# AiRyunn/BoT

Measured on AMD Instinct MI355X. Metric: edges/sec full-batch GAT fwd+bwd on ogbn-arxiv; achieved HBM GB/s vs peak, higher is better.
Workload: dtype f32

## Files before the change

### bot_amd/_C.py

```python
from __future__ import annotations

import ctypes
import os
from ctypes import c_char_p, c_double, c_float, c_int32, c_int64, c_uint64, c_void_p

import torch

_HERE = os.path.dirname(os.path.abspath(__file__))
LIB_PATH = os.environ.get("BOT_AMD_LIB") or os.path.join(_HERE, "lib", "libbot_gnn.so")
ABI_VERSION = 19

if not os.path.exists(LIB_PATH):
    raise ImportError(
        f"{LIB_PATH} is missing: build the gfx950 kernels first "
        "(`make -C bot_amd/csrc` or `python -c 'import __graft_entry__ as g; g.build()'`). "
        "bot_amd has no CPU / PyTorch fallback."
    )
_lib = ctypes.CDLL(LIB_PATH)

_P = c_void_p
_SIGS = {
    "bot_abi_version": (ctypes.c_int, []),
    "bot_last_error": (c_char_p, []),
    "bot_last_kernel": (c_char_p, []),
    "bot_debug_abort_trace": (ctypes.c_int, [c_char_p]),
    "bot_row_plan_default_chunk": (c_int32, [c_int64]),
    "bot_row_plan_size_host": (ctypes.c_int, [_P, c_int64, c_int32, _P, _P, _P]),
    "bot_row_plan_fill_host": (ctypes.c_int, [_P, c_int64, c_int32, _P, _P, _P]),
    "bot_degrees_i64": (ctypes.c_int, [_P, c_int64, _P, _P]),
    "bot_spmm_workspace_floats": (c_int64, [c_int64, c_int32, c_int32]),
    "bot_spmm_set_layout": (ctypes.c_int, [c_int32]),
    "bot_spmm_f32": (ctypes.c_int, [_P, _P, c_int64, c_int64, _P, c_int64, _P, _P, c_int64, _P, c_int64, c_int64, _P, _P,
                                    c_int32, c_int32, _P, c_int64, c_int64, _P, c_int64, c_int64, _P, _P]),
    "bot_spmm_blocked_f32": (ctypes.c_int, [_P, _P, _P, _P, _P, c_int32, c_int32, c_int32, c_int32, c_int32, c_int32, _P, c_int64, _P,
                                            c_int32, c_int32, _P, c_int64, _P, c_int64, _P]),
    "bot_spmm_dot_f32": (ctypes.c_int, [_P, _P, c_int64, c_int64, _P, c_int64, _P, _P, c_int64, _P, c_int64, c_int64, _P, _P,
                                        _P, c_int64, c_int64, c_int32, c_int32, _P, c_int64, c_int64, _P, _P, _P, _P]),
    "bot_spmm_bcast_f32": (ctypes.c_int, [_P, _P, c_int64, c_int64, _P, c_int64, _P, _P, c_int64, _P, c_int64, _P, _P, c_int32,
                                          c_int32, _P, c_int64, c_int64, _P, _P]),
    "bot_spmm_bcast_halves_f16": (ctypes.c_int, [_P, _P, c_int64, c_int64, _P, c_int64, _P, _P, c_int64, _P, c_int64, _P, _P, c_int32, c_int32, _P, _P,
                                                 c_int64, c_int64, c_int32, c_int32, _P, _P]),
    "bot_spmm_dot_bcast_f32": (ctypes.c_int, [_P, _P, c_int64, c_int64, _P, c_int64, _P, _P, c_int64, _P, c_int64, c_int64, _P,
                                              _P, _P, c_int64, c_int32, c_int32, _P, c_int64, _P, _P, _P]),
    "bot_sddmm_dot_f32": (ctypes.c_int, [_P, _P, c_int64, c_int64, _P, c_int64, _P, c_int64, c_int64, _P, c_int64, c_int64,
                                         c_int32, c_int32, _P, _P, c_int32, _P]),
    "bot_sddmm_dot_bcast_f32": (ctypes.c_int, [_P, _P, c_int64, c_int64, _P, c_int64, _P, c_int64, _P, c_int64, c_int64, c_int32,
                                               c_int32, _P, _P, _P]),
    "bot_sddmm_u_add_v_f32": (ctypes.c_int, [_P, _P, c_int64, _P, _P, c_int32, _P, _P]),
    "bot_gat_attn_fwd_f32": (ctypes.c_int, [_P, _P, c_int64, c_int64, _P, c_int64, c_int32, _P, _P, _P, _P, _P, c_float,
                                            c_int32, _P, _P, _P, c_float, c_uint64, _P, _P, _P]),
    "bot_gat_attn_bwd_f32": (ctypes.c_int, [_P, _P, c_int64, c_int64, _P, c_int64, c_int32, _P, _P, _P, _P, c_float, c_int32,
                                            _P, _P, _P, _P, _P, _P, _P, c_float, c_uint64, _P, _P]),
    "bot_gat_infer_workspace_floats": (c_int64, [c_int64, c_int32, c_int32]),
    "bot_gat_infer_f32": (ctypes.c_int, [_P, _P, c_int64, c_int64, _P, c_int64, _P, _P, c_int64, c_int64, _P, c_int64, c_int64,
                                         _P, c_int64, _P, c_int64, _P, _P, c_float, c_int32, c_int32, _P, c_int64, c_int64, _P, _P,
                                         c_int32, _P, c_int64, c_int64, _P, _P, _P]),
    "bot_segment_sum_f32": (ctypes.c_int, [_P, c_int64, c_int64, _P, c_int64, c_int32, _P, _P, c_int32, _P, _P]),
    "bot_gather_rows_f32": (ctypes.c_int, [_P, c_int64, _P, c_int64, c_int32, _P, c_int64, _P]),
    "bot_scatter_add_rows_f32": (ctypes.c_int, [_P, c_int64, _P, c_int64, c_int32, _P, c_int64, _P]),
    "bot_merge_weight_fwd_f32": (ctypes.c_int, [_P, _P, _P, _P, c_int32, c_int32, c_int32, c_int32, c_int32, c_int32, _P, _P]),
    "bot_merge_weight_bwd_f32": (ctypes.c_int, [_P, _P, _P, c_int32, c_int32, c_int32, c_int32, c_int32, c_int32, _P, _P, _P, _P, _P, _P]),
    "bot_edge_mlp_workspace_floats": (c_int64, []),
    "bot_edge_mlp_fwd_f32": (ctypes.c_int, [_P, c_int32, _P, _P, c_int32, _P, c_int32, c_int64, _P, _P]),
    "bot_edge_mlp_bwd_f32": (ctypes.c_int, [_P, c_int32, _P, _P, c_int32, _P, c_int32, _P, c_int64, _P, _P, _P, _P, _P]),
    "bot_random_keep_workspace_bytes": (c_int64, []),
    "bot_random_keep_u8": (ctypes.c_int, [c_int64, c_int64, c_uint64, _P, _P, _P]),
    "bot_halves_workspace_floats": (c_int64, []),
    "bot_halves_scale_f32": (ctypes.c_int, [_P, c_int64, c_int64, c_int32, _P, _P, _P]),
    "bot_halves_split_f16": (ctypes.c_int, [_P, c_int64, c_int64, c_int32, _P, c_int32, _P, c_int64, c_int32, _P]),
    "bot_halves_split_cols_f16": (ctypes.c_int, [_P, c_int64, c_int64, c_int32, _P, c_int32, _P, c_int64, c_int32, c_int32, _P]),
    "bot_halves_split_heads_f16": (ctypes.c_int, [_P, c_int64, c_int64, c_int32, c_int32, _P, _P, c_int64, c_int32, c_int32, _P]),
    "bot_gemm_halves_f32": (ctypes.c_int, [c_int32, c_int32, c_int64, c_int64, c_int64, _P, _P, c_int64, _P, c_int64, _P, c_int64,
                                           c_int32, c_int64, c_int64, c_int64, c_float, _P, c_int64, c_int32, c_int32, _P]),
    "bot_gemm_halves3_nt_f32": (ctypes.c_int, [c_int64, c_int64, c_int64, _P, _P, _P, c_int64, c_int64, _P, c_int64, c_int64, _P, c_int64,
                                               c_int32, _P]),
    "bot_gemm_halves3_tn_workspace_floats": (c_int64, [c_int64, c_int64, c_int64]),
    "bot_gemm_halves3_tn_f32": (ctypes.c_int, [c_int64, c_int64, c_int64, c_int64, c_int64, _P, _P, _P, c_int64, c_int64, _P, c_int64, c_int64, _P,
                                               c_int64, _P, c_int32, _P]),
    "bot_gemm_halves3_nt_grouped_f32": (ctypes.c_int, [c_int64, c_int64, _P, _P, _P, c_int64, c_int64, _P, c_int64, c_int64, _P, c_int64, c_int32, _P,
                                                       c_int32, _P, _P, c_int32, _P, c_int32, _P]),
    "bot_gemm_halves3_tn_grouped_workspace_floats": (c_int64, [c_int64, c_int32]),
    "bot_gemm_halves3_tn_grouped_f32": (ctypes.c_int, [c_int64, _P, _P, _P, c_int64, c_int64, _P, c_int64, c_int64, _P, c_int32, _P, _P, c_int32, _P]),
    "bot_tn_narrow_workspace_floats": (c_int64, [c_int64, c_int32, c_int32]),
    "bot_tn_narrow_f32": (ctypes.c_int, [_P, c_int64, _P, c_int64, c_int64, c_int32, c_int32, _P, c_int64, c_int32, _P, _P]),
    "bot_bn_act_bwd_reduce_max_f32": (ctypes.c_int, [_P, c_int64, _P, c_int64, c_int64, c_int32, _P, _P, _P, _P, c_int32, c_float, c_uint64, _P, _P, _P, _P, _P]),
    "bot_bn_bwd_bound_f32": (ctypes.c_int, [c_int32, c_int64, _P, _P, _P, c_double, _P, _P, _P, _P]),
    "bot_bn_act_bwd_apply_halves_f32": (ctypes.c_int, [_P, c_int64, _P, c_int64, c_int64, c_int32, _P, _P, _P, _P, c_int32, c_float, c_uint64, _P, _P, _P, c_double,
                                                       _P, c_int64, _P, _P, c_int64, c_int32, c_int32, c_int32, _P]),
    "bot_label_split_f32": (ctypes.c_int, [_P, c_int64, _P, c_int64, _P, c_float, c_uint64, _P, c_int32, _P, _P, _P, _P, _P]),
    "bot_build_input_f32": (ctypes.c_int, [_P, c_int64, c_int64, c_int32, c_int32, _P, c_float, c_uint64, _P, _P, c_int64, _P]),
    "bot_build_input_reuse_f32": (ctypes.c_int, [_P, c_int64, c_int64, c_int32, c_int32, _P, _P, _P, c_int64, c_float, c_uint64, _P, _P, c_int64, _P]),
    "bot_node_loss_f32": (ctypes.c_int, [_P, c_int64, c_int64, c_int32, _P, c_int64, _P, _P, c_int32, c_float, _P, c_int64, _P, c_int64, _P]),
    "bot_rmsprop_step_f32": (ctypes.c_int, [c_int32, _P, _P, _P, _P, c_float, _P, c_float, c_float, c_float, _P]),
    "bot_gemm_halves_last_algo": (ctypes.c_int, [_P, _P]),
    "bot_gemm_halves_library_version": (ctypes.c_int, [_P, _P]),
    "bot_tn_gemm_workspace_floats": (c_int64, [c_int64, c_int32, c_int32, c_int32]),
    "bot_tn_gemm_f32": (ctypes.c_int, [_P, c_int64, _P, c_int64, c_int64, c_int32, c_int32, _P, c_int64, c_int32, c_int32, c_int64, c_int64,
                                       c_int64, _P, _P]),
    "bot_skinny_gemm_f32": (ctypes.c_int, [_P, c_int64, _P, c_int64, c_int32, _P, c_int64, c_int64, c_int32, c_int32, c_int32, c_int32,
                                           c_int64, c_int64, c_int64, _P]),
    "bot_bn_workspace_floats": (c_int64, [c_int32]),
    "bot_colstats_f32": (ctypes.c_int, [_P, c_int64, c_int64, c_int32, _P, _P, _P, _P]),
    "bot_colsum_f32": (ctypes.c_int, [_P, c_int64, c_int64, c_int32, _P, _P, _P]),
    "bot_bn_stats_f32": (ctypes.c_int, [_P, c_int64, c_int64, c_int32, c_float, c_float, _P, _P, _P, _P, _P, _P, _P]),
    "bot_bn_stats_halves_f32": (ctypes.c_int, [_P, c_int64, c_int64, c_int32, c_float, c_float, _P, _P, _P, _P, _P, _P, _P, c_float, _P, _P, _P]),
    "bot_bn_act_fwd_halves_f32": (ctypes.c_int, [_P, c_int64, c_int64, c_int32, _P, _P, _P, _P, c_int32, c_float, c_uint64, _P, _P, c_int64,
                                                 _P, _P, c_int64, c_int32, c_int32, _P]),
    "bot_bn_act_fwd_f32": (ctypes.c_int, [_P, c_int64, c_int64, c_int32, _P, _P, _P, _P, c_int32, c_float, c_uint64, _P, _P, c_int64, _P]),
    "bot_bn_act_bwd_reduce_f32": (ctypes.c_int, [_P, c_int64, _P, c_int64, c_int64, c_int32, _P, _P, _P, _P, c_int32, c_float,
                                                 c_uint64, _P, _P, _P, _P, _P]),
    "bot_bn_act_bwd_apply_f32": (ctypes.c_int, [_P, c_int64, _P, c_int64, c_int64, c_int32, _P, _P, _P, _P, c_int32, c_float,
                                                c_uint64, _P, _P, _P, c_double, _P, c_int64, _P, _P]),
    "bot_halves_tn_combine_f32": (ctypes.c_int, [_P, _P, c_int32, c_int32, c_int32, c_int32, _P, _P, _P, c_int64, _P]),
    "bot_halves_scale_from_slots2_f32": (ctypes.c_int, [_P, c_float, _P, c_float, _P, _P]),
    "bot_halves_tail_f16": (ctypes.c_int, [c_int64, c_int32, _P, _P, _P, _P, _P, c_int64, c_int32, _P]),
    "bot_spmm_dot_halves_fits": (ctypes.c_int, [_P, c_int64, c_int64, _P, c_int64, c_int64, c_int32, c_int32, _P, c_int64, c_int64, c_int32]),
    "bot_spmm_dot_halves_f16": (ctypes.c_int, [_P, _P, c_int64, c_int64, _P, c_int64, _P, _P, c_int64, _P, c_int64, c_int64, _P, _P, _P, c_int64, c_int64,
                                               c_int32, c_int32, _P, _P, c_int64, c_int64, c_int32, _P, _P, _P]),
    "bot_gemm_halves3_nt_bn_rows": (c_int32, [c_int64]),
    "bot_gemm_halves3_nt3_f32": (ctypes.c_int, [c_int64, c_int64, c_int64, _P, _P, c_int64, _P, _P, c_int64, c_int64, _P, c_int64, c_int64, c_int32, _P, c_int64,
                                                _P, c_int32, _P]),
    "bot_bn_act_bwd_reduce_partials_f32": (ctypes.c_int, [_P, c_int32, c_int32, _P, _P, _P]),
    "bot_bn_bwd_bound_partials_f32": (ctypes.c_int, [c_int32, _P, c_int32, _P, _P, c_double, _P, _P, _P, _P]),
    "bot_bn_bwd_partials_finish_f32": (ctypes.c_int, [_P, _P, c_int32, c_int32, _P, _P, c_int32, c_double, _P, _P, _P, _P]),
    "bot_gemm_halves3_nt2_f32": (ctypes.c_int, [c_int64, c_int64, c_int64, _P, _P, c_int64, _P, _P, c_int64, c_int64, _P, c_int64, c_int64, c_int32, _P, c_int64,
                                                c_int32, _P]),
    "bot_halves_split_frag_f16": (ctypes.c_int, [_P, c_int64, c_int64, c_int32, _P, _P, c_int32, _P]),
    "bot_gemm_halves3_tn2_f32": (ctypes.c_int, [c_int64, c_int64, c_int64, c_int64, c_int64, _P, _P, _P, c_int64, _P, c_int64, c_int64, _P, c_int64, c_int64, _P,
                                                c_int64, _P, c_int32, _P]),
    "bot_stream_create": (ctypes.c_int, [c_int32, _P]),
    "bot_gemm_halves3_nt_grouped2_f32": (ctypes.c_int, [c_int64, c_int64, _P, _P, _P, c_int64, c_int64, _P, c_int64, c_int64, _P, c_int64, c_int32, _P,
                                                        c_int32, _P, _P, c_int32, _P, _P, _P, _P, c_int32, c_int32, _P]),
    "bot_bn_stats_halves_partials_f32": (ctypes.c_int, [_P, _P, c_int32, _P, c_int64, c_int32, c_float, c_float, _P, _P, _P, _P, _P, _P, _P, c_float, _P, _P, _P]),
    "bot_absmax_slots": (c_int32, []),
    "bot_absmax_slots_f32": (ctypes.c_int, [_P, c_int64, c_int64, c_int32, _P, _P]),
    "bot_halves_scale_from_slots_f32": (ctypes.c_int, [_P, _P, _P]),
    "bot_sample_neighbors_count_i32": (ctypes.c_int, [_P, c_int64, _P, c_int64, c_int32, _P, _P]),
    "bot_sample_neighbors_i32": (ctypes.c_int, [_P, c_int64, _P, c_int64, c_int32, c_uint64, _P, _P, _P]),
    "bot_block_tiles": (c_int64, [c_int64]),
    "bot_block_mark_i32": (ctypes.c_int, [_P, c_int64, _P, _P, c_int64, _P, c_int64, _P, _P, _P]),
    "bot_block_relabel_i32": (ctypes.c_int, [_P, c_int64, _P, _P, _P, c_int64, _P, c_int64, _P, c_int64, _P, _P, _P, _P]),
    "bot_subgraph_mark_i32": (ctypes.c_int, [_P, c_int64, _P, c_int64, _P, _P]),
    "bot_subgraph_count_i32": (ctypes.c_int, [_P, _P, c_int64, _P, c_int64, _P, _P, _P]),
    "bot_subgraph_fill_i32": (ctypes.c_int, [_P, _P, _P, c_int64, _P, c_int64, _P, _P, _P, _P, _P]),
    "bot_subgraph_unmark_i32": (ctypes.c_int, [_P, c_int64, _P, c_int64, _P]),
    "bot_sample_weights_prepare_f32": (ctypes.c_int, [_P, _P, c_int64, c_int64, _P, _P, _P, _P, _P]),
    "bot_sample_neighbors_weighted_count_i32": (ctypes.c_int, [_P, c_int64, _P, c_int64, c_int32, _P, _P]),
    "bot_sample_neighbors_weighted_i32": (ctypes.c_int, [_P, _P, _P, c_int64, _P, c_int64, c_int32, c_uint64, _P, _P, _P]),
}
for _name, (_res, _args) in _SIGS.items():
    _fn = getattr(_lib, _name)
    _fn.restype, _fn.argtypes = _res, _args
EXPORTED = tuple(_SIGS)

if _lib.bot_abi_version() != ABI_VERSION:
    raise ImportError(f"libbot_gnn.so ABI {_lib.bot_abi_version()} != binding ABI {ABI_VERSION}; rebuild")


class BotKernelError(RuntimeError):
    pass


PROFILE = None


PROFILE_SKIP = ()


def _timed(name, key, launch):
    if PROFILE is None or name in PROFILE_SKIP:
        return launch()
    e0, e1 = torch.cuda.Event(enable_timing=True), torch.cuda.Event(enable_timing=True)
    e0.record()
    rc = launch()
    e1.record()
    PROFILE.append((name, key, e0, e1, _lib.bot_last_kernel().decode()))
    return rc


def _check(rc: int, what: str):
    if rc != 0:
        raise BotKernelError(f"{what} failed (rc={rc}): {_lib.bot_last_error().decode()}")


def _ptr(t):
    return None if t is None else t.data_ptr()


def _ld(t):
    return max(int(t.stride(-2)), int(t.shape[-1])) if t.shape[-2] == 1 else int(t.stride(-2))


def _stream():
    return torch.cuda.current_stream().cuda_stream


def _dev(*ts):
    dev = None
    for t in ts:
        if t is None:
            continue
        if not t.is_cuda:
            raise BotKernelError(
                "bot_amd kernels run on MI355X only: got a CPU tensor and there is no CPU fallback "
                "(move the graph and features to the GPU)")
        if dev is None:
            dev = t.device
        elif t.device != dev:
            raise BotKernelError(f"operands live on different devices ({dev} and {t.device}): graph structures and features "
                                 "must be on the same GPU")


def _f32(t, name):
    if t is not None and t.dtype != torch.float32:
# ... 699 lines not shown
    return (ctypes.c_int64 * len(flat))(*flat)


def gemm_halves3_nt_grouped(a, b, scale_a, scale_b, a2_off, b2_off, out, groups, k_seg, mode=0, col_scale=None, col_shift=None, relu=False, absmax=None,
                            stats=None):
    _dev(a, b, out, scale_a, scale_b, col_scale, col_shift, absmax)
    assert a.dtype == torch.float16 and b.dtype == torch.float16 and a.dim() == 2 and b.dim() == 2 and a.stride(1) == 1 and b.stride(1) == 1
    assert out.dtype == torch.float32 and out.stride(-1) == 1
    tab = _table(groups, 6)
    sp = sm = sv = None
    sF = 0
    if stats is not None:
        sp, sm, sv = stats
        _dev(sp, sm, sv)
        sF = sv.shape[1]
        tiles = (a.shape[0] + 255) // 256
        assert sp.shape == (tiles, 2, sF) and sm.shape == (tiles, 2, sF) and sv.shape == (tiles, sF)
        assert sp.is_contiguous() and sm.is_contiguous() and sv.is_contiguous()
        assert sp.dtype == sm.dtype == sv.dtype == torch.float32
    _check(_timed("gemm_halves", (a.shape[0], sum(int(g[1]) * 96 * int(g[4]) for g in groups), 1, 1), lambda: _lib.bot_gemm_halves3_nt_grouped2_f32(
        a.shape[0], b.shape[0], scale_a.data_ptr(), scale_b.data_ptr(), a.data_ptr(), _ld(a), a2_off, b.data_ptr(), _ld(b), b2_off, out.data_ptr(),
        int(out.stride(-2)), len(groups), tab, int(k_seg), _ptr(col_scale), _ptr(col_shift), int(bool(relu)), _ptr(absmax), _ptr(sp), _ptr(sm), _ptr(sv),
        int(sF), int(mode), _stream())), "gemm_halves3_nt_grouped")
    return out


def gemm_halves3_tn_grouped(x, d, scale_x, scale_d, x2_off, d2_off, out, tiles, mode=0):
    _dev(x, d, out, scale_x, scale_d)
    assert x.dtype == torch.float16 and d.dtype == torch.float16 and x.stride(1) == 1 and d.stride(1) == 1 and x.shape[0] == d.shape[0]
    assert out.dtype == torch.float32 and out.is_contiguous()
    n = x.shape[0]
    ws = torch.empty(int(_lib.bot_gemm_halves3_tn_grouped_workspace_floats(n, len(tiles))), dtype=torch.float32, device=x.device)
    tab = _table(tiles, 7)
    _check(_timed("gemm_halves", (n, sum(3 * int(t[1]) * int(t[3]) for t in tiles), 1, 1), lambda: _lib.bot_gemm_halves3_tn_grouped_f32(
        n, scale_x.data_ptr(), scale_d.data_ptr(), x.data_ptr(), _ld(x), x2_off, d.data_ptr(), _ld(d), d2_off, out.data_ptr(), len(tiles), tab,
        ws.data_ptr(), int(mode), _stream())), "gemm_halves3_tn_grouped")
    return out


def gemm_halves3_tn(x, d, scale_x, scale_d, piece_x, piece_d, k, p, mode=0, x2_off=None, d2_off=None, scale_d2=None, p_split=0):
    _dev(x, d, scale_x, scale_d, scale_d2)
    n = x.shape[0]
    out = torch.empty((k, p), dtype=torch.float32, device=x.device)
    ws = torch.empty(int(_lib.bot_gemm_halves3_tn_workspace_floats(n, piece_x, piece_d)), dtype=torch.float32, device=x.device)
    _check(_timed("gemm_halves", (k, p, 3 * n, 1), lambda: _lib.bot_gemm_halves3_tn2_f32(
        n, k, p, piece_x, piece_d, scale_x.data_ptr(), scale_d.data_ptr(), _ptr(scale_d2), int(p_split), x.data_ptr(), _ld(x),
        2 * piece_x if x2_off is None else x2_off, d.data_ptr(), _ld(d), 2 * piece_d if d2_off is None else d2_off,
        out.data_ptr(), _ld(out), ws.data_ptr(), int(mode), _stream())), "gemm_halves3_tn")
    return out


def _idx64(t, name):
    if t.dtype != torch.int64 or not t.is_contiguous() or t.dim() != 1:
        raise BotKernelError(f"{name} must be a contiguous 1-D int64 tensor (got {t.dtype}, stride {tuple(t.stride())})")


def _labels64(labels):
    if labels.dtype != torch.int64:
        raise BotKernelError(f"labels must be int64 (got {labels.dtype})")
    lab = labels.reshape(labels.shape[0], -1)
    if lab.shape[1] > 1 and lab.stride(1) != 1:
        lab = lab.contiguous()
    return lab


def label_split(train_idx, labels, mask, mask_rate, seed, use_labels, code, wn):
    _dev(train_idx, labels, wn)
    _idx64(train_idx, "train_idx")
    count = torch.empty(1, dtype=torch.float32, device=wn.device)
    ws = torch.empty(128, dtype=torch.int32, device=wn.device)
    lab = _labels64(labels)
    if wn.dtype != torch.float32 or not wn.is_contiguous() or (code is not None and (code.dtype != torch.int32 or not code.is_contiguous())):
        raise BotKernelError("label_split: wn must be contiguous float32, code contiguous int32")
    m = None
    if mask is not None:
        _dev(mask)
        m = mask.to(torch.bool).contiguous().view(torch.uint8)
        if m.numel() != train_idx.numel():
            raise BotKernelError("label_split: mask must have one entry per training node")
    _check(_lib.bot_label_split_f32(train_idx.data_ptr(), train_idx.numel(), lab.data_ptr(), lab.stride(0), _ptr(m), float(mask_rate), int(seed),
                                    _seed_off(1.0), int(bool(use_labels)), _ptr(code), wn.data_ptr(), count.data_ptr(), ws.data_ptr(), _stream()), "label_split")
    return count


def build_input(feat, code, n_classes, p, seed):
    _dev(feat)
    _f32(feat, "feat")
    n, F = feat.shape
    out = torch.empty((n, F + n_classes), dtype=torch.float32, device=feat.device)
    _check(_lib.bot_build_input_f32(feat.data_ptr(), _ld(feat), n, F, n_classes, _ptr(code), float(p), int(seed), _seed_off(p), out.data_ptr(), _ld(out),
                                    _stream()), "build_input")
    return out


REUSE_CALLS = 0


def build_input_reuse(feat, code, reuse, pred, n_classes, p, seed, out=None):
    global REUSE_CALLS
    _dev(feat, code, reuse, pred, out)
    _f32(feat, "feat"), _f32(pred, "pred"), _f32(out, "out")
    n, F = feat.shape
    if feat.stride(1) != 1 and F > 1:
        feat = feat.contiguous()
    if pred.dim() != 2 or pred.shape[0] != n or pred.shape[1] < n_classes or (pred.stride(1) != 1 and pred.shape[1] > 1):
        raise BotKernelError(f"build_input_reuse: pred must be [{n}, >= {n_classes}] with unit column stride, got {tuple(pred.shape)}")
    if code is None or code.dtype != torch.int32 or not code.is_contiguous() or code.numel() != n:
        raise BotKernelError(f"build_input_reuse: code must be contiguous int32 [{n}]")
    if reuse is not None and (reuse.dtype != torch.uint8 or not reuse.is_contiguous() or reuse.numel() != n):
        raise BotKernelError(f"build_input_reuse: reuse must be contiguous uint8 [{n}]")
    if out is None:
        out = torch.empty((n, F + n_classes), dtype=torch.float32, device=feat.device)
    elif out.shape != (n, F + n_classes) or out.stride(1) != 1:
        raise BotKernelError(f"build_input_reuse: out must be [{n}, {F + n_classes}] with unit column stride")
    _check(_lib.bot_build_input_reuse_f32(feat.data_ptr(), _ld(feat), n, F, n_classes, code.data_ptr(), _ptr(reuse), pred.data_ptr(), _ld(pred), float(p),
                                          int(seed), _seed_off(p), out.data_ptr(), _ld(out), _stream()), "build_input_reuse")
    REUSE_CALLS += 1
    torch.autograd.graph.increment_version(out)
    return out


LOSS_KINDS = {"logit": 0, "loge": 1, "savage": 2}


def node_loss(x, labels, wn, count, kind, eps, want_grad=True):
    _dev(x, labels, wn, count)
    _f32(x, "x")
    n, C = x.shape
    n_pad = (n + 63) // 64 * 64
    y = torch.empty(n_pad, dtype=torch.float32, device=x.device)
    dx = torch.empty((n, C), dtype=torch.float32, device=x.device) if want_grad else None
    lab = _labels64(labels)
    if wn.dtype != torch.float32 or not wn.is_contiguous() or count.dtype != torch.float32:
        raise BotKernelError("node_loss: wn / count must be contiguous float32")
    _check(_lib.bot_node_loss_f32(x.data_ptr(), _ld(x), n, C, lab.data_ptr(), lab.stride(0), wn.data_ptr(), count.data_ptr(), LOSS_KINDS[kind], float(eps),
                                  y.data_ptr(), n_pad, _ptr(dx), C, _stream()), "node_loss")
    return y, dx


def rmsprop_step(params, grads, square_avgs, lr, alpha, eps, weight_decay, lr_dev=None):
    for i in range(0, len(params), 48):
        ps, gs, sq = params[i:i + 48], grads[i:i + 48], square_avgs[i:i + 48]
        k = len(ps)
        for t in (*ps, *gs, *sq):
            if t.dtype != torch.float32 or not t.is_contiguous():
                raise BotKernelError("rmsprop_step: contiguous float32 tensors only")
        P = (c_void_p * k)(*[t.data_ptr() for t in ps])
        G = (c_void_p * k)(*[t.data_ptr() for t in gs])
        S = (c_void_p * k)(*[t.data_ptr() for t in sq])
        Nn = (c_int64 * k)(*[t.numel() for t in ps])
        if lr_dev is not None and (lr_dev.dtype != torch.float32 or lr_dev.device != ps[0].device):
            raise BotKernelError("rmsprop_step: a tensor learning rate must be float32 on the parameters' device")
        _check(_lib.bot_rmsprop_step_f32(k, P, G, S, Nn, float(lr), _ptr(lr_dev), float(alpha), float(eps), float(weight_decay), _stream()), "rmsprop_step")


def skinny_gemm(a, b, *, b_is_kn, out, accumulate=False, batch=1, strides=(0, 0, 0), m=None, n=None, k=None, ldc=None):
    _dev(a, b, out)
    for t, name in ((a, "a"), (b, "b"), (out, "out")):
        _f32(t, name)
        if t.stride(-1) != 1 and t.shape[-1] != 1:
            raise BotKernelError(f"skinny_gemm: {name} must have unit column stride")
    if m is None:
        m, k = a.shape[-2], a.shape[-1]
    if n is None:
        n = b.shape[-1] if b_is_kn else b.shape[-2]
    sa, sb, sc = strides
    _check(_timed("skinny_gemm", (m, n, k, batch), lambda: _lib.bot_skinny_gemm_f32(
        a.data_ptr(), _ld(a), b.data_ptr(), _ld(b), int(b_is_kn), out.data_ptr(), _ld(out) if ldc is None else ldc, m, n, k,
        int(accumulate), batch, sa, sb, sc, _stream())), "skinny_gemm")
    return out


def tn_gemm(x, y, *, out=None, batch=1, strides=(0, 0, 0), n=None, kx=None, ky=None, transpose_out=False):
    _dev(x, y)
    _f32(x, "x"), _f32(y, "y")
    if (x.stride(-1) != 1 and x.shape[-1] != 1) or (y.stride(-1) != 1 and y.shape[-1] != 1):
        raise BotKernelError("tn_gemm: operands must have unit column stride")
    if n is None:
        n, kx, ky = x.shape[-2], x.shape[-1], y.shape[-1]
    if out is None:
        shp = (ky, kx) if transpose_out else (kx, ky)
        out = torch.empty(shp if batch == 1 else (batch,) + shp, dtype=torch.float32, device=x.device)
    sx, sy, so = strides
    if batch > 1 and so == 0:
        so = out.stride(0)
    ws = torch.empty(int(_lib.bot_tn_gemm_workspace_floats(n, kx, ky, batch)), dtype=torch.float32, device=x.device)
    _check(_timed("tn_gemm", (n, kx, ky, batch), lambda: _lib.bot_tn_gemm_f32(
        x.data_ptr(), _ld(x), y.data_ptr(), _ld(y), n, kx, ky, out.data_ptr(), _ld(out), int(transpose_out), batch, sx, sy, so,
        ws.data_ptr(),
        _stream())), "tn_gemm")
    return out


def tn_narrow(x, y, out, transpose_out=False):
    _dev(x, y, out)
    _f32(x, "x"), _f32(y, "y"), _f32(out, "out")
    n, kx, ky = x.shape[0], x.shape[1], y.shape[1]
    assert y.shape[0] == n and out.shape == ((ky, kx) if transpose_out else (kx, ky))
    if x.stride(1) != 1 or y.stride(1) != 1 or (out.stride(1) != 1 and out.shape[1] != 1):
        raise BotKernelError("tn_narrow: operands must have unit column stride")
    ws = torch.empty(int(_lib.bot_tn_narrow_workspace_floats(n, kx, ky)), dtype=torch.float32, device=x.device)
    _check(_timed("tn_narrow", (n, kx, ky), lambda: _lib.bot_tn_narrow_f32(
        x.data_ptr(), _ld(x), y.data_ptr(), _ld(y), n, kx, ky, out.data_ptr(), _ld(out), int(transpose_out), ws.data_ptr(), _stream())), "tn_narrow")
    return out


def colsum(x):
    _dev(x)
    x = _mat(x, "x")
    n, F = x.shape
    out = torch.empty(F, dtype=torch.float32, device=x.device)
    _check(_lib.bot_colsum_f32(x.data_ptr(), x.stride(0), n, F, out.data_ptr(), _bn_ws(F, x.device).data_ptr(), _stream()), "colsum")
    return out


def _written(*ts):
    ts = [t for t in ts if t is not None]
    if ts:
        torch._C._increment_version(ts)


def bn_stats(x, eps, momentum, running_mean=None, running_var=None, num_batches_tracked=None):
    _dev(x, running_mean, running_var)
    x = _mat(x, "x")
    n, F = x.shape
    mean = torch.empty(F, dtype=torch.float32, device=x.device)
    invstd = torch.empty(F, dtype=torch.float32, device=x.device)
    _check(_lib.bot_bn_stats_f32(x.data_ptr(), x.stride(0), n, F, float(eps), float(momentum), mean.data_ptr(), invstd.data_ptr(),
                                 _ptr(running_mean), _ptr(running_var), _ptr(num_batches_tracked), _bn_ws(F, x.device).data_ptr(),
                                 _stream()), "bn_stats")
    _written(running_mean, running_var, num_batches_tracked)
    return mean, invstd


def bn_stats_halves(x, eps, momentum, running_mean, running_var, num_batches_tracked, weight, bias, p):
    _dev(x, running_mean, running_var, weight, bias)
    x = _mat(x, "x")
    n, F = x.shape
    mean = torch.empty(F, dtype=torch.float32, device=x.device)
    invstd = torch.empty(F, dtype=torch.float32, device=x.device)
    hscale = torch.empty(2, dtype=torch.float32, device=x.device)
    _check(_lib.bot_bn_stats_halves_f32(x.data_ptr(), x.stride(0), n, F, float(eps), float(momentum), mean.data_ptr(), invstd.data_ptr(),
                                        _ptr(running_mean), _ptr(running_var), _ptr(num_batches_tracked), _ptr(weight), _ptr(bias),
                                        float(p), hscale.data_ptr(), _bn_ws(F, x.device).data_ptr(), _stream()), "bn_stats_halves")
    _written(running_mean, running_var, num_batches_tracked)
    return mean, invstd, hscale


def bn_stats_halves_partials(part, minmax, pivot, n, eps, momentum, running_mean, running_var, num_batches_tracked, weight, bias, p):
    _dev(part, minmax, pivot, running_mean, running_var, weight, bias)
    nblk, _, F = part.shape
    assert pivot.shape == (nblk, F) and minmax.shape == part.shape and part.is_contiguous() and minmax.is_contiguous() and pivot.is_contiguous()
    mean = torch.empty(F, dtype=torch.float32, device=part.device)
    invstd = torch.empty(F, dtype=torch.float32, device=part.device)
    hscale = torch.empty(2, dtype=torch.float32, device=part.device)
    ws = torch.empty(F, dtype=torch.float32, device=part.device)
    _check(_lib.bot_bn_stats_halves_partials_f32(part.data_ptr(), minmax.data_ptr(), int(nblk), pivot.data_ptr(), int(n), int(F), float(eps), float(momentum),
                                                 mean.data_ptr(), invstd.data_ptr(), _ptr(running_mean), _ptr(running_var), _ptr(num_batches_tracked),
                                                 _ptr(weight), _ptr(bias), float(p), hscale.data_ptr(), ws.data_ptr(), _stream()), "bn_stats_halves_partials")
    _written(running_mean, running_var, num_batches_tracked)
    return mean, invstd, hscale


def bn_act_fwd(x, mean, invstd, weight, bias, relu, p, seed, halves=None, want_y=True):
    _dev(x, mean, invstd)
    x = _mat(x, "x")
    n, F = x.shape
    if halves is not None:
        hscale, piece = halves[:2]
        pieces = halves[2] if len(halves) > 2 else 3
        y = torch.empty((n, F), dtype=torch.float32, device=x.device) if want_y else None
        buf = torch.empty((n, pieces * piece), dtype=torch.float16, device=x.device)
        _check(_timed("bn_act_fwd", (F,), lambda: _lib.bot_bn_act_fwd_halves_f32(
            x.data_ptr(), x.stride(0), n, F, mean.data_ptr(), invstd.data_ptr(), _ptr(weight), _ptr(bias), int(relu), float(p),
            int(seed), _seed_off(p), _ptr(y), F, hscale.data_ptr(), buf.data_ptr(), buf.stride(0), piece, pieces, _stream())),
            "bn_act_fwd_halves")
        return y, buf
    y = torch.empty((n, F), dtype=torch.float32, device=x.device)
    _check(_timed("bn_act_fwd", (F,), lambda: _lib.bot_bn_act_fwd_f32(
        x.data_ptr(), x.stride(0), n, F, mean.data_ptr(), invstd.data_ptr(), _ptr(weight), _ptr(bias), int(relu), float(p),
        int(seed), _seed_off(p), y.data_ptr(), y.stride(0), _stream())), "bn_act_fwd")
    return y


def bn_act_bwd_reduce(dy, x, mean, invstd, weight, bias, relu, p, seed, want_max=False):
    _dev(dy, x)
    dy, x = _mat(dy, "dy"), _mat(x, "x")
    n, F = x.shape
    sg = torch.empty(F, dtype=torch.float32, device=x.device)
    sgx = torch.empty(F, dtype=torch.float32, device=x.device)
    ws = _bn_ws(F, x.device)
    fn = _lib.bot_bn_act_bwd_reduce_max_f32 if want_max else _lib.bot_bn_act_bwd_reduce_f32
    _check(fn(dy.data_ptr(), dy.stride(0), x.data_ptr(), x.stride(0), n, F, mean.data_ptr(), invstd.data_ptr(), _ptr(weight), _ptr(bias), int(relu),
              float(p), int(seed), _seed_off(p), sg.data_ptr(), sgx.data_ptr(), ws.data_ptr(), _stream()), "bn_act_bwd_reduce")
    return (sg, sgx, ws) if want_max else (sg, sgx)


def bn_bwd_bound(ws, n, sum_g, sum_gx, total_count, weight, invstd, slots):
    _dev(ws, invstd, slots)
    F = invstd.shape[0]
    _check(_lib.bot_bn_bwd_bound_f32(F, n, ws.data_ptr(), _ptr(sum_g), _ptr(sum_gx), float(total_count), _ptr(weight), invstd.data_ptr(), slots.data_ptr(),
                                     _stream()), "bn_bwd_bound")
    return slots


def bn_act_bwd_apply_halves(dy, x, mean, invstd, weight, bias, relu, p, seed, sum_g, sum_gx, total_count, hscale, hout, hD, hDP, out=None, h2_off=None):
# ... 62 lines not shown


class PreparedWeights:

    def __init__(self, prefix, n_pos):
        self.prefix, self.n_pos = prefix, n_pos


def sample_weights_prepare(csc, w):
    _dev(csc.indptr, w)
    _f32(w, "edge weights")
    E = int(csc.indices.numel())
    if not (w.dim() == 1 or (w.dim() == 2 and w.shape[1] == 1)) or w.shape[0] != E:
        raise ValueError(f"edge weights must be [E] or [E, 1] with E = {E}, got {tuple(w.shape)}")
    w = w.reshape(-1).contiguous()
    dev = w.device
    prefix = torch.empty(E, dtype=torch.int64, device=dev)
    n_pos = torch.empty(csc.n_rows, dtype=torch.int32, device=dev)
    flag = torch.empty(1, dtype=torch.int32, device=dev)
    rc = _lib.bot_sample_weights_prepare_f32(csc.indptr.data_ptr(), csc.eid.data_ptr(), csc.n_rows, E, w.data_ptr(), prefix.data_ptr(),
                                             n_pos.data_ptr(), flag.data_ptr(), _stream())
    if rc == -2:
        raise ValueError(f"edge weights: {_lib.bot_last_error().decode()}")
    _check(rc, "sample_weights_prepare")
    return PreparedWeights(prefix, n_pos)


def sample_neighbors_weighted(csc, prepared, seeds, k, seed):
    _dev(csc.indptr, prepared.prefix, seeds)
    assert seeds.dtype == torch.int32 and seeds.is_contiguous()
    n = int(seeds.numel())
    dev = seeds.device
    counts = torch.empty(n, dtype=torch.int32, device=dev)
    _check(_lib.bot_sample_neighbors_weighted_count_i32(prepared.n_pos.data_ptr(), csc.n_rows, _ptr(seeds), n, int(k), _ptr(counts),
                                                        _stream()), "sample_neighbors_weighted_count")
    offsets = torch.zeros(n + 1, dtype=torch.int64, device=dev)
    torch.cumsum(counts, 0, out=offsets[1:])
    total = int(offsets[-1])
    pos = torch.empty(total, dtype=torch.int32, device=dev)
    _check(_timed("sample_weighted", (int(k),), lambda: _lib.bot_sample_neighbors_weighted_i32(
        csc.indptr.data_ptr(), prepared.prefix.data_ptr(), prepared.n_pos.data_ptr(), csc.n_rows, _ptr(seeds), n, int(k),
        seed & 0xFFFFFFFFFFFFFFFF, offsets.data_ptr(), _ptr(pos), _stream())), "sample_neighbors_weighted")
    return offsets, pos


def block_relabel(csc, seeds, pos, node_map):
    _dev(csc.indptr, seeds, pos, node_map)
    n_seeds, n_pos, n_nodes = int(seeds.numel()), int(pos.numel()), int(node_map.numel())
    dev = seeds.device
    tiles = torch.empty(max(1, int(_lib.bot_block_tiles(n_nodes))), dtype=torch.int64, device=dev)
    n_new = torch.zeros(1, dtype=torch.int64, device=dev)
    _check(_lib.bot_block_mark_i32(_ptr(seeds), n_seeds, csc.indices.data_ptr(), _ptr(pos), n_pos, node_map.data_ptr(), n_nodes,
                                   tiles.data_ptr(), n_new.data_ptr(), _stream()), "block_mark")
    n_src = n_seeds + int(n_new)
    src_nid = torch.empty(n_src, dtype=torch.int32, device=dev)
    local = torch.empty(n_pos, dtype=torch.int32, device=dev)
    parent_eid = torch.empty(n_pos, dtype=torch.int32, device=dev)
    _check(_lib.bot_block_relabel_i32(_ptr(seeds), n_seeds, csc.indices.data_ptr(), csc.eid.data_ptr(), _ptr(pos), n_pos, node_map.data_ptr(),
                                      n_nodes, tiles.data_ptr(), n_src, _ptr(src_nid), _ptr(local), _ptr(parent_eid), _stream()), "block_relabel")
    return src_nid, local, parent_eid


def node_subgraph(csc, nodes, node_map):
    _dev(csc.indptr, nodes, node_map)
    _i32(nodes, "nodes"), _i32(node_map, "node_map")
    n, n_nodes = int(nodes.numel()), int(node_map.numel())
    dev = nodes.device
    if csc.n_rows != n_nodes:
        raise ValueError(f"node_subgraph takes a square parent: {csc.n_rows} CSC rows, a node map of {n_nodes}")
    if n > n_nodes:
        raise ValueError(f"{n} nodes asked of a graph of {n_nodes}: the set holds a duplicate")
    tail = torch.zeros(n + 2, dtype=torch.int64, device=dev)
    offsets, n_dup = tail[:n + 1], tail[n + 1:]
    empty = torch.empty(0, dtype=torch.int32, device=dev)
    if n == 0:
        return offsets, empty, empty.clone()
    counts = torch.empty(n, dtype=torch.int32, device=dev)
    st = _stream()

    def extract():
        rc = _lib.bot_subgraph_mark_i32(nodes.data_ptr(), n, node_map.data_ptr(), n_nodes, n_dup.data_ptr(), st)
        return rc or _lib.bot_subgraph_count_i32(csc.indptr.data_ptr(), csc.indices.data_ptr(), csc.n_rows, nodes.data_ptr(), n,
                                                 node_map.data_ptr(), counts.data_ptr(), st)
    _check(_timed("subgraph", ("count",), extract), "subgraph_mark / subgraph_count")
    torch.cumsum(counts, 0, out=offsets[1:])
    total, bad = (int(x) for x in tail[n:].tolist())
    if bad:
        _check(_lib.bot_subgraph_unmark_i32(nodes.data_ptr(), n, node_map.data_ptr(), n_nodes, st), "subgraph_unmark")
        out_of_range, dup = bad >> 32, bad & 0xFFFFFFFF
        raise ValueError(f"node_subgraph: {dup} duplicate and {out_of_range} out-of-range ids among the {n} nodes "
                         f"(ids are unique and in [0, {n_nodes}))")
    local_src = torch.empty(total, dtype=torch.int32, device=dev)
    parent_eid = torch.empty(total, dtype=torch.int32, device=dev)

    def fill():
        rc = 0
        if total:
            rc = _lib.bot_subgraph_fill_i32(csc.indptr.data_ptr(), csc.indices.data_ptr(), csc.eid.data_ptr(), csc.n_rows, nodes.data_ptr(), n,
                                            node_map.data_ptr(), offsets.data_ptr(), local_src.data_ptr(), parent_eid.data_ptr(), st)
        return rc or _lib.bot_subgraph_unmark_i32(nodes.data_ptr(), n, node_map.data_ptr(), n_nodes, st)
    _check(_timed("subgraph", ("fill",), fill), "subgraph_fill / subgraph_unmark")
    return offsets, local_src, parent_eid


def edge_mlp_fwd(ef, W1, b1, W2):
    _dev(ef, W1, b1, W2)
    ef, W1, b1, W2 = (_f32(t, "edge_mlp operand").contiguous() for t in (ef, W1, b1, W2))
    E, H = ef.shape[0], W2.shape[0]
    out = torch.empty((E, H), dtype=torch.float32, device=ef.device)
    _check(_lib.bot_edge_mlp_fwd_f32(ef.data_ptr(), ef.shape[1], W1.data_ptr(), b1.data_ptr(), W1.shape[0], W2.data_ptr(), H, E,
                                     out.data_ptr(), _stream()), "edge_mlp_fwd")
    return out


def edge_mlp_bwd(ef, W1, b1, W2, dz):
    _dev(ef, W1, b1, W2, dz)
    ef, W1, b1, W2, dz = (_f32(t, "edge_mlp operand").contiguous() for t in (ef, W1, b1, W2, dz))
    E, H = ef.shape[0], W2.shape[0]
    dW1, db1, dW2 = torch.empty_like(W1), torch.empty_like(b1), torch.empty_like(W2)
    ws = torch.empty(int(_lib.bot_edge_mlp_workspace_floats()), dtype=torch.float32, device=ef.device)
    _check(_lib.bot_edge_mlp_bwd_f32(ef.data_ptr(), ef.shape[1], W1.data_ptr(), b1.data_ptr(), W1.shape[0], W2.data_ptr(), H,
                                     dz.data_ptr(), E, dW1.data_ptr(), db1.data_ptr(), dW2.data_ptr(), ws.data_ptr(), _stream()),
           "edge_mlp_bwd")
    return dW1, db1, dW2


def merge_weight_fwd(W, Wres, attn_l, attn_r, H, D, P, with_fc, block=None):
    block = H * D if block is None else int(block)
    _dev(W, Wres, attn_l, attn_r)
    W = _f32(W, "W").contiguous()
    Wres = None if Wres is None else _f32(Wres, "Wres").contiguous()
    al = _f32(attn_l, "attn_l").contiguous()
    ar = None if attn_r is None else _f32(attn_r, "attn_r").contiguous()
    K = W.shape[1]
    out = torch.empty((K, P), dtype=torch.float32, device=W.device)
    _check(_lib.bot_merge_weight_fwd_f32(W.data_ptr(), _ptr(Wres), al.data_ptr(), _ptr(ar), H, D, K, P, int(with_fc), block, out.data_ptr(),
                                         _stream()), "merge_weight_fwd")
    return out


def merge_weight_bwd(W, attn_l, attn_r, H, D, P, with_fc, has_res, dm, block=None):
    _dev(W, attn_l, attn_r, dm)
    block = H * D if block is None else int(block)
    W, al, dm = W.contiguous(), attn_l.contiguous(), _f32(dm, "d_merged").contiguous()
    ar = None if attn_r is None else attn_r.contiguous()
    K = W.shape[1]
    dW = torch.empty_like(W)
    dWres = torch.empty_like(W) if has_res else None
    dal = torch.empty_like(al)
    dar = None if ar is None else torch.empty_like(ar)
    _check(_lib.bot_merge_weight_bwd_f32(W.data_ptr(), al.data_ptr(), _ptr(ar), H, D, K, P, int(with_fc), block, dm.data_ptr(), dW.data_ptr(),
                                         _ptr(dWres), dal.data_ptr(), _ptr(dar), _stream()), "merge_weight_bwd")
    return dW, dWres, dal, dar
```

### bot_amd/csrc/common.h

```cpp
#pragma once
#include <hip/hip_runtime.h>
#include <stdint.h>
#include <stdio.h>

#include "../../include/bot_gnn.h"

namespace bot {

void set_error(const char* fmt, ...);
void set_kernel(const char* fmt, ...);
void launch_halves_scale(const float* part, int n, float* scale, hipStream_t st);

inline int hip_status(const char* what) {
    hipError_t e = hipGetLastError();
    if (e != hipSuccess) {
        set_error("%s: %s", what, hipGetErrorString(e));
        return (int)e;
    }
    return 0;
}

#define BOT_REQUIRE(cond, code, ...)    \
    do {                                \
        if (!(cond)) {                  \
            bot::set_error(__VA_ARGS__); \
            return (code);              \
        }                               \
    } while (0)

inline bool aligned(const void* p, size_t a) { return (reinterpret_cast<uintptr_t>(p) % a) == 0; }

constexpr int kBlock = 256;
constexpr int kWave = 64;

template <int VEC> struct Vec;
template <> struct Vec<1> { using type = float; };
template <> struct Vec<2> { using type = float2; };
template <> struct Vec<4> { using type = float4; };

template <int VEC>
__device__ __forceinline__ void vload(float (&r)[VEC], const float* p) {
    using T = typename Vec<VEC>::type;
    T v = *reinterpret_cast<const T*>(p);
    if constexpr (VEC == 1) { r[0] = v; }
    if constexpr (VEC == 2) { r[0] = v.x; r[1] = v.y; }
    if constexpr (VEC == 4) { r[0] = v.x; r[1] = v.y; r[2] = v.z; r[3] = v.w; }
}

template <int VEC>
__device__ __forceinline__ void vstore_nt(float* p, const float (&r)[VEC]) {
    typedef float nv __attribute__((ext_vector_type(VEC)));
    nv v;
#pragma unroll
    for (int t = 0; t < VEC; ++t) v[t] = r[t];
    __builtin_nontemporal_store(v, reinterpret_cast<nv*>(p));
}

template <int VEC>
__device__ __forceinline__ void vstore(float* p, const float (&r)[VEC]) {
    using T = typename Vec<VEC>::type;
    T v;
    if constexpr (VEC == 1) { v = r[0]; }
    if constexpr (VEC == 2) { v.x = r[0]; v.y = r[1]; }
    if constexpr (VEC == 4) { v.x = r[0]; v.y = r[1]; v.z = r[2]; v.w = r[3]; }
    *reinterpret_cast<T*>(p) = v;
}

template <int LANES>
__device__ __forceinline__ int group_bcast(int v, int j) {
    if constexpr (LANES == 64) return __builtin_amdgcn_readlane(v, j);
    else return __shfl(v, j, LANES);
}
template <int LANES>
__device__ __forceinline__ float group_bcast(float v, int j) {
    return __int_as_float(group_bcast<LANES>(__float_as_int(v), j));
}

template <int LANES>
__device__ __forceinline__ float group_sum(float v) {
#pragma unroll
    for (int m = LANES / 2; m >= 1; m >>= 1) v += __shfl_xor(v, m, LANES);
    return v;
}
template <int LANES>
__device__ __forceinline__ float group_max(float v) {
#pragma unroll
    for (int m = LANES / 2; m >= 1; m >>= 1) v = fmaxf(v, __shfl_xor(v, m, LANES));
    return v;
}

template <int LANES>
__device__ __forceinline__ float transpose_reduce4(float (&p)[4], int lane) {
    const bool h2 = lane & 2;
    float r[2];
#pragma unroll
    for (int i = 0; i < 2; ++i) {
        const float keep = h2 ? p[i + 2] : p[i];
        const float send = h2 ? p[i] : p[i + 2];
        r[i] = keep + __shfl_xor(send, 2, LANES);
    }
    const bool h1 = lane & 1;
    float s = (h1 ? r[1] : r[0]) + __shfl_xor(h1 ? r[0] : r[1], 1, LANES);
#pragma unroll
    for (int m = 4; m < LANES; m <<= 1) s += __shfl_xor(s, m, LANES);
    return s;
}

template <int LANES>
__device__ __forceinline__ float transpose_reduce16(float (&p)[16], int lane) {
    float q[8], r[4], s2[2];
    const bool b8 = lane & 8, b4 = lane & 4, b2 = lane & 2, b1 = lane & 1;
#pragma unroll
    for (int i = 0; i < 8; ++i) q[i] = (b8 ? p[i + 8] : p[i]) + __shfl_xor(b8 ? p[i] : p[i + 8], 8, LANES);
#pragma unroll
    for (int i = 0; i < 4; ++i) r[i] = (b4 ? q[i + 4] : q[i]) + __shfl_xor(b4 ? q[i] : q[i + 4], 4, LANES);
#pragma unroll
    for (int i = 0; i < 2; ++i) s2[i] = (b2 ? r[i + 2] : r[i]) + __shfl_xor(b2 ? r[i] : r[i + 2], 2, LANES);
    float s = (b1 ? s2[1] : s2[0]) + __shfl_xor(b1 ? s2[0] : s2[1], 1, LANES);
#pragma unroll
    for (int m = 16; m < LANES; m <<= 1) s += __shfl_xor(s, m, LANES);
    return s;
}

struct Philox {
    static __device__ __forceinline__ void round(uint32_t (&c)[4], uint32_t k0, uint32_t k1) {
        const uint64_t p0 = (uint64_t)0xD2511F53u * c[0], p1 = (uint64_t)0xCD9E8D57u * c[2];
        const uint32_t n0 = (uint32_t)(p1 >> 32) ^ c[1] ^ k0, n1 = (uint32_t)p1;
        const uint32_t n2 = (uint32_t)(p0 >> 32) ^ c[3] ^ k1, n3 = (uint32_t)p0;
        c[0] = n0, c[1] = n1, c[2] = n2, c[3] = n3;
    }
    static __device__ __forceinline__ void gen(uint64_t seed, uint64_t ctr, uint32_t (&out)[4]) {
        uint32_t c[4] = {(uint32_t)ctr, (uint32_t)(ctr >> 32), 0u, 0u};
        uint32_t k0 = (uint32_t)seed, k1 = (uint32_t)(seed >> 32);
#pragma unroll
        for (int i = 0; i < 10; ++i) {
            round(c, k0, k1);
            k0 += 0x9E3779B9u, k1 += 0xBB67AE85u;
        }
#pragma unroll
        for (int i = 0; i < 4; ++i) out[i] = c[i];
    }
};

constexpr int kAbsmaxSlots = 64;
#ifdef __HIPCC__
__device__ __forceinline__ float wave_absmax(float m) {
#pragma unroll
    for (int o = 32; o > 0; o >>= 1) m = fmaxf(m, __shfl_xor(m, o));
    return m;
}
__device__ __forceinline__ void absmax_publish(float wave_max, uint32_t* slots) {
    if ((threadIdx.x & 63) == 0) {
        const uint32_t bits = __float_as_uint(wave_max);
        uint32_t* p = slots + ((blockIdx.x + 7 * blockIdx.y) & (kAbsmaxSlots - 1));
        if (bits > __hip_atomic_load(p, __ATOMIC_RELAXED, __HIP_MEMORY_SCOPE_AGENT)) atomicMax(p, bits);
    }
}
#endif
void launch_absmax_slots(const float* x, int64_t ldx, int64_t n, int32_t F, uint32_t* slots, hipStream_t st);

constexpr float kHalvesShift = 2048.f;

inline int pick_vec(int32_t D, std::initializer_list<int64_t> strides, std::initializer_list<const void*> ptrs) {
    for (int v : {4, 2}) {
        bool ok = (D % v) == 0;
        for (int64_t s : strides) ok = ok && (s % v) == 0;
        for (const void* p : ptrs) ok = ok && (p == nullptr || aligned(p, 4 * v));
        if (ok) return v;
    }
    return 1;
}


}
```

### bot_amd/csrc/halves.hip

```cpp
#include <hip/hip_fp16.h>

#include "common.h"

namespace bot {

constexpr int kMaxBlocks = 1024;

__global__ __launch_bounds__(kBlock) void absmax_partial_kernel(const float* x, int64_t ldx, int64_t n, int32_t F, float* part) {
    __shared__ float lds[kBlock / kWave];
    float m = 0.f;
    const int64_t total = n * (int64_t)F;
    if (ldx == F && (reinterpret_cast<uintptr_t>(x) & 15) == 0) {
        const int64_t nq = total >> 2;
        const float4* x4 = reinterpret_cast<const float4*>(x);
        const int64_t stride = (int64_t)gridDim.x * kBlock;
        int64_t i = (int64_t)blockIdx.x * kBlock + threadIdx.x;
        for (; i + 3 * stride < nq; i += 4 * stride) {
            const float4 a = x4[i], b = x4[i + stride], c = x4[i + 2 * stride], d = x4[i + 3 * stride];
            m = fmaxf(m, fmaxf(fmaxf(fmaxf(fabsf(a.x), fabsf(a.y)), fmaxf(fabsf(a.z), fabsf(a.w))),
                               fmaxf(fmaxf(fabsf(b.x), fabsf(b.y)), fmaxf(fabsf(b.z), fabsf(b.w)))));
            m = fmaxf(m, fmaxf(fmaxf(fmaxf(fabsf(c.x), fabsf(c.y)), fmaxf(fabsf(c.z), fabsf(c.w))),
                               fmaxf(fmaxf(fabsf(d.x), fabsf(d.y)), fmaxf(fabsf(d.z), fabsf(d.w)))));
        }
        for (; i < nq; i += stride) {
            const float4 a = x4[i];
            m = fmaxf(m, fmaxf(fmaxf(fabsf(a.x), fabsf(a.y)), fmaxf(fabsf(a.z), fabsf(a.w))));
        }
        for (int64_t j = (nq << 2) + (int64_t)blockIdx.x * kBlock + threadIdx.x; j < total; j += stride) m = fmaxf(m, fabsf(x[j]));
    } else if (ldx == F) {
        for (int64_t i = (int64_t)blockIdx.x * kBlock + threadIdx.x; i < total; i += (int64_t)gridDim.x * kBlock) m = fmaxf(m, fabsf(x[i]));
    } else {
        for (int64_t i = (int64_t)blockIdx.x * kBlock + threadIdx.x; i < total; i += (int64_t)gridDim.x * kBlock) {
            const int64_t r = i / F;
            m = fmaxf(m, fabsf(x[r * ldx + (i - r * F)]));
        }
    }
#pragma unroll
    for (int o = 32; o > 0; o >>= 1) m = fmaxf(m, __shfl_xor(m, o));
    if ((threadIdx.x & 63) == 0) lds[threadIdx.x >> 6] = m;
    __syncthreads();
    if (threadIdx.x == 0) {
        for (int w = 1; w < kBlock / kWave; ++w) m = fmaxf(m, lds[w]);
        part[blockIdx.x] = m;
    }
}

__global__ __launch_bounds__(kWave) void halves_scale_kernel(const float* part, int nblk, float* scale) {
    float m = 0.f;
    for (int i = threadIdx.x; i < nblk; i += kWave) m = fmaxf(m, part[i]);
#pragma unroll
    for (int o = 32; o > 0; o >>= 1) m = fmaxf(m, __shfl_xor(m, o));
    if (threadIdx.x == 0) {
        float s = 1.f;
        if (m > 0.f && m < INFINITY) {
            int e;
            const float f = frexpf(m, &e);
            if (f == 0.5f) e -= 1;
            s = ldexpf(1.f, min(60, 14 - e));
        }
        scale[0] = s;
        scale[1] = 1.f / s;
    }
}

template <int ORDER>
__global__ __launch_bounds__(128) void halves_split_kernel(const float* x, int64_t ldx, int32_t F, const float* scale, __half* out,
                                                           int64_t ldo, int32_t piece, bool wide, int32_t width) {
    const int64_t r = blockIdx.x;
    const int c = (blockIdx.y * 128 + threadIdx.x) * 2;
    if (c >= width) return;
    const float s = scale ? scale[0] : 1.f;
    float v0 = 0.f, v1 = 0.f;
    const float* xr = x + r * ldx;
    if (c + 1 < F) {
        if (wide) {
            const float2 v = *reinterpret_cast<const float2*>(xr + c);
            v0 = v.x * s, v1 = v.y * s;
        } else {
            v0 = xr[c] * s, v1 = xr[c + 1] * s;
        }
    } else if (c < F) {
        v0 = xr[c] * s;
    }
    const __half a0 = __float2half_rn(v0), a1 = __float2half_rn(v1);
    const float r0 = v0 - __half2float(a0), r1 = v1 - __half2float(a1);
    __half* o = out + r * ldo + c;
    const __half2 hi = __halves2half2(a0, a1);
    *reinterpret_cast<__half2*>(o) = hi;
    if (ORDER == 0) {
        *reinterpret_cast<__half2*>(o + piece) = hi;
        *reinterpret_cast<__half2*>(o + 2 * (int64_t)piece) = __halves2half2(__float2half_rn(r0 * kHalvesShift), __float2half_rn(r1 * kHalvesShift));
    } else if (ORDER == 2) {
        *reinterpret_cast<__half2*>(o + piece) = __halves2half2(__float2half_rn(r0 * kHalvesShift), __float2half_rn(r1 * kHalvesShift));
    } else {
        *reinterpret_cast<__half2*>(o + piece) = __halves2half2(__float2half_rn(r0), __float2half_rn(r1));
        *reinterpret_cast<__half2*>(o + 2 * (int64_t)piece) =
            __halves2half2(__float2half_rn(__half2float(a0) * (1.f / kHalvesShift)), __float2half_rn(__half2float(a1) * (1.f / kHalvesShift)));
    }
}

__global__ __launch_bounds__(128) void halves_split_frag_kernel(const float* x, int64_t ldx, int64_t n, int32_t F, const float* scale, __half* out,
                                                                int32_t piece, int64_t region) {
    const int64_t r = blockIdx.x;
    const int c = (blockIdx.y * 128 + threadIdx.x) * 2;
    if (c >= piece) return;
    const float s = scale ? scale[0] : 1.f;
    float v0 = 0.f, v1 = 0.f;
    if (r < n) {
        const float* xr = x + r * ldx;
        if (c < F) v0 = xr[c] * s;
        if (c + 1 < F) v1 = xr[c + 1] * s;
    }
    const __half a0 = __float2half_rn(v0), a1 = __float2half_rn(v1);
    const float r0 = v0 - __half2float(a0), r1 = v1 - __half2float(a1);
    const int T = piece >> 5;
    const int64_t o = ((((r >> 4) * T + (c >> 5)) * 64) + ((r & 15) + 16 * ((c & 31) >> 3))) * 8 + (c & 7);
    *reinterpret_cast<__half2*>(out + o) = __halves2half2(a0, a1);
    *reinterpret_cast<__half2*>(out + region + o) = __halves2half2(__float2half_rn(r0), __float2half_rn(r1));
}

__global__ __launch_bounds__(128) void halves_split_heads_kernel(const float* x, int64_t ldx, int32_t H, int32_t D, const float* scale, __half* out,
                                                                 int64_t ldo, int32_t h2_off, int32_t DP, bool wide) {
    const int64_t r = blockIdx.x;
    const int c = (blockIdx.y * 128 + threadIdx.x) * 2;
    if (c >= H * DP) return;
    const int h = c / DP, j = c - h * DP;
    const float s = scale ? scale[0] : 1.f;
    float v0 = 0.f, v1 = 0.f;
    const float* xr = x + r * ldx + (int64_t)h * D + j;
    if (j + 1 < D) {
        if (wide) {
            const float2 v = *reinterpret_cast<const float2*>(xr);
            v0 = v.x * s, v1 = v.y * s;
        } else {
            v0 = xr[0] * s, v1 = xr[1] * s;
        }
    } else if (j < D) {
        v0 = xr[0] * s;
    }
    const __half a0 = __float2half_rn(v0), a1 = __float2half_rn(v1);
    const float r0 = v0 - __half2float(a0), r1 = v1 - __half2float(a1);
    __half* o = out + r * ldo + c;
    *reinterpret_cast<__half2*>(o) = __halves2half2(a0, a1);
    *reinterpret_cast<__half2*>(o + h2_off) = __halves2half2(__float2half_rn(r0 * kHalvesShift), __float2half_rn(r1 * kHalvesShift));
}

__global__ __launch_bounds__(kWave) void halves_scale2_kernel(const float* part, int nblk, float mult, const float* cap, float cap_ratio, float* scale) {
    float m = 0.f;
    for (int i = threadIdx.x; i < nblk; i += kWave) m = fmaxf(m, part[i]);
#pragma unroll
    for (int o = 32; o > 0; o >>= 1) m = fmaxf(m, __shfl_xor(m, o));
    if (threadIdx.x == 0) {
        m *= mult;
        float s = 1.f;
        if (m > 0.f && m < INFINITY) {
            int e;
            const float f = frexpf(m, &e);
            if (f == 0.5f) e -= 1;
            s = ldexpf(1.f, min(60, 14 - e));
        }
        if (cap) s = fminf(s, cap[0] * cap_ratio);
        scale[0] = s;
        scale[1] = 1.f / s;
    }
}

constexpr int kTailSegs = 8;
struct TailArgs {
    int col[kTailSegs], width[kTailSegs];
    const float* src[kTailSegs];
    int64_t ld[kTailSegs];
    int n_seg, total;
};
__global__ __launch_bounds__(kBlock) void halves_tail_kernel(TailArgs t, int64_t n, const float* scale, __half* out, int64_t ldo, int32_t h2_off) {
    const int64_t gid = (int64_t)blockIdx.x * kBlock + threadIdx.x;
    if (gid >= n * t.total) return;
    const int64_t r = gid / t.total;
    int j = (int)(gid - r * t.total), g = 0;
    while (j >= t.width[g]) j -= t.width[g], ++g;
    const float v = t.src[g] ? t.src[g][r * t.ld[g] + j] * scale[0] : 0.f;
    const __half a = __float2half_rn(v);
    __half* o = out + r * ldo + t.col[g] + j;
    o[0] = a;
    o[h2_off] = __float2half_rn((v - __half2float(a)) * kHalvesShift);
}

void launch_halves_scale(const float* part, int n, float* scale, hipStream_t st) {
    hipLaunchKernelGGL(halves_scale_kernel, dim3(1), dim3(kWave), 0, st, part, n, scale);
}

__global__ __launch_bounds__(kBlock) void absmax_slots_kernel(const float* x, int64_t ldx, int64_t n, int32_t F, uint32_t* slots) {
    float m = 0.f;
    const int64_t total = n * (int64_t)F;
    const int64_t stride = (int64_t)gridDim.x * kBlock;
    if (ldx == F && (reinterpret_cast<uintptr_t>(x) & 15) == 0) {
        const int64_t nq = total >> 2;
        const float4* x4 = reinterpret_cast<const float4*>(x);
        int64_t i = (int64_t)blockIdx.x * kBlock + threadIdx.x;
        for (; i + 3 * stride < nq; i += 4 * stride) {
            const float4 a = x4[i], b = x4[i + stride], c = x4[i + 2 * stride], d = x4[i + 3 * stride];
            m = fmaxf(m, fmaxf(fmaxf(fmaxf(fabsf(a.x), fabsf(a.y)), fmaxf(fabsf(a.z), fabsf(a.w))),
                               fmaxf(fmaxf(fabsf(b.x), fabsf(b.y)), fmaxf(fabsf(b.z), fabsf(b.w)))));
            m = fmaxf(m, fmaxf(fmaxf(fmaxf(fabsf(c.x), fabsf(c.y)), fmaxf(fabsf(c.z), fabsf(c.w))),
                               fmaxf(fmaxf(fabsf(d.x), fabsf(d.y)), fmaxf(fabsf(d.z), fabsf(d.w)))));
        }
        for (; i < nq; i += stride) {
            const float4 a = x4[i];
            m = fmaxf(m, fmaxf(fmaxf(fabsf(a.x), fabsf(a.y)), fmaxf(fabsf(a.z), fabsf(a.w))));
        }
        for (int64_t j = (nq << 2) + (int64_t)blockIdx.x * kBlock + threadIdx.x; j < total; j += stride) m = fmaxf(m, fabsf(x[j]));
    } else {
        for (int64_t i = (int64_t)blockIdx.x * kBlock + threadIdx.x; i < total; i += stride) {
// ... 175 lines not shown
```

### bot_amd/csrc/merge.hip

```cpp
#include "common.h"

namespace bot {

struct MergeArgs {
    const float* W;
    const float* Wres;
    const float* al;
    const float* ar;
    int32_t H, D, K, P, with_fc;
    int32_t blk;
    float* out;
    const float* dm;
    float* dW;
    float* dWres;
    float* dal;
    float* dar;
};

__global__ __launch_bounds__(kBlock) void merge_fwd_kernel(MergeArgs a, int n_tiles, int tiles_k) {
    __shared__ float tile[32][33];
    const int HD = a.H * a.D;
    const int c0 = a.with_fc ? a.blk : 0, c1 = c0 + (a.Wres ? a.blk : 0), c2 = c1 + a.H, c3 = c2 + (a.ar ? a.H : 0);
    if ((int)blockIdx.x < n_tiles) {
        const int tk = blockIdx.x % tiles_k, tp = blockIdx.x / tiles_k;
        const int tx = threadIdx.x & 31, ty = threadIdx.x >> 5;
#pragma unroll
        for (int j = 0; j < 32; j += 8) {
            const int p = tp * 32 + ty + j, k = tk * 32 + tx;
            float v = 0.f;
            if (p < c1 && k < a.K) {
                const bool first = p < c0 || !a.with_fc;
                const int q = p < c0 ? p : p - c0;
                if (q < HD) v = (a.with_fc && first) ? a.W[(int64_t)q * a.K + k] : a.Wres[(int64_t)q * a.K + k];
            }
            tile[ty + j][tx] = v;
        }
        __syncthreads();
#pragma unroll
        for (int j = 0; j < 32; j += 8) {
            const int k = tk * 32 + ty + j, p = tp * 32 + tx;
            if (p < c1 && k < a.K) a.out[(int64_t)k * a.P + p] = tile[tx][ty + j];
        }
        return;
    }
    const int64_t gid = (int64_t)(blockIdx.x - n_tiles) * kBlock + threadIdx.x;
    const int nq = a.P - c1;
    if (gid >= (int64_t)nq * a.K) return;
    const int q = (int)(gid / a.K), k = (int)(gid - (int64_t)q * a.K), p = c1 + q;
    float v = 0.f;
    if (p < c3) {
        const bool left = p < c2;
        const int h = left ? p - c1 : p - c2;
        const float* at = left ? a.al : a.ar;
        const float* wc = a.W + (int64_t)h * a.D * a.K + k;
        const float* ah = at + h * a.D;
        float s0 = 0.f, s1 = 0.f, s2 = 0.f, s3 = 0.f;
        int d = 0;
        for (; d + 8 <= a.D; d += 8) {
            float w[8];
#pragma unroll
            for (int t = 0; t < 8; ++t) w[t] = wc[(int64_t)(d + t) * a.K];
            s0 = fmaf(w[0], ah[d], s0), s1 = fmaf(w[1], ah[d + 1], s1), s2 = fmaf(w[2], ah[d + 2], s2), s3 = fmaf(w[3], ah[d + 3], s3);
            s0 = fmaf(w[4], ah[d + 4], s0), s1 = fmaf(w[5], ah[d + 5], s1), s2 = fmaf(w[6], ah[d + 6], s2), s3 = fmaf(w[7], ah[d + 7], s3);
        }
        for (; d < a.D; ++d) s0 = fmaf(wc[(int64_t)d * a.K], ah[d], s0);
        v = (s0 + s1) + (s2 + s3);
    }
    a.out[(int64_t)k * a.P + p] = v;
}

__global__ __launch_bounds__(kBlock) void merge_bwd_w_kernel(MergeArgs a) {
    const int64_t gid = (int64_t)blockIdx.x * kBlock + threadIdx.x;
    const int HD = a.H * a.D;
    if (gid >= (int64_t)HD * a.K) return;
    const int p = (int)(gid / a.K), k = (int)(gid - (int64_t)p * a.K);
    const int h = p / a.D;
    const int c0 = a.with_fc ? a.blk : 0, c1 = c0 + (a.Wres ? a.blk : 0), c2 = c1 + a.H;
    const float* row = a.dm + (int64_t)k * a.P;
    float g = a.with_fc ? row[p] : 0.f;
    g = fmaf(a.al[p], row[c1 + h], g);
    if (a.ar) g = fmaf(a.ar[p], row[c2 + h], g);
    a.dW[gid] = g;
    if (a.dWres) a.dWres[gid] = row[c0 + p];
}

__global__ __launch_bounds__(kBlock) void merge_bwd_a_kernel(MergeArgs a) {
    const int lane = threadIdx.x & 63;
    const int p = (int)(((int64_t)blockIdx.x * kBlock + threadIdx.x) >> 6);
    const int HD = a.H * a.D;
    if (p >= HD) return;
    const int h = p / a.D;
    const int c0 = a.with_fc ? a.blk : 0, c1 = c0 + (a.Wres ? a.blk : 0), c2 = c1 + a.H;
    float sl = 0.f, sr = 0.f;
    for (int k = lane; k < a.K; k += 64) {
        const float w = a.W[(int64_t)p * a.K + k];
        sl = fmaf(w, a.dm[(int64_t)k * a.P + c1 + h], sl);
        if (a.ar) sr = fmaf(w, a.dm[(int64_t)k * a.P + c2 + h], sr);
    }
    sl = group_sum<64>(sl);
    sr = group_sum<64>(sr);
    if (lane == 0) {
        a.dal[p] = sl;
        if (a.dar) a.dar[p] = sr;
    }
}

static int merge_check(const char* who, const float* W, const float* al, int32_t H, int32_t D, int32_t K, int32_t P, const float* Wres,
                       const float* ar, int32_t with_fc, int32_t blk) {
    BOT_REQUIRE(H >= 1 && D >= 1 && K >= 1, BOT_E_RANGE, "%s: H=%d D=%d K=%d", who, H, D, K);
    BOT_REQUIRE(blk >= H * D, BOT_E_RANGE, "%s: block width %d smaller than H*D = %d", who, blk, H * D);
    BOT_REQUIRE(W && al, BOT_E_NULL, "%s: W / attn_l is NULL", who);
    const int64_t used = (int64_t)(with_fc ? blk : 0) + (Wres ? blk : 0) + H + (ar ? H : 0);
    BOT_REQUIRE(P >= used, BOT_E_RANGE, "%s: P=%d smaller than the %lld merged columns", who, P, (long long)used);
    return 0;
}

}

extern "C" {

int bot_merge_weight_fwd_f32(const float* W, const float* Wres, const float* attn_l, const float* attn_r, int32_t H, int32_t D,
                             int32_t K, int32_t P, int32_t with_fc, int32_t block, float* out, bot_stream_t stream) {
    using namespace bot;
    if (int rc = merge_check("merge_weight_fwd", W, attn_l, H, D, K, P, Wres, attn_r, with_fc, block)) return rc;
    BOT_REQUIRE(out != nullptr, BOT_E_NULL, "merge_weight_fwd: out is NULL");
    MergeArgs a{W, Wres, attn_l, attn_r, H, D, K, P, with_fc, block, out, nullptr, nullptr, nullptr, nullptr, nullptr};
    const int c1 = (with_fc ? block : 0) + (Wres ? block : 0);
    const int tiles_k = (K + 31) / 32, n_tiles = tiles_k * ((c1 + 31) / 32);
    const int64_t rest = (int64_t)(P - c1) * K;
    hipLaunchKernelGGL(merge_fwd_kernel, dim3((unsigned)(n_tiles + (rest + kBlock - 1) / kBlock)), dim3(kBlock), 0, (hipStream_t)stream, a,
                       n_tiles, tiles_k);
    return hip_status("merge_weight_fwd launch");
}

int bot_merge_weight_bwd_f32(const float* W, const float* attn_l, const float* attn_r, int32_t H, int32_t D, int32_t K, int32_t P,
                             int32_t with_fc, int32_t block, const float* d_merged, float* dW, float* dWres, float* d_attn_l, float* d_attn_r,
                             bot_stream_t stream) {
    using namespace bot;
    if (int rc = merge_check("merge_weight_bwd", W, attn_l, H, D, K, P, dWres, attn_r, with_fc, block)) return rc;
    BOT_REQUIRE(d_merged && dW && d_attn_l && ((attn_r == nullptr) == (d_attn_r == nullptr)), BOT_E_NULL, "merge_weight_bwd: NULL pointer");
    MergeArgs a{W, dWres, attn_l, attn_r, H, D, K, P, with_fc, block, nullptr, d_merged, dW, dWres, d_attn_l, d_attn_r};
    hipStream_t st = (hipStream_t)stream;
    const int64_t n = (int64_t)H * D * K;
    hipLaunchKernelGGL(merge_bwd_w_kernel, dim3((unsigned)((n + kBlock - 1) / kBlock)), dim3(kBlock), 0, st, a);
    hipLaunchKernelGGL(merge_bwd_a_kernel, dim3((unsigned)(((int64_t)H * D * 64 + kBlock - 1) / kBlock)), dim3(kBlock), 0, st, a);
    return hip_status("merge_weight_bwd launch");
}

}
```

### bot_amd/nn/__init__.py

```python
from __future__ import annotations

import torch
import torch.nn as nn
import torch.nn.functional as F

from .. import gemm, halo, ops
from ..errors import DGLError

__all__ = ["ElementWiseLinear", "GraphConv", "GATConv", "GCN", "GAT"]


def _pair(x):
    return x if isinstance(x, tuple) else (x, x)


def _sampled(graph) -> bool:
    return graph.is_block and graph.halo is None


def _src_rows(graph, x):
    if not _sampled(graph):
        return graph.extend(x)
    if x.shape[0] != graph.number_of_src_nodes():
        raise ValueError(f"a block takes features of its {graph.number_of_src_nodes()} source nodes, got {x.shape[0]} rows")
# ... 167 lines not shown

    def reset_parameters(self):
        gain = nn.init.calculate_gain("relu")
        for lin in (getattr(self, n, None) for n in ("fc", "fc_src", "fc_dst", "res_fc")):
            if isinstance(lin, nn.Linear):
                nn.init.xavier_normal_(lin.weight, gain=gain)
        nn.init.xavier_normal_(self.attn_l, gain=gain)
        if isinstance(self.attn_r, nn.Parameter):
            nn.init.xavier_normal_(self.attn_r, gain=gain)

    def set_allow_zero_in_degree(self, set_value):
        self._allow_zero_in_degree = set_value

    def _kept_edges(self, graph):
        return ops.random_edge_keep(graph, self.edge_drop)

    def forward(self, graph, feat, keep=None):
        if not self._allow_zero_in_degree:
            assert not has_zero_in_degree(graph), "0-in-degree nodes (models.py:477-479)"
        H, D = self._num_heads, self._out_feats
        if isinstance(feat, tuple):
            h, h_dst = self.feat_drop(feat[0]), self.feat_drop(feat[1])
            W, W_dst = (self.fc_src.weight, self.fc_dst.weight) if hasattr(self, "fc_src") else (self.fc.weight, self.fc.weight)
        else:
            if not hasattr(self, "fc"):
                raise DGLError("a GATConv built with a pair of input sizes takes a (feat_src, feat_dst) pair")
            h = self.feat_drop(feat)
            h_dst = h[:graph.number_of_dst_nodes()] if _sampled(graph) else h
            W = W_dst = self.fc.weight
        ft = F.linear(h, W).view(-1, H, D)
        Wh = W.view(H, D, -1)
        el = F.linear(h, (Wh * self.attn_l.view(H, D, 1)).sum(1))
        er = None
        if self.attn_r is not None:
            Wd = Wh if W_dst is W else W_dst.view(H, D, -1)
            er = F.linear(h_dst, (Wd * self.attn_r.view(H, D, 1)).sum(1)).unsqueeze(-1)
        if self._use_symmetric_norm:
            norm = degree_norm(graph, "out", -0.5)
            ft = ft * _bcast(norm, ft)
            el = el * norm.unsqueeze(-1)
        transfer = halo.start(graph, ft) if halo.enabled(graph) else None
        if transfer is None:
            ft = _src_rows(graph, ft)
        el = _src_rows(graph, el).unsqueeze(-1)
        keep_order = "eid"
        if keep is None and self.training and self.edge_drop > 0:
            keep, keep_order = self._kept_edges(graph), "csc"
        a = ops.gat_attention(graph, el, er, keep=keep, negative_slope=self.leaky_relu.negative_slope, order="csc",
                              keep_order=keep_order)
        a = self.attn_drop(a)
        rst = ops.u_mul_e_sum(graph, ft, a, order="csc") if transfer is None else halo.u_mul_e_sum(graph, ft, a, transfer=transfer)
        if self._use_symmetric_norm:
            rst = rst * _bcast(degree_norm(graph, "in", 0.5), rst)
        if self.res_fc is not None:
            rst = torch.addmm(rst.reshape(rst.shape[0], H * D), h_dst, self.res_fc.weight.t()).view(-1, H, D)
        if self._activation is not None:
            rst = self._activation(rst)
        return rst


def _block_list(graph, feat, n_layers):
    if not isinstance(graph, (list, tuple)):
        if feat is None:
            raise TypeError("a stack called on a Graph needs its node features")
        return None
    if len(graph) != n_layers:
        raise ValueError(f"{n_layers} layers need {n_layers} blocks, got {len(graph)}")
    return list(graph)


class GCN(nn.Module):

    def __init__(self, in_feats, n_classes, n_hidden, n_layers, activation, norm="none", norm_adj="symm",
                 dropout=0.0, input_drop=0, residual=False, use_linear=False):
        super().__init__()
        self.n_layers, self.n_hidden, self.n_classes = n_layers, n_hidden, n_classes
        self.use_linear, self.residual = use_linear, residual
        self.convs = nn.ModuleList()
        if use_linear:
            self.linear = nn.ModuleList()
        self.norms = nn.ModuleList()
        for i in range(n_layers):
            fin = n_hidden if i > 0 else in_feats
            fout = n_hidden if i < n_layers - 1 else n_classes
            last = i == n_layers - 1
            self.convs.append(GraphConv(fin, fout, "both" if norm_adj == "symm" else "right", bias=norm == "none" or last))
            if use_linear:
                self.linear.append(nn.Linear(fin, fout, bias=False))
            if not last and norm == "batch":
                self.norms.append(nn.BatchNorm1d(fout))
        self.input_drop, self.dropout = nn.Dropout(input_drop), nn.Dropout(dropout)
        self.activation = activation

    def forward(self, graph, feat=None):
        from . import fused
        blocks = _block_list(graph, feat, self.n_layers)
        h = graph.to_internal(feat) if blocks is None else (blocks[0].srcdata["feat"] if feat is None else feat)
        if not fused.take_input_dropped():
            h = self.input_drop(h)
        h_last = None
        for i in range(self.n_layers):
            g = graph if blocks is None else blocks[i]
            conv = self.convs[i](g, h)
            if self.use_linear:
                h = conv + self.linear[i](h if blocks is None else h[:conv.shape[0]])
            else:
                h = conv
            if i < self.n_layers - 1:
                if self.residual and h_last is not None:
                    h = h + (h_last if blocks is None else h_last[:h.shape[0]])
                h_last = h
                if len(self.norms):
                    h = _epilogue(h, self.norms[i], self.activation, self.dropout, self.training)
                else:
                    h = self.dropout(self.activation(h))
        return h if blocks is not None else graph.to_original(h)


class GAT(nn.Module):

    def __init__(self, dim_node, dim_edge, dim_output, n_hidden, n_layers, n_heads, activation, norm="none",
                 dropout=0.0, input_drop=0.0, attn_drop=0.0, edge_drop=0.0, non_interactive_attn=False,
                 use_symmetric_norm=False, linear=False, residual=False):
        super().__init__()
        self.n_node_feats, self.n_hidden, self.n_classes = dim_node, n_hidden, dim_output
        self.n_layers, self.num_heads = n_layers, n_heads
        self.convs, self.norms, self.biases = nn.ModuleList(), nn.ModuleList(), nn.ModuleList()
        for i in range(n_layers):
            last = i == n_layers - 1
            fin = n_heads * n_hidden if i > 0 else dim_node
            fout = dim_output if last else n_hidden
            heads = 1 if last else n_heads
            self.convs.append(GATConv(fin, fout, num_heads=heads, attn_drop=attn_drop, edge_drop=edge_drop,
                                      non_interactive_attn=non_interactive_attn,
                                      use_symmetric_norm=use_symmetric_norm, linear=linear))
            if last:
                self.biases.append(ElementWiseLinear(fout, weight=False, bias=True))
            elif norm == "batch":
                self.norms.append(nn.BatchNorm1d(heads * fout))
            elif norm == "none":
                self.biases.append(ElementWiseLinear(heads * fout, weight=False, bias=True))
        self.input_drop, self.dropout = nn.Dropout(input_drop), nn.Dropout(dropout)
        self.activation, self.residual = activation, residual
        self.fuse_layers = True

    def forward(self, graph, feat=None):
        from . import fused
        blocks = _block_list(graph, feat, self.n_layers)
        h = graph.to_internal(feat) if blocks is None else (blocks[0].srcdata["feat"] if feat is None else feat)
        if not fused.take_input_dropped():
            h = self.input_drop(h)
        h_last = None
        infer = self.fuse_layers and not self.training and not torch.is_grad_enabled() and (h.is_cuda or fused.FORCE)
        for i in range(self.n_layers):
            last = i == self.n_layers - 1
            g = graph if blocks is None else blocks[i]
            if infer:
                epi = self.biases[-1] if last else (self.norms[i] if len(self.norms) else self.biases[i])
                if fused.can_infer(self.convs[i], epi, self.activation, g, self.residual, last):
                    h = fused.gat_infer_layer(self.convs[i], epi, g, h, relu=not last, first=i == 0)
                    if last:
                        return h if blocks is not None else graph.to_original(h)
                    continue
            norm = None if last else (self.norms[i] if len(self.norms) else False)
            if (self.fuse_layers and norm is not False and (h.is_cuda or fused.FORCE)
                    and fused.can_fuse(self.convs[i], norm, self.activation, g, self.training, self.residual)):
                y_needed = True
                if not last and norm is not None:
                    nxt_last = i + 1 == self.n_layers - 1
                    nxt_norm = None if nxt_last else (self.norms[i + 1] if len(self.norms) else False)
                    nxt_g, rows = (graph, h.shape[0]) if blocks is None else (blocks[i + 1], g.number_of_dst_nodes())
                    y_needed = nxt_norm is False or not fused.halves_only_consumer(
                        self.convs[i + 1], nxt_norm, self.activation, nxt_g, self.training, self.residual, rows, h.is_cuda)
                h = fused.gat_hidden_layer(self.convs[i], norm, g, h, self.dropout.p, self.training, y_needed=y_needed)
                if last:
                    h = h.view(h.shape[0], self.convs[i]._num_heads, -1)
                else:
                    continue
            else:
                h = self.convs[i](g, h)
            if i < self.n_layers - 1:
                if self.residual and h_last is not None:
                    h = h + (h_last if blocks is None else h_last[:h.shape[0]])
                h_last = h
                h = h.flatten(1)
                if len(self.norms):
                    h = _epilogue(h, self.norms[i], self.activation, self.dropout, self.training)
                else:
                    h = self.dropout(self.activation(self.biases[i](h)))
        out = self.biases[-1](h.view(h.shape[0], -1) if h.shape[1] == 1 else h.mean(1))
        return out if blocks is not None else graph.to_original(out)
```

### bot_amd/nn/fused.py

```python
from __future__ import annotations

import os
from types import SimpleNamespace

import torch
import torch.nn as nn
import torch.nn.functional as F

from .. import _C, gemm, halo, side
from ..graph import take_rows
from ..ops import bn_epilogue_forward, bn_epilogue_sums, new_dropout_seed, stats_partials_for


ABSMAX_BYPRODUCT = os.environ.get("BOT_ABSMAX_BYPRODUCT", "1") != "0"
SKIP_Y = os.environ.get("BOT_SKIP_Y", "1") != "0"
HANDLES = 0
SKINNY = os.environ.get("BOT_SKINNY", "1") != "0"
FORCE = False
CALLS = 0
AGG_CALLS = 0
L0_CALLS = 0


def can_fuse(conv, norm, activation, graph, training, stack_residual) -> bool:
    epilogue_ok = norm is None or (isinstance(norm, nn.BatchNorm1d) and activation in (F.relu, torch.relu) and not stack_residual)
    return (epilogue_ok and hasattr(conv, "fc") and not (conv._use_symmetric_norm and graph.halo is not None)
            and conv._activation is None
            and not (training and (conv.edge_drop > 0 or conv.feat_drop.p > 0)) and conv._out_feats <= 256)


def sym_scales(graph):
    from . import _graph_cache, degree_norm
    c = _graph_cache(graph)
    if "sym_scales" not in c:
        csc = graph.csc
        s_out, s_in = degree_norm(graph, "out", -0.5), degree_norm(graph, "in", 0.5)
        deg = (csc.indptr[1:] - csc.indptr[:-1]).long()
        dst = torch.repeat_interleave(torch.arange(csc.n_rows, device=deg.device), deg)
        c["sym_scales"] = (s_out, (take_rows(s_out, csc.indices) * s_in[dst]).unsqueeze(1).contiguous())
    return c["sym_scales"]


def block_width(HD: int) -> int:
    return (HD + 3) // 4 * 4


def cat_weight(conv):
    H, D = conv._num_heads, conv._out_feats
    W = conv.fc.weight
    Wh = W.view(H, D, -1)
    gap = block_width(H * D) - H * D
    rows = [W] + ([W.new_zeros(gap, W.shape[1])] if gap else [])
    if conv.res_fc is not None:
        rows += [conv.res_fc.weight] + ([W.new_zeros(gap, W.shape[1])] if gap else [])
    rows.append((Wh * conv.attn_l.view(H, D, 1)).sum(1))
    if conv.attn_r is not None:
        rows.append((Wh * conv.attn_r.view(H, D, 1)).sum(1))
    used = sum(r.shape[0] for r in rows)
    pad = (-used) % 128
    if pad:
        rows.append(W.new_zeros(pad, W.shape[1]))
    return torch.cat(rows)


class _MergeWeight(torch.autograd.Function):

    @staticmethod
    def forward(ctx, W, Wres, attn_l, attn_r, H, D, with_fc):
        blk = block_width(H * D) if with_fc else H * D
        used = (blk if with_fc else 0) + (blk if Wres is not None else 0) + H + (H if attn_r is not None else 0)
        P = used + (-used) % 128
        ctx.save_for_backward(W, attn_l, attn_r)
        ctx.wres_ref = Wres
        ctx.cfg = (H, D, P, with_fc, Wres is not None, blk)
        return _C.merge_weight_fwd(W, Wres, attn_l.reshape(-1), None if attn_r is None else attn_r.reshape(-1), H, D, P, with_fc, block=blk)

    @staticmethod
    def backward(ctx, dm):
        W, attn_l, attn_r = ctx.saved_tensors
        H, D, P, with_fc, has_res, blk = ctx.cfg

        def body():
            return _C.merge_weight_bwd(W, attn_l.reshape(-1), None if attn_r is None else attn_r.reshape(-1), H, D, P, with_fc, has_res, dm, block=blk)
        if side.produced(dm):
            if with_fc and side.MERGE_ON_SIDE and side.usable(dm) and all(p is None or (p.grad is None and side.unhooked(p))
                                                                          for p in (W, ctx.wres_ref, attn_l, attn_r)):
                dW, dWres, dal, dar = side.run(body, dm, W, attn_l, attn_r)
            else:
                side.join()
                dW, dWres, dal, dar = body()
        else:
            dW, dWres, dal, dar = body()
        return dW, dWres, dal.view_as(attn_l), (None if dar is None else dar.view_as(attn_r)), None, None, None


def merged_weight(conv, with_fc=True):
    W = conv.fc.weight
    if W.is_cuda and WEIGHT_KP:
        return _MergeWeight.apply(W, conv.res_fc.weight if conv.res_fc is not None else None, conv.attn_l,
                                  conv.attn_r if isinstance(conv.attn_r, torch.Tensor) else None, conv._num_heads, conv._out_feats,
                                  with_fc)
    return _kp(cat_weight(conv) if with_fc else cat_weight_aggfirst(conv))


def _ext_width(HD, H):
    return HD + (H + 3) // 4 * 4


def _extend_forward(graph, out, HD, H, c):
    import torch.distributed as dist
    plan = graph.halo
    n_own = out.shape[0]
    W = _ext_width(HD, H)
    ext = torch.empty((n_own + plan.n_halo, W), dtype=out.dtype, device=out.device)
    ext[:n_own, :HD] = out[:, :HD]
    ext[:n_own, HD:HD + H] = out[:, c:c + H]
    if W > HD + H:
        ext[:n_own, HD + H:].zero_()
    send = _C.gather_rows(ext[:n_own], plan.send_rows) if plan.n_send else ext.new_empty((0, W))
    halo.a2a(ext[n_own:], send, plan.recv_splits, plan.send_splits, plan.group)
    return ext


def _extend_backward(graph, dext, n_own):
    import torch.distributed as dist
    plan = graph.halo
    back = torch.empty((plan.n_send, dext.shape[1]), dtype=dext.dtype, device=dext.device)
    halo.a2a(back, dext[n_own:], plan.send_splits, plan.recv_splits, plan.group)
    own = dext[:n_own]
    off = 0
    for cnt in plan.send_splits:
        if cnt:
            _C.scatter_add_rows(own, plan.send_rows[off:off + cnt], back[off:off + cnt])
        off += cnt
    return own


OVERLAP_CALLS = 0
_ship_rows, _return_rows, _fold_back = halo.ship_rows, halo.return_rows, halo.fold_back


def _epilogue_forward(x, bn, bn_w, bn_b, bn_training, drop_p, y_needed=True, partials=None):
    global HANDLES
    y, mean, invstd, epi = bn_epilogue_forward(x, bn, bn_w, bn_b, True, drop_p, bn_training, True, True, y_needed, partials)
    if gemm.is_handle(y):
        HANDLES += 1
    return y, mean, invstd, epi


def _finish_forward(ctx, x, bn, bn_w, bn_b, bn_training, drop_p, y_needed, partials=None, **keep):
    y, ctx.epi = x, None
    if bn is not None:
        y, mean, invstd, ctx.epi = _epilogue_forward(x, bn, bn_w, bn_b, bn_training, drop_p, y_needed, partials)
        keep.update(x=x, mean=mean, invstd=invstd, bn_w=bn_w, bn_b=bn_b)
    ctx.saved_names = tuple(keep)
    ctx.save_for_backward(*keep.values())
    return y


def _saved(ctx):
    return SimpleNamespace(**dict(zip(ctx.saved_names, ctx.saved_tensors)))


def _attn_backward(ctx, da, el, er, a):
    g = ctx.graph
    H, _, _, has_er, slope = ctx.cfg
    if ctx.sym:
        s_out, w_e = sym_scales(g)
        da = da * w_e
    dz, der = _C.gat_attn_bwd(g.csc, el, er, None, None, slope, H, a, da, None, None, has_er, ctx.zs, drop=ctx.adrop)
    d_el = _C.segment_sum(g.csr, dz, g.csr2csc)
    if ctx.sym:
        d_el = d_el * s_out.unsqueeze(1)
    return d_el, der


def _score_columns(dout, c, d_el, der=None):
    H = d_el.shape[1]
    dout[:, c:c + H] = d_el
    used = c + H
    if der is not None:
        nd = der.shape[0]
        dout[:nd, used:used + H] = der
        if nd < dout.shape[0]:
            dout[nd:, used:used + H].zero_()
        used += H
    if used < dout.shape[1]:
        dout[:, used:].zero_()
    return used


DOUT_DIRECT = os.environ.get("BOT_DOUT_DIRECT", "1") != "0"
DOUT_DIRECT_CALLS = 0
TAIL_CAP = 2.0 ** 20


def rowsum_bound(graph, attn_p: float) -> float:
    from . import _graph_cache
    c = _graph_cache(graph)
    if "max_out_deg" not in c:
        ip = graph.csr.indptr
        c["max_out_deg"] = int((ip[1:] - ip[:-1]).max()) if ip.numel() > 1 else 0
    return max(1.0, c["max_out_deg"] / (1.0 - attn_p))


def _dout_direct_ok(ctx, g, h, H, D, P, B, has_res, epi) -> bool:
    HD = H * D
    c = 2 * B
    return (DOUT_DIRECT and ctx.halves is not None and has_res and epi is not None and not ctx.overlap and g.halo is None and not ctx.sym
            and g.number_of_dst_nodes() == h.shape[0]
            and HD % 2 == 0 and H >= 2 and c % 32 == 0 and P % 64 == 0 and gemm.left_order(P) == 2
            and gemm.NT_KERNEL == "halves3" and gemm.TN_KERNEL == "halves3" and (ctx.halves[2] * P >= gemm.TN_MIN_OUT or gemm.FORCE or FORCE) and not epi.sync)


class _GATHidden(torch.autograd.Function):
    @staticmethod
    def forward(ctx, h, Wcat, bn_w, bn_b, graph, bn, H, D, has_res, has_er, slope, attn_p, drop_p, bn_training, kp, sym, y_needed=True):
        N, HD = graph.number_of_dst_nodes(), H * D
        csc = graph.csc
        ctx.cfg, ctx.graph = (H, D, has_res, has_er, slope), graph
        ctx.sym = sym
        ctx.kp = kp
        xh = None
        if gemm.enabled(h):
            xh = gemm.take(h, 0)
            ws = gemm.split_right(Wcat.t().contiguous() if kp else Wcat)
            ctx.wscale = ws.scale
            ctx.xscale = xh.scale
            out = gemm.mm_nt(xh, ws)
        else:
            out = torch.mm(h, Wcat) if kp else torch.mm(h, Wcat.t())
        ctx.halves = None if xh is None else (xh.n, xh.F, xh.piece, xh.order)
        ctx.bn_link = None if xh is None else xh.bn_link
        hk = h if xh is None else xh.buf
        B = block_width(HD)
        c = 2 * B if has_res else B
        ext = None
        ctx.overlap = halo.enabled(graph) and not sym
        if ctx.overlap:
            global OVERLAP_CALLS
            OVERLAP_CALLS += 1
            plan, sp = graph.halo, graph.halo_split
            el_own = out[:, c:c + H].contiguous()
            el_halo, _, _ = _ship_rows(plan, el_own)
            ft_halo, work, send_keep = _ship_rows(plan, out[:, :HD], async_op=True)
            el = torch.cat([el_own, el_halo])
            er = out[:, c + H:c + 2 * H].contiguous() if has_er else None
            ctx.zs = _C.zsign_buffer(csc, H, slope)
            ctx.adrop = (attn_p, new_dropout_seed(attn_p)) if attn_p > 0 else None
            a, a_d = _C.gat_attn_fwd(csc, el, er, None, None, None, slope, H, None, ctx.zs, drop=ctx.adrop or (0.0, 0))
            res = out[:, B:B + HD].unflatten(1, (H, D)) if has_res else None
            x3 = _C.spmm(sp["csc_own"], out[:, :HD].unflatten(1, (H, D)), a_d, sp["csc_own_pos"], addend=res)
            work.wait()
            del send_keep
            if sp["csc_halo"].nnz:
                _C.spmm(sp["csc_halo"], ft_halo.unflatten(1, (H, D)), a_d, sp["csc_halo_pos"], out=x3, addend=x3)
            return _finish_forward(ctx, x3.view(N, HD), bn, bn_w, bn_b, bn_training, drop_p, y_needed,
                                   h=hk, Wcat=Wcat, table=out, el=el, er=er, a=a, a_d=a_d, ft_halo=ft_halo)
        if graph.halo is not None:
            ext = _extend_forward(graph, out, HD, H, c)
            ft = ext[:, :HD].unflatten(1, (H, D))
            el = ext[:, HD:HD + H].contiguous()
        else:
            ft = out[:, :HD].unflatten(1, (H, D))
            el = out[:, c:c + H].contiguous()
        er = out[:N, c + H:c + 2 * H].contiguous() if has_er else None
        if sym:
            s_out, w_e = sym_scales(graph)
            el = el * s_out.unsqueeze(1)
        ctx.zs = _C.zsign_buffer(csc, H, slope)
        ctx.adrop = (attn_p, new_dropout_seed(attn_p)) if attn_p > 0 else None
        a, a_d = _C.gat_attn_fwd(csc, el, er, None, None, None, slope, H, None, ctx.zs, drop=ctx.adrop or (0.0, 0))
        if sym:
            a_d = a_d * w_e
        res = out[:N, B:B + HD].unflatten(1, (H, D)) if has_res else None
        if HD % 4 and bn is not None and sweep_is_row_kernel(graph, H, D):
            xbuf = torch.empty((N, (HD + 3) // 4 * 4), dtype=out.dtype, device=out.device)
            x = xbuf[:, :HD]
            _C.spmm(csc, ft, a_d, None, out=x.unflatten(1, (H, D)), addend=res)
        else:
            x = _C.spmm(csc, ft, a_d, None, addend=res).view(N, HD)
        return _finish_forward(ctx, x, bn, bn_w, bn_b, bn_training, drop_p, y_needed,
                               h=hk, Wcat=Wcat, table=ext if ext is not None else out, el=el, er=er, a=a, a_d=a_d)

    @staticmethod
    def backward(ctx, dy):
        H, D, has_res, has_er, slope = ctx.cfg
        g, epi, s = ctx.graph, ctx.epi, _saved(ctx)
        h, Wcat, table, el, er, a, a_d = s.h, s.Wcat, s.table, s.el, s.er, s.a, s.a_d
        dy = dy.contiguous()
        d_bn_w = d_bn_b = None
        kp = ctx.kp
        N, HD, P = h.shape[0], H * D, Wcat.shape[1 if kp else 0]
        Nd = g.number_of_dst_nodes()
        B = block_width(HD)
        if _dout_direct_ok(ctx, g, h, H, D, P, B, has_res, epi):
            out = _backward_direct(ctx, dy, s, P, B)
            if out is not None:
                return out
        dout = torch.empty((N, P), dtype=dy.dtype, device=h.device)
        dx = dout[:Nd, B:B + HD] if has_res else torch.empty((Nd, HD), dtype=dy.dtype, device=h.device)
        slots = None
        if B != HD:
            dout[:, HD:B].zero_()
            if has_res:
                dout[:, B + HD:2 * B].zero_()
        if has_res and Nd < N:
            dout[Nd:, B:B + HD].zero_()
        if epi is None:
            dx.copy_(dy)
        else:
            (sg, sgx), (d_bn_b, d_bn_w) = bn_epilogue_sums(epi, dy, s.x, s.mean, s.invstd, s.bn_w, s.bn_b, True, epi.bn_training and epi.sync)
            if ctx.halves is not None and has_res and not ctx.overlap and g.halo is None and ABSMAX_BYPRODUCT:
                slots = _C.absmax_slots(dy.device)
            _C.bn_act_bwd_apply(dy, s.x, s.mean, s.invstd, s.bn_w, s.bn_b, True, epi.drop_p, epi.seed, sg, sgx, epi.total, out=dx, absmax=slots)
        c = 2 * B if has_res else B
        ft, dx3 = table[:, :HD].unflatten(1, (H, D)), dx.unflatten(1, (H, D))
        if ctx.overlap:
            plan, sp = g.halo, g.halo_split
            da = torch.empty((g.csr.nnz, H), dtype=dy.dtype, device=h.device)
            dft_halo = torch.empty((plan.n_halo, HD), dtype=dy.dtype, device=h.device)
            if sp["csr_halo"].nnz:
                _C.spmm_dot(sp["csr_halo"], dx3, a_d, sp["csr_halo_c2c"], s.ft_halo.unflatten(1, (H, D)), out=dft_halo.unflatten(1, (H, D)), dot=da)
            elif plan.n_halo:
                dft_halo.zero_()
            back_ft, work = _return_rows(plan, dft_halo, async_op=True)
            _C.spmm_dot(sp["csr_own"], dx3, a_d, sp["csr_own_c2c"], ft, out=dout[:, :HD].unflatten(1, (H, D)), dot=da)
            d_el, der = _attn_backward(ctx, da, el, er, a)
            back_el, _ = _return_rows(plan, d_el[N:].contiguous())
            work.wait()
            _fold_back(plan, dout[:, :HD], back_ft)
            d_el = _fold_back(plan, d_el[:N].contiguous(), back_el)
        elif g.halo is not None:
            dext = torch.empty_like(table)
            _, da = _C.spmm_dot(g.csr, dx3, a_d, g.csr2csc, ft, out=dext[:, :HD].unflatten(1, (H, D)))
            d_el, der = _attn_backward(ctx, da, el, er, a)
            _score_columns(dext, HD, d_el)
            own = _extend_backward(g, dext, N)
            dout[:, :HD] = own[:, :HD]
            d_el = own[:, HD:HD + H]
        else:
            _, da = _C.spmm_dot(g.csr, dx3, a_d, g.csr2csc, ft, out=dout[:, :HD].unflatten(1, (H, D)), absmax=slots)
            d_el, der = _attn_backward(ctx, da, el, er, a)
        used = _score_columns(dout, c, d_el, der)
        dW = dh = None
        if ctx.halves is not None:
            xh = gemm.Halves(h, ctx.xscale, *ctx.halves)
            if slots is not None:
                _C.absmax_into(dout[:, c:used], slots)
                dh_ = gemm.split(dout, 0, scale=_C.halves_scale_from_slots(slots))
            else:
                dh_ = gemm.split(dout, 0)
            if ctx.needs_input_grad[0]:
                dh = gemm.mm_nt(dh_, gemm.split_right(Wcat if kp else Wcat.t().contiguous(), scale=ctx.wscale), link=ctx.bn_link)
            if ctx.needs_input_grad[1]:
                def wgrad():
                    dW = gemm.tn(xh, dh_)
                    return dW if kp else dW.t().contiguous()
                dW = side.run(wgrad, xh, dh_) if (side.usable(dout) and xh.piece * dh_.piece >= side.MIN_OUT) else wgrad()
        else:
            if ctx.needs_input_grad[1]:
                dW = torch.mm(h.t(), dout) if kp else torch.mm(dout.t(), h)
            if ctx.needs_input_grad[0]:
                dh = torch.mm(dout, Wcat.t()) if kp else torch.mm(dout, Wcat)
        return (dh, dW, d_bn_w if ctx.needs_input_grad[2] else None, d_bn_b if ctx.needs_input_grad[3] else None,
                None, None, None, None, None, None, None, None, None, None, None, None, None)


def _backward_direct(ctx, dy, s, P, B):
    global DOUT_DIRECT_CALLS
    H, D, _, has_er, _ = ctx.cfg
    g, epi, kp, h, Wcat = ctx.graph, ctx.epi, ctx.kp, s.h, s.Wcat
    N, HD = h.shape[0], H * D
    c = 2 * B
    used = c + (2 * H if has_er else H)
    piece = P
    buf = torch.empty((N, 2 * piece), dtype=torch.float16, device=h.device)
    dxb = torch.empty((N, B), dtype=dy.dtype, device=h.device)
    dx = dxb[:, :HD]
    ft = s.table[:, :HD].unflatten(1, (H, D))
    if not _C.spmm_dot_halves_fits(dx.unflatten(1, (H, D)), ft, buf, D, piece):
        return None
    DOUT_DIRECT_CALLS += 1
    slots = _C.absmax_slots(dy.device)
    (sg, sgx), (d_bn_b, d_bn_w) = bn_epilogue_sums(epi, dy, s.x, s.mean, s.invstd, s.bn_w, s.bn_b, True, epi.bn_training and epi.sync, slots)
    s1 = _C.halves_scale_from_slots(slots, mult=rowsum_bound(g, ctx.adrop[0] if ctx.adrop else 0.0))
    _C.bn_act_bwd_apply_halves(dy, s.x, s.mean, s.invstd, s.bn_w, s.bn_b, True, epi.drop_p, epi.seed, sg, sgx, epi.total,
                               s1, buf[:, B:], HD, HD, out=dx, h2_off=piece)
    da = _C.spmm_dot_halves(g.csr, dx.unflatten(1, (H, D)), s.a_d, g.csr2csc, ft, s1, buf, D, piece)
    d_el, der = _attn_backward(ctx, da, s.el, s.er, s.a)
    slots2 = _C.absmax_slots(dy.device)
    _C.absmax_into(d_el, slots2)
    if has_er:
        _C.absmax_into(der, slots2)
    s2 = _C.halves_scale_from_slots(slots2, cap=s1, cap_ratio=TAIL_CAP)
    segs = [(c, H, d_el)] + ([(c + H, H, der)] if has_er else [])
    if B != HD:
        segs += [(HD, B - HD, None), (B + HD, B - HD, None)]
    if used < P:
        segs.append((used, P - used, None))
    _C.halves_tail(segs, s2, buf, piece)
    dW = dh = None
    xh = gemm.Halves(h, ctx.xscale, *ctx.halves)
    if ctx.needs_input_grad[0]:
        Ws = gemm.split_right(Wcat if kp else Wcat.t().contiguous(), scale=ctx.wscale)
        link = ctx.bn_link
        st = link.stats_for(N, Ws.n, piece) if link is not None else None
        dh = _C.gemm_halves3_nt(buf, Ws.buf, s1, Ws.scale, piece, Ws.piece, piece, a2_off=piece, scale_a2=s2, k_split=c, b_frag=Ws.order == 3, n=Ws.n, bn=st)
        if st is not None:
            link.deliver(st, dh)
    if ctx.needs_input_grad[1]:
        def wgrad():
            dWk = _C.gemm_halves3_tn(xh.buf, buf, xh.scale, s1, xh.piece, piece, xh.F, P, x2_off=xh.h2_off, d2_off=piece, scale_d2=s2, p_split=c)
            return dWk if kp else dWk.t().contiguous()
        dW = side.run(wgrad, xh, buf, s1, s2) if (side.usable(buf) and xh.piece * piece >= side.MIN_OUT) else wgrad()
    return (dh, dW, d_bn_w if ctx.needs_input_grad[2] else None, d_bn_b if ctx.needs_input_grad[3] else None,
            None, None, None, None, None, None, None, None, None, None, None, None, None)


def cat_weight_aggfirst(conv):
    H, D = conv._num_heads, conv._out_feats
    W = conv.fc.weight
    Wh = W.view(H, D, -1)
    rows = [conv.res_fc.weight] if conv.res_fc is not None else []
    rows.append((Wh * conv.attn_l.view(H, D, 1)).sum(1))
    if conv.attn_r is not None:
        rows.append((Wh * conv.attn_r.view(H, D, 1)).sum(1))
    used = sum(r.shape[0] for r in rows)
    pad = (-used) % 128
    if pad:
        rows.append(W.new_zeros(pad, W.shape[1]))
    return torch.cat(rows)


WEIGHT_KP = True


def _kp(w):
    return w.t().contiguous() if WEIGHT_KP else w


AGG_FIRST = True


L0_HALVES = os.environ.get("BOT_L0_HALVES", "1") != "0"
L0_DIRECT = os.environ.get("BOT_L0_DIRECT", "1") != "0"
_L0_TABLES = {}
_L0_DH = {}


def _l0_dh(device, N, H, D, DP):
    key = (str(device), N, H, D, DP)
    buf = _L0_DH.get(key)
    if buf is None:
        buf = torch.zeros((N, 2 * H * DP), dtype=torch.float16, device=device)
        if not (buf.is_cuda and torch.cuda.is_current_stream_capturing()):
            _L0_DH[key] = buf
    return buf


def _l0_tables(H, D, Fin, P2, kp, N):
    key = (H, D, Fin, P2, kp, N)
    if key not in _L0_TABLES:
        FP = (Fin + 63) // 64 * 64
        DP = (D + 63) // 64 * 64
        HD = H * D
        fwd = [(h * D, D, 0, h * FP, 2 * FP // 32, h * D) for h in range(H)]
        dz = [(h * Fin, Fin, 0, h * DP, DP // 32, h * N * Fin) for h in range(H)]
        tn = []
        for h in range(H):
            for j in range((D + 127) // 128):
                pv = min(128, D - 128 * j)
                col = h * D + 128 * j
                tn.append((FP * (1 + h), Fin, h * DP + 128 * j, pv, col * Fin, Fin, 1))
                if kp:
                    tn.append((0, Fin, h * DP + 128 * j, pv, HD * Fin + col, P2, 0))
                else:
                    tn.append((0, Fin, h * DP + 128 * j, pv, HD * Fin + col * Fin, Fin, 1))
        _L0_TABLES[key] = (FP, DP, fwd, dz, tn)
    return _L0_TABLES[key]


def _l0_halves_ok(h, H, D, Fin, has_res, sym, attn_p, graph) -> bool:
    return (L0_HALVES and (h.is_cuda or FORCE) and has_res and not sym and attn_p <= 0.7 and D <= 256 and Fin <= 192 and H * 2 * ((D + 127) // 128) <= 16
            and gemm.MODE == "halves" and gemm.NT_KERNEL == "halves3" and gemm.TN_KERNEL == "halves3" and (h.shape[0] >= gemm.MIN_ROWS or gemm.FORCE or FORCE))


def _small_mm(a, b, b_is_kn, out):
    if a.is_cuda and SKINNY:
        return _C.skinny_gemm(a, b, b_is_kn=b_is_kn, out=out)
    out.copy_(a @ (b if b_is_kn else b.t()))
    return out


def use_agg_first(conv) -> bool:
    return AGG_FIRST and conv._in_src_feats <= conv._out_feats and conv._num_heads <= 4 and conv._in_src_feats <= 256


class _GATHiddenAggFirst(torch.autograd.Function):

    @staticmethod
    def forward(ctx, h, W, Wr, bn_w, bn_b, graph, bn, H, D, has_res, has_er, slope, attn_p, drop_p, bn_training, kp, sym, y_needed=True):
        N, Fin, HD = h.shape[0], h.shape[1], H * D
        Nd = graph.number_of_dst_nodes()
        csc = graph.csc
        ctx.cfg, ctx.graph = (H, D, has_res, has_er, slope), graph
        ctx.sym = sym
        ctx.kp = kp
        skinny = SKINNY and h.is_cuda and Fin <= 256 and N >= 4096
        l0h = _l0_halves_ok(h, H, D, Fin, has_res, sym, attn_p, graph) and not ctx.needs_input_grad[0]
        ctx.l0h = l0h
        if l0h:
            P2 = Wr.shape[1 if kp else 0]
            out2 = torch.empty((N, P2), dtype=h.dtype, device=h.device)
            _small_mm(h, Wr[:, HD:] if kp else Wr[HD:], kp, out2[:, HD:])
        elif skinny:
            out2 = _C.skinny_gemm(h, Wr, b_is_kn=kp, out=torch.empty((N, Wr.shape[1 if kp else 0]), dtype=h.dtype, device=h.device))
        else:
            out2 = torch.mm(h, Wr) if kp else torch.mm(h, Wr.t())
        ctx.skinny = skinny
        c = HD if has_res else 0
        ext = None
        if graph.halo is not None:
            import torch.distributed as dist
            plan = graph.halo
            Wd = _ext_width(Fin, H)
            ext = torch.empty((N + plan.n_halo, Wd), dtype=h.dtype, device=h.device)
            ext[:N, :Fin] = h
            ext[:N, Fin:Fin + H] = out2[:, c:c + H]
            if Wd > Fin + H:
                ext[:N, Fin + H:].zero_()
            send = _C.gather_rows(ext[:N], plan.send_rows) if plan.n_send else ext.new_empty((0, Wd))
            halo.a2a(ext[N:], send, plan.recv_splits, plan.send_splits, plan.group)
            xsrc = ext[:, :Fin]
            el = ext[:, Fin:Fin + H].contiguous()
        else:
            xsrc = h
            el = out2[:, c:c + H].contiguous()
        er = out2[:Nd, c + H:c + 2 * H].contiguous() if has_er else None
        if sym:
            s_out, w_e = sym_scales(graph)
            el = el * s_out.unsqueeze(1)
        ctx.zs = _C.zsign_buffer(csc, H, slope)
        ctx.adrop = (attn_p, new_dropout_seed(attn_p)) if attn_p > 0 else None
        a, a_d = _C.gat_attn_fwd(csc, el, er, None, None, None, slope, H, None, ctx.zs, drop=ctx.adrop or (0.0, 0))
        if sym:
            a_d = a_d * w_e
        if l0h:
            global L0_CALLS
            L0_CALLS += 1
            FP, DP, g_fwd, _, _ = _l0_tables(H, D, Fin, out2.shape[1], kp, Nd)
            KA = (1 + H) * FP
            xscale = _C.halves_scale(h) if ext is None else _C.halves_scale_from_slots(_C.absmax_into(xsrc, _C.absmax_slots(h.device)))
            A = torch.empty((Nd, 2 * KA), dtype=torch.float16, device=h.device)
            _C.halves_split_cols(h if Nd == N else h[:Nd], xscale, 2, A, KA, 0, FP)
            _C.spmm_bcast_halves(csc, xsrc, a_d, None, xscale, A, FP, FP, KA, FP)
            Wres = (Wr.t()[:HD] if kp else Wr[:HD]).contiguous()
            slots = _C.absmax_slots(h.device)
            _C.absmax_into(Wres, slots)
            _C.absmax_into(W, slots)
            wscale = _C.halves_scale_from_slots(slots)
            B = torch.empty((HD, 6 * FP), dtype=torch.float16, device=h.device)
            _C.halves_split_cols(Wres, wscale, 1, B, 2 * FP, 0, FP)
            _C.halves_split_cols(W, wscale, 1, B, 2 * FP, FP, FP)
            x = out2[:Nd, :HD]
            partials = None
            if bn is not None and h.is_cuda | FORCE:
                carries = int(_C._lib.bot_gemm_halves3_nt_bn_rows(2 * FP)) == 256
                partials = stats_partials_for(bn, bn_training, Nd, HD, h.device, carries and gemm.epilogue_piece(HD, x) is not None)
            _C.gemm_halves3_nt_grouped(A, B, xscale, wscale, KA, 2 * FP, out2, g_fwd, FP // 32, stats=partials)
            return _finish_forward(ctx, x, bn, bn_w, bn_b, bn_training, drop_p, y_needed, partials, h=h, W=W, Wr=Wr, z=A,
                                   table=ext if ext is not None else h, el=el, er=er, a=a, a_d=a_d, xscale=xscale)
        z = _C.spmm_bcast(csc, xsrc, a_d, None, head_outer=True)
        Wh = W.view(H, D, Fin)
        if has_res and skinny:
            _C.skinny_gemm(z, Wh, b_is_kn=False, out=out2, accumulate=True, batch=H, strides=(Nd * Fin, D * Fin, D), m=Nd, n=D, k=Fin)
            x = out2[:Nd, :HD]
        elif has_res:
            for i in range(H):
                out2[:Nd, i * D:(i + 1) * D].addmm_(z[i], Wh[i].t())
            x = out2[:Nd, :HD]
        elif skinny:
            agg = _C.skinny_gemm(z, Wh, b_is_kn=False, out=torch.empty((H, Nd, D), dtype=h.dtype, device=h.device), batch=H,
                                 strides=(Nd * Fin, D * Fin, Nd * D), m=Nd, n=D, k=Fin)
            x = agg.permute(1, 0, 2).reshape(Nd, HD)
        else:
            agg = torch.empty((H, Nd, D), dtype=h.dtype, device=h.device)
            for i in range(H):
                torch.mm(z[i], Wh[i].t(), out=agg[i])
            x = agg.permute(1, 0, 2).reshape(Nd, HD)
        return _finish_forward(ctx, x, bn, bn_w, bn_b, bn_training, drop_p, y_needed, h=h, W=W, Wr=Wr, z=z,
                               table=ext if ext is not None else h, el=el, er=er, a=a, a_d=a_d)

    @staticmethod
    def backward(ctx, dy):
        H, D, has_res, has_er, slope = ctx.cfg
        g, epi, s = ctx.graph, ctx.epi, _saved(ctx)
        h, W, Wr, z, table, el, er, a, a_d = s.h, s.W, s.Wr, s.z, s.table, s.el, s.er, s.a, s.a_d
        dy = dy.contiguous()
        d_bn_w = d_bn_b = None
        l0h, kp = ctx.l0h, ctx.kp
        N, Fin, HD, P2 = h.shape[0], h.shape[1], H * D, Wr.shape[1 if kp else 0]
        Nd = g.number_of_dst_nodes()
        dout2 = torch.empty((N, P2), dtype=h.dtype, device=h.device)
        dx = dout2[:Nd, :HD] if has_res else torch.empty((Nd, HD), dtype=h.dtype, device=h.device)
        if has_res and Nd < N:
            dout2[Nd:, :HD].zero_()
        direct = l0h and L0_DIRECT and epi is not None and D % 2 == 0
        slots = _C.absmax_slots(dy.device) if l0h and (ABSMAX_BYPRODUCT or direct) and epi is not None else None
        Dh = dscale = None
        if epi is None:
            dx.copy_(dy)
        else:
            (sg, sgx), (d_bn_b, d_bn_w) = bn_epilogue_sums(epi, dy, s.x, s.mean, s.invstd, s.bn_w, s.bn_b, True, epi.bn_training and epi.sync,
                                                           slots if direct else None)
            if direct:
                DP = (D + 63) // 64 * 64
                dscale = _C.halves_scale_from_slots(slots)
                Dh = _C.bn_act_bwd_apply_halves(dy, s.x, s.mean, s.invstd, s.bn_w, s.bn_b, True, epi.drop_p, epi.seed, sg, sgx, epi.total,
                                                dscale, _l0_dh(dy.device, Nd, H, D, DP), D, DP)
            else:
                _C.bn_act_bwd_apply(dy, s.x, s.mean, s.invstd, s.bn_w, s.bn_b, True, epi.drop_p, epi.seed, sg, sgx, epi.total, out=dx, absmax=slots)
        Wh = W.view(H, D, Fin)
        dz = torch.empty((H, Nd, Fin), dtype=h.dtype, device=h.device)
        dW3 = torch.empty((H, D, Fin), dtype=h.dtype, device=h.device) if ctx.needs_input_grad[1] and not l0h else None
        if l0h:
            FP, DP, _, g_dz, t_tn = _l0_tables(H, D, Fin, P2, kp, Nd)
            if Dh is None:
                dscale = _C.halves_scale_from_slots(slots) if slots is not None else _C.halves_scale(dx)
                Dh = _C.halves_split_heads(dx, dscale, H, D, DP)
            Wt = gemm.split(Wh.transpose(1, 2).reshape(H * Fin, D), 1)
            _C.gemm_halves3_nt_grouped(Dh, Wt.buf, dscale, Wt.scale, H * DP, Wt.piece, dz[0], g_dz, 0)
            flat = torch.empty(HD * Fin + P2 * Fin, dtype=h.dtype, device=h.device)

            def wgrad():
                _C.gemm_halves3_tn_grouped(z, Dh, s.xscale, dscale, (1 + H) * FP, H * DP, flat, t_tn)
                return flat
            if side.usable(flat):
                side.run(wgrad, z, Dh, s.xscale, dscale, flat)
            else:
                wgrad()
        elif ctx.skinny and D <= 256:
            _C.skinny_gemm(dx, Wh, b_is_kn=True, out=dz, batch=H, strides=(D, D * Fin, Nd * Fin), m=Nd, n=Fin, k=D)
        if ctx.skinny and dW3 is not None:
            _C.tn_gemm(dx, z, out=dW3, batch=H, strides=(D, Nd * Fin, 0), n=Nd, kx=D, ky=Fin)
        for i in range(H if not l0h else 0):
            dxi = dx[:, i * D:(i + 1) * D]
            if not (ctx.skinny and D <= 256):
                torch.mm(dxi, Wh[i], out=dz[i])
            if dW3 is not None and not ctx.skinny:
                torch.mm(dxi.t(), z[i], out=dW3[i])
        dW = dW3.view(HD, Fin) if dW3 is not None else None
        halo = g.halo is not None
        c = HD if has_res else 0
        need_dh = ctx.needs_input_grad[0]
        if not need_dh:
            xsrc = table[:, :Fin] if halo else h
            da = _C.sddmm_dot_bcast(g.csc, xsrc, dz)
            dh_g = None
        elif halo:
            dext = torch.empty_like(table)
            _, da = _C.spmm_dot_bcast(g.csr, dz, a_d, g.csr2csc, table[:, :Fin], out=dext[:, :Fin])
        else:
            dh_g, da = _C.spmm_dot_bcast(g.csr, dz, a_d, g.csr2csc, h)
        d_el, der = _attn_backward(ctx, da, el, er, a)
        if halo and not need_dh:
            dsm = d_el.new_zeros((d_el.shape[0], (H + 3) // 4 * 4))
            dsm[:, :H] = d_el
            d_el = _extend_backward(g, dsm, N)[:, :H]
        elif halo:
            _score_columns(dext, Fin, d_el)
            own = _extend_backward(g, dext, N)
            dh_g, d_el = own[:, :Fin], own[:, Fin:Fin + H]
        _score_columns(dout2, c, d_el, der)
        dWr = None
        if l0h:
            dW = flat[:HD * Fin].view(HD, Fin)
            dWr = flat[HD * Fin:].view((Fin, P2) if kp else (P2, Fin))
            tail = dout2[:, HD:]
            if h.is_cuda and tail.shape[1] <= 32:
                _C.tn_narrow(tail, h, dWr[:, HD:] if kp else dWr[HD:], transpose_out=kp)
            elif h.is_cuda:
                _C.tn_gemm(tail, h, out=dWr[:, HD:] if kp else dWr[HD:], transpose_out=kp)
            elif kp:
                dWr[:, HD:] = h.t() @ tail
            else:
                dWr[HD:] = tail.t() @ h
            side.join()
            if not ctx.needs_input_grad[1]:
                dW = None
            if not ctx.needs_input_grad[2]:
                dWr = None
        elif ctx.needs_input_grad[2]:
            dWr = torch.mm(h.t(), dout2) if kp else torch.mm(dout2.t(), h)
        dh = None
        if need_dh:
            dh = torch.addmm(dh_g, dout2, Wr.t() if kp else Wr)
        return (dh, dW, dWr, d_bn_w if ctx.needs_input_grad[3] else None, d_bn_b if ctx.needs_input_grad[4] else None,
                None, None, None, None, None, None, None, None, None, None, None, None, None)


def halves_only_consumer(conv, norm, activation, graph, training, stack_residual, n_rows, on_device) -> bool:
    return (SKIP_Y and (on_device or FORCE) and can_fuse(conv, norm, activation, graph, training, stack_residual) and not use_agg_first(conv)
            and gemm.MODE == "halves" and (gemm.FORCE or (on_device and n_rows >= gemm.MIN_ROWS)))


_INPUT_DROPPED = [False]


class input_already_dropped:

    def __init__(self, on=True):
        self.on = bool(on)

    def __enter__(self):
        _INPUT_DROPPED[0] = self.on
        return self

    def __exit__(self, *exc):
        _INPUT_DROPPED[0] = False
        return False


def take_input_dropped() -> bool:
    v = _INPUT_DROPPED[0]
    _INPUT_DROPPED[0] = False
    return v


def gat_hidden_layer(conv, bn, graph, h, dropout_p, training, y_needed=True):
    from . import has_zero_in_degree
    if not conv._allow_zero_in_degree:
        assert not has_zero_in_degree(graph), "0-in-degree nodes (models.py:477-479)"
    global CALLS
    CALLS += 1
    H, D = conv._num_heads, conv._out_feats
    attn_p = conv.attn_drop.p if training else 0.0
    bn_w = bn.weight if bn is not None and bn.affine else None
    bn_b = bn.bias if bn is not None and bn.affine else None
    bn_training = bn is not None and (bn.training or not bn.track_running_stats)
    if use_agg_first(conv):
        global AGG_CALLS
        AGG_CALLS += 1
        return _GATHiddenAggFirst.apply(h, conv.fc.weight, merged_weight(conv, with_fc=False), bn_w, bn_b, graph, bn, H, D,
                                        conv.res_fc is not None, conv.attn_r is not None, conv.leaky_relu.negative_slope,
                                        attn_p, dropout_p if training and bn is not None else 0.0, bn_training, WEIGHT_KP,
                                        conv._use_symmetric_norm, y_needed)
    if bn is None:
        return _GATHidden.apply(h, merged_weight(conv), None, None, graph, None, H, D, conv.res_fc is not None,
                                conv.attn_r is not None, conv.leaky_relu.negative_slope, attn_p, 0.0, False, WEIGHT_KP,
                                conv._use_symmetric_norm)
    return _GATHidden.apply(h, merged_weight(conv), bn.weight if bn.affine else None, bn.bias if bn.affine else None, graph, bn,
                            H, D, conv.res_fc is not None, conv.attn_r is not None, conv.leaky_relu.negative_slope,
                            conv.attn_drop.p if training else 0.0, dropout_p if training else 0.0, bn_training, WEIGHT_KP,
                            conv._use_symmetric_norm, y_needed)



_GENERATION = [0]


def bump_generation():
    _GENERATION[0] += 1


def _versions(*ts):
    return (_GENERATION[0],) + tuple((t.data_ptr(), t._version) for t in ts if t is not None)


def _cached(owner, slot, key, make):
    c = owner.__dict__.setdefault("_bot_infer_cache", {})
    hit = c.get(slot)
    if hit is None or hit[0] != key:
        hit = c[slot] = (key, make())
    return hit[1]


def _infer_key(conv):
    return _versions(conv.fc.weight, conv.res_fc.weight if conv.res_fc is not None else None, conv.attn_l, conv.attn_r) + (WEIGHT_KP,)


def infer_weight(conv):
    return _cached(conv, "wcat", _infer_key(conv), lambda: merged_weight(conv).detach())


def eval_affine(mod):
    if isinstance(mod, nn.BatchNorm1d):
        key = _versions(mod.weight, mod.bias, mod.running_mean, mod.running_var)

        def make():
            scale = torch.rsqrt(mod.running_var + mod.eps)
            if mod.affine:
                scale = scale * mod.weight
            shift = -mod.running_mean * scale
            if mod.affine:
                shift = shift + mod.bias
            return scale.contiguous(), shift.contiguous()
        return _cached(mod, "affine", key, make)
    return (mod.weight.detach() if mod.weight is not None else None), (mod.bias.detach() if mod.bias is not None else None)


def sweep_is_row_kernel(graph, H, D) -> bool:
    from .. import blocked
    csc = graph.csc
    return not csc.indptr.is_cuda or blocked.plan_for(csc, graph.number_of_nodes(), H, D) is None


def can_infer(conv, epi, activation, graph, stack_residual, last) -> bool:
    if torch.is_grad_enabled() or not hasattr(conv, "fc") or conv._activation is not None or conv.training:
        return False
    if isinstance(epi, nn.BatchNorm1d):
        if epi.training or not epi.track_running_stats or epi.running_mean is None:
            return False
    elif not (type(epi).__name__ == "ElementWiseLinear" and not epi.inplace):
        return False
    if not last and (activation not in (F.relu, torch.relu) or stack_residual):
        return False
    if last and conv._num_heads != 1:
        return False
    return (not (conv._use_symmetric_norm and graph.halo is not None)
            and conv._out_feats <= 256 and sweep_is_row_kernel(graph, conv._num_heads, conv._out_feats))


class _LabelReuse:
    active = None


class label_reuse:
    def __init__(self, static_cols):
        self.static_cols, self.store = int(static_cols), {}

    def __enter__(self):
        self.prev, _LabelReuse.active = _LabelReuse.active, self
        return self

    def __exit__(self, *exc):
        _LabelReuse.active = self.prev
        self.store.clear()
        return False


INFER_CALLS = 0


def count_infer():
    global INFER_CALLS
    INFER_CALLS += 1


L0_INFER = os.environ.get("BOT_L0_INFER", "1") != "0"
L0_INFER_CALLS = 0


L0_INFER_OVER_LABEL_REUSE = os.environ.get("BOT_L0_INFER_LABEL_REUSE", "1") != "0"


def _infer_l0_ok(conv, graph, h, label_reuse_cols) -> bool:
    return (L0_INFER and L0_HALVES and use_agg_first(conv) and (not label_reuse_cols or L0_INFER_OVER_LABEL_REUSE) and graph.halo is None
            and conv.res_fc is not None
            and not conv._use_symmetric_norm and conv._out_feats <= 256 and h.shape[1] <= 192 and (h.is_cuda or FORCE)
            and gemm.MODE == "halves" and gemm.NT_KERNEL == "halves3" and (h.shape[0] >= gemm.MIN_ROWS or gemm.FORCE or FORCE))


def _infer_l0(conv, epi, graph, h, relu):
    global L0_INFER_CALLS
    L0_INFER_CALLS += 1
    H, D = conv._num_heads, conv._out_feats
    HD, N, Fin = H * D, graph.number_of_dst_nodes(), h.shape[1]
    has_er = conv.attn_r is not None
    csc = graph.csc
    Wr = _cached(conv, "wcat_agg", _infer_key(conv), lambda: merged_weight(conv, with_fc=False).detach())
    kp = WEIGHT_KP
    P2 = Wr.shape[1 if kp else 0]
    FP, _, g_fwd, _, _ = _l0_tables(H, D, Fin, P2, kp, N)
    KA = (1 + H) * FP

    def right_operand():
        Wres = (Wr.t()[:HD] if kp else Wr[:HD]).contiguous()
        W = conv.fc.weight.detach()
        slots = _C.absmax_slots(h.device)
        _C.absmax_into(Wres, slots)
        _C.absmax_into(W, slots)
        wscale = _C.halves_scale_from_slots(slots)
        B = torch.empty((HD, 6 * FP), dtype=torch.float16, device=h.device)
        _C.halves_split_cols(Wres, wscale, 1, B, 2 * FP, 0, FP)
        _C.halves_split_cols(W, wscale, 1, B, 2 * FP, FP, FP)
        return B, wscale
    B, wscale = _cached(conv, "infer_l0_halves", _infer_key(conv) + (str(h.device),), right_operand)
    tail = torch.empty((h.shape[0], P2 - HD), dtype=h.dtype, device=h.device)
    _small_mm(h, Wr[:, HD:] if kp else Wr[HD:], kp, tail)
    el = tail[:, :H]
    er = tail[:N, H:2 * H] if has_er else None
    a = _C.gat_attn_fwd(csc, el, er, None, None, None, conv.leaky_relu.negative_slope, H, None)
    xscale = _C.halves_scale(h)
    A = torch.empty((N, 2 * KA), dtype=torch.float16, device=h.device)
    _C.halves_split_cols(h if N == h.shape[0] else h[:N], xscale, 2, A, KA, 0, FP)
    _C.spmm_bcast_halves(csc, h, a, None, xscale, A, FP, FP, KA, FP)
    scale, shift = eval_affine(epi)
    y = torch.empty((N, HD), dtype=h.dtype, device=h.device)
    slots = _C.absmax_slots(h.device) if (relu and ABSMAX_BYPRODUCT and gemm.enabled(h)) else None
    _C.gemm_halves3_nt_grouped(A, B, xscale, wscale, KA, 2 * FP, y, g_fwd, FP // 32, col_scale=scale, col_shift=shift, relu=relu, absmax=slots)
    if slots is not None:
        gemm.stash_scale(y, _C.halves_scale_from_slots(slots))
    return y


@torch.no_grad()
def gat_infer_layer(conv, epi, graph, h, relu, first=False):
# ... 47 lines not shown
```

### include/bot_gnn.h

```cpp
#ifndef BOT_GNN_H
#define BOT_GNN_H

#include <stdint.h>

#ifdef __cplusplus
extern "C" {
#endif

#define BOT_ABI_VERSION 19

#define BOT_E_NULL (-1)
#define BOT_E_RANGE (-2)
#define BOT_E_ALIGN (-3)
#define BOT_E_PLAN (-4)

typedef void* bot_stream_t;

int bot_abi_version(void);
const char* bot_last_error(void);
int bot_stream_create(int32_t high_priority, bot_stream_t* out);
const char* bot_last_kernel(void);
int bot_debug_abort_trace(const char* path_host);

int bot_row_plan_size_host(const int32_t* indptr_host, int64_t n_rows, int32_t chunk,
                           int64_t* n_items, int64_t* n_long, int64_t* n_slots);
int bot_row_plan_fill_host(const int32_t* indptr_host, int64_t n_rows, int32_t chunk,
                           int32_t* items_host , int32_t* long_rows_host ,
                           int32_t* long_ptr_host );
int32_t bot_row_plan_default_chunk(int64_t nnz);

int bot_degrees_i64(const int32_t* indptr, int64_t n_rows, int64_t* deg, bot_stream_t stream);

int64_t bot_spmm_workspace_floats(int64_t n_slots, int32_t H, int32_t D);
int bot_spmm_set_layout(int32_t layout);
int bot_spmm_f32(const int32_t* indptr, const int32_t* indices, int64_t n_rows, int64_t nnz,
                 const int32_t* items, int64_t n_items,
                 const int32_t* long_rows, const int32_t* long_ptr, int64_t n_long,
                 const float* x, int64_t ldx, int64_t hsx,
                 const float* w, const int32_t* wperm,
                 int32_t H, int32_t D,
                 float* out, int64_t ldo, int64_t hso,
                 const float* addend, int64_t lda, int64_t hsa,
                 float* partial, bot_stream_t stream);

int bot_spmm_blocked_f32(const int32_t* tile_rows, const int32_t* ptr, const int32_t* b_src, const uint8_t* b_lrow,
                         const int32_t* b_pos, int32_t n_tiles, int32_t nblk, int32_t block_rows, int32_t T, int32_t epi,
                         int32_t round_tiles, const float* x, int64_t ldx, const float* w, int32_t H, int32_t D, float* out,
                         int64_t ldo, const float* addend, int64_t lda, bot_stream_t stream);


int bot_spmm_dot_f32(const int32_t* indptr, const int32_t* indices, int64_t n_rows, int64_t nnz,
                     const int32_t* items, int64_t n_items,
                     const int32_t* long_rows, const int32_t* long_ptr, int64_t n_long,
                     const float* x, int64_t ldx, int64_t hsx,
                     const float* w, const int32_t* wperm,
                     const float* y, int64_t ldy, int64_t hsy,
                     int32_t H, int32_t D,
                     float* out, int64_t ldo, int64_t hso,
                     float* dot_out, float* partial, uint32_t* absmax_slots, bot_stream_t stream);

int bot_spmm_bcast_f32(const int32_t* indptr, const int32_t* indices, int64_t n_rows, int64_t nnz,
                       const int32_t* items, int64_t n_items,
                       const int32_t* long_rows, const int32_t* long_ptr, int64_t n_long,
                       const float* x, int64_t ldx, const float* w, const int32_t* wperm,
                       int32_t H, int32_t D, float* out, int64_t ldo, int64_t hso,
                       float* partial, bot_stream_t stream);
int bot_spmm_bcast_halves_f16(const int32_t* indptr, const int32_t* indices, int64_t n_rows, int64_t nnz,
                              const int32_t* items, int64_t n_items,
                              const int32_t* long_rows, const int32_t* long_ptr, int64_t n_long,
                              const float* x, int64_t ldx, const float* w, const int32_t* wperm,
                              int32_t H, int32_t D, const float* hscale, uint16_t* hout, int64_t ldh, int64_t hsh, int32_t h2_off,
                              int32_t hpiece, float* partial, bot_stream_t stream);
int bot_spmm_dot_bcast_f32(const int32_t* indptr, const int32_t* indices, int64_t n_rows, int64_t nnz,
                           const int32_t* items, int64_t n_items,
                           const int32_t* long_rows, const int32_t* long_ptr, int64_t n_long,
                           const float* x, int64_t ldx, int64_t hsx, const float* w, const int32_t* wperm,
                           const float* y, int64_t ldy, int32_t H, int32_t D,
                           float* out, int64_t ldo, float* dot_out, float* partial, bot_stream_t stream);

int bot_sddmm_dot_f32(const int32_t* indptr, const int32_t* indices, int64_t n_rows, int64_t nnz,
                      const int32_t* items, int64_t n_items,
                      const float* x, int64_t ldx, int64_t hsx,
                      const float* y, int64_t ldy, int64_t hsy,
                      int32_t H, int32_t D,
                      float* out, const int32_t* operm, int32_t accumulate, bot_stream_t stream);

int bot_sddmm_dot_bcast_f32(const int32_t* indptr, const int32_t* indices, int64_t n_rows, int64_t nnz,
                            const int32_t* items, int64_t n_items,
                            const float* x, int64_t ldx,
                            const float* y, int64_t ldy, int64_t hsy,
                            int32_t H, int32_t D,
                            float* out, const int32_t* operm, bot_stream_t stream);

int bot_sddmm_u_add_v_f32(const int32_t* src, const int32_t* dst, int64_t n_edges,
                          const float* x, const float* y, int32_t W, float* out, bot_stream_t stream);

int bot_gat_attn_fwd_f32(const int32_t* indptr, const int32_t* indices, int64_t n_rows, int64_t nnz,
                         const int32_t* long_rows, int64_t n_long, int32_t chunk,
                         const float* el, const float* er, const float* ee, const int32_t* eperm,
                         const uint8_t* keep, float slope, int32_t H,
                         float* a, const int32_t* aperm, uint8_t* zsign,
                         float attn_drop, uint64_t drop_seed, const uint64_t* seed_offset, float* a_drop,
                         bot_stream_t stream);

int bot_gat_attn_bwd_f32(const int32_t* indptr, const int32_t* indices, int64_t n_rows, int64_t nnz,
                         const int32_t* long_rows, int64_t n_long, int32_t chunk,
                         const float* el, const float* er, const float* ee, const int32_t* eperm,
                         float slope, int32_t H,
                         const float* a, const float* da, const int32_t* aperm,
                         float* dz, const int32_t* zperm, float* der, const uint8_t* zsign,
                         float attn_drop, uint64_t drop_seed, const uint64_t* seed_offset, bot_stream_t stream);

int64_t bot_gat_infer_workspace_floats(int64_t n_slots, int32_t H, int32_t D);
int bot_gat_infer_f32(const int32_t* indptr, const int32_t* indices, int64_t n_rows, int64_t nnz,
                      const int32_t* items, int64_t n_items,
                      const int32_t* long_rows, const int32_t* long_ptr, int64_t n_long, int64_t n_slots,
                      const float* x, int64_t ldx, int64_t hsx,
                      const float* el, int64_t ldel, const float* er, int64_t lder,
                      const float* ee, const float* ew, float slope, int32_t H, int32_t D,
                      const float* addend, int64_t lda, int64_t hsa,
                      const float* scale, const float* shift, int32_t relu,
                      float* out, int64_t ldo, int64_t hso,
                      float* workspace, uint32_t* absmax_slots , bot_stream_t stream);

int bot_segment_sum_f32(const int32_t* indptr, int64_t n_rows, int64_t nnz,
                        const int32_t* long_rows, int64_t n_long, int32_t chunk,
                        const float* vals, const int32_t* perm, int32_t W,
                        float* out, bot_stream_t stream);

int bot_gather_rows_f32(const float* x, int64_t ldx, const int32_t* rows, int64_t n_sel, int32_t F,
                        float* out, int64_t ldo, bot_stream_t stream);
int bot_scatter_add_rows_f32(float* x, int64_t ldx, const int32_t* rows, int64_t n_sel, int32_t F,
                             const float* vals, int64_t ldv, bot_stream_t stream);

int64_t bot_bn_workspace_floats(int32_t F);
int bot_colstats_f32(const float* x, int64_t ldx, int64_t n, int32_t F, float* mean, float* m2, float* workspace,
                     bot_stream_t stream);
int bot_colsum_f32(const float* x, int64_t ldx, int64_t n, int32_t F, float* sum, float* workspace, bot_stream_t stream);
int bot_bn_stats_f32(const float* x, int64_t ldx, int64_t n, int32_t F, float eps, float momentum, float* mean, float* invstd,
                     float* running_mean, float* running_var, int64_t* num_batches_tracked, float* workspace,
                     bot_stream_t stream);
int bot_bn_act_fwd_f32(const float* x, int64_t ldx, int64_t n, int32_t F, const float* mean, const float* invstd,
                       const float* weight, const float* bias, int32_t relu, float p, uint64_t seed,
                       const uint64_t* seed_offset, float* y, int64_t ldy, bot_stream_t stream);
int bot_bn_stats_halves_f32(const float* x, int64_t ldx, int64_t n, int32_t F, float eps, float momentum, float* mean, float* invstd,
                            float* running_mean, float* running_var, int64_t* num_batches_tracked, const float* weight,
                            const float* bias, float p, float* hscale, float* workspace, bot_stream_t stream);
int bot_bn_act_fwd_halves_f32(const float* x, int64_t ldx, int64_t n, int32_t F, const float* mean, const float* invstd,
                              const float* weight, const float* bias, int32_t relu, float p, uint64_t seed,
                              const uint64_t* seed_offset, float* y, int64_t ldy, const float* hscale, uint16_t* hout, int64_t ldh,
                              int32_t piece, int32_t pieces, bot_stream_t stream);
int bot_bn_act_bwd_reduce_f32(const float* dy, int64_t lddy, const float* x, int64_t ldx, int64_t n, int32_t F,
                              const float* mean, const float* invstd, const float* weight, const float* bias,
                              int32_t relu, float p, uint64_t seed, const uint64_t* seed_offset, float* sum_g, float* sum_gx,
                              float* workspace, bot_stream_t stream);
int bot_bn_act_bwd_apply_f32(const float* dy, int64_t lddy, const float* x, int64_t ldx, int64_t n, int32_t F,
                             const float* mean, const float* invstd, const float* weight, const float* bias,
                             int32_t relu, float p, uint64_t seed, const uint64_t* seed_offset, const float* sum_g,
                             const float* sum_gx, double total_count, float* dx, int64_t lddx, uint32_t* absmax_slots , bot_stream_t stream);
int bot_bn_act_bwd_reduce_max_f32(const float* dy, int64_t lddy, const float* x, int64_t ldx, int64_t n, int32_t F,
                                  const float* mean, const float* invstd, const float* weight, const float* bias,
                                  int32_t relu, float p, uint64_t seed, const uint64_t* seed_offset, float* sum_g, float* sum_gx,
                                  float* workspace, bot_stream_t stream);
int bot_bn_bwd_bound_f32(int32_t F, int64_t n, const float* workspace, const float* sum_g, const float* sum_gx, double total_count,
                         const float* weight, const float* invstd, uint32_t* absmax_slots, bot_stream_t stream);
int bot_bn_act_bwd_apply_halves_f32(const float* dy, int64_t lddy, const float* x, int64_t ldx, int64_t n, int32_t F,
                                    const float* mean, const float* invstd, const float* weight, const float* bias,
                                    int32_t relu, float p, uint64_t seed, const uint64_t* seed_offset, const float* sum_g,
                                    const float* sum_gx, double total_count, float* dx, int64_t lddx, const float* hscale, uint16_t* hout,
                                    int64_t ldh, int32_t h2_off, int32_t hD, int32_t hDP, bot_stream_t stream);

int bot_merge_weight_fwd_f32(const float* W, const float* Wres, const float* attn_l, const float* attn_r, int32_t H, int32_t D,
                             int32_t K, int32_t P, int32_t with_fc, int32_t block, float* merged, bot_stream_t stream);
int bot_merge_weight_bwd_f32(const float* W, const float* attn_l, const float* attn_r, int32_t H, int32_t D, int32_t K,
                             int32_t P, int32_t with_fc, int32_t block, const float* d_merged, float* dW, float* dWres,
                             float* d_attn_l, float* d_attn_r, bot_stream_t stream);

int64_t bot_edge_mlp_workspace_floats(void);
int bot_edge_mlp_fwd_f32(const float* ef, int32_t I, const float* W1, const float* b1, int32_t J, const float* W2,
                         int32_t H, int64_t n_edges, float* ee, bot_stream_t stream);
int bot_edge_mlp_bwd_f32(const float* ef, int32_t I, const float* W1, const float* b1, int32_t J, const float* W2,
                         int32_t H, const float* dz, int64_t n_edges, float* dW1, float* db1, float* dW2,
                         float* workspace, bot_stream_t stream);

int64_t bot_random_keep_workspace_bytes(void);
int bot_random_keep_u8(int64_t n, int64_t n_keep, uint64_t seed, uint8_t* keep, void* workspace, bot_stream_t stream);

int bot_sample_neighbors_count_i32(const int32_t* indptr, int64_t n_rows, const int32_t* seeds, int64_t n_seeds, int32_t k, int32_t* counts,
                                   bot_stream_t stream);
int bot_sample_neighbors_i32(const int32_t* indptr, int64_t n_rows, const int32_t* seeds, int64_t n_seeds, int32_t k, uint64_t seed,
                             const int64_t* offsets, int32_t* out, bot_stream_t stream);
int64_t bot_block_tiles(int64_t n_nodes);
int bot_block_mark_i32(const int32_t* seeds, int64_t n_seeds, const int32_t* indices, const int32_t* pos, int64_t n_pos, int32_t* map,
                       int64_t n_nodes, int64_t* tile_counts, int64_t* n_new, bot_stream_t stream);
int bot_block_relabel_i32(const int32_t* seeds, int64_t n_seeds, const int32_t* indices, const int32_t* eid, const int32_t* pos, int64_t n_pos,
                          int32_t* map, int64_t n_nodes, const int64_t* tile_offsets, int64_t n_src, int32_t* src_nid, int32_t* local,
                          int32_t* parent_eid, bot_stream_t stream);

int bot_subgraph_mark_i32(const int32_t* nodes, int64_t n, int32_t* map, int64_t n_nodes, int64_t* n_dup, bot_stream_t stream);
int bot_subgraph_count_i32(const int32_t* indptr, const int32_t* indices, int64_t n_rows, const int32_t* nodes, int64_t n, const int32_t* map,
                           int32_t* counts, bot_stream_t stream);
int bot_subgraph_fill_i32(const int32_t* indptr, const int32_t* indices, const int32_t* eid, int64_t n_rows, const int32_t* nodes, int64_t n,
                          const int32_t* map, const int64_t* offsets, int32_t* local_src, int32_t* parent_eid, bot_stream_t stream);
int bot_subgraph_unmark_i32(const int32_t* nodes, int64_t n, int32_t* map, int64_t n_nodes, bot_stream_t stream);

int bot_sample_weights_prepare_f32(const int32_t* indptr, const int32_t* eid, int64_t n_rows, int64_t n_edges, const float* w,
                                   uint64_t* prefix, int32_t* n_pos, int32_t* flag, bot_stream_t stream);
int bot_sample_neighbors_weighted_count_i32(const int32_t* n_pos, int64_t n_rows, const int32_t* seeds, int64_t n_seeds, int32_t k,
                                            int32_t* counts, bot_stream_t stream);
int bot_sample_neighbors_weighted_i32(const int32_t* indptr, const uint64_t* prefix, const int32_t* n_pos, int64_t n_rows, const int32_t* seeds,
                                      int64_t n_seeds, int32_t k, uint64_t seed, const int64_t* offsets, int32_t* out, bot_stream_t stream);

int64_t bot_halves_workspace_floats(void);
int bot_halves_scale_f32(const float* x, int64_t ldx, int64_t n, int32_t F, float* scale, float* workspace, bot_stream_t stream);
int32_t bot_absmax_slots(void);
int bot_absmax_slots_f32(const float* x, int64_t ldx, int64_t n, int32_t F, uint32_t* slots, bot_stream_t stream);
int bot_halves_scale_from_slots_f32(const uint32_t* slots, float* scale, bot_stream_t stream);
int bot_halves_split_f16(const float* x, int64_t ldx, int64_t n, int32_t F, const float* scale, int32_t order, uint16_t* out,
                         int64_t ldo, int32_t piece, bot_stream_t stream);
int bot_halves_split_cols_f16(const float* x, int64_t ldx, int64_t n, int32_t F, const float* scale, int32_t order, uint16_t* out,
                              int64_t ldo, int32_t piece, int32_t width, bot_stream_t stream);
int bot_halves_split_heads_f16(const float* x, int64_t ldx, int64_t n, int32_t H, int32_t D, const float* scale, uint16_t* out, int64_t ldo,
                               int32_t h2_off, int32_t DP, bot_stream_t stream);
int bot_halves_tn_combine_f32(const float* a, const float* b, int32_t chunks, int32_t K, int32_t PP, int32_t P, const float* rem_a,
                              const float* rem_b, float* out, int64_t ldo, bot_stream_t stream);
int bot_gemm_halves_f32(int32_t trans_a, int32_t trans_b, int64_t m, int64_t n, int64_t k, const float* alpha, const uint16_t* A,
                        int64_t lda, const uint16_t* B, int64_t ldb, float* C, int64_t ldc, int32_t batch, int64_t stride_a,
                        int64_t stride_b, int64_t stride_c, float beta, void* workspace, int64_t workspace_bytes, int32_t tune,
                        int32_t algo_index, bot_stream_t stream);
int bot_gemm_halves3_nt_f32(int64_t m, int64_t n, int64_t k, const float* scale_a, const float* scale_b, const uint16_t* A, int64_t lda,
                            int64_t a2_off, const uint16_t* B, int64_t ldb, int64_t b2_off, float* C, int64_t ldc, int32_t mode,
                            bot_stream_t stream);
int64_t bot_gemm_halves3_tn_workspace_floats(int64_t n_rows, int64_t kp, int64_t pp);
int bot_gemm_halves3_tn_f32(int64_t n_rows, int64_t k, int64_t p, int64_t kp, int64_t pp, const float* scale_x, const float* scale_d,
                            const uint16_t* X, int64_t ldx, int64_t x2_off, const uint16_t* D, int64_t ldd, int64_t d2_off, float* out,
                            int64_t ldo, float* workspace, int32_t mode, bot_stream_t stream);

int bot_halves_scale_from_slots2_f32(const uint32_t* slots, float mult, const float* cap_scale, float cap_ratio, float* scale, bot_stream_t stream);
int bot_halves_tail_f16(int64_t n, int32_t n_seg, const int64_t* seg_cols, const float* const* srcs, const int64_t* src_ld, const float* scale, uint16_t* out,
                        int64_t ldo, int32_t h2_off, bot_stream_t stream);
int bot_spmm_dot_halves_fits(const float* x, int64_t ldx, int64_t hsx, const float* y, int64_t ldy, int64_t hsy, int32_t H, int32_t D, const uint16_t* hout,
                             int64_t ldh, int64_t hsh, int32_t h2_off);
int bot_spmm_dot_halves_f16(const int32_t* indptr, const int32_t* indices, int64_t n_rows, int64_t nnz, const int32_t* items, int64_t n_items,
                            const int32_t* long_rows, const int32_t* long_ptr, int64_t n_long, const float* x, int64_t ldx, int64_t hsx, const float* w,
                            const int32_t* wperm, const float* y, int64_t ldy, int64_t hsy, int32_t H, int32_t D, const float* hscale, uint16_t* hout,
                            int64_t ldh, int64_t hsh, int32_t h2_off, float* dot_out, float* partial, bot_stream_t stream);
int bot_gemm_halves3_nt2_f32(int64_t m, int64_t n, int64_t k, const float* scale_a, const float* scale_a2, int64_t k_split, const float* scale_b,
                             const uint16_t* A, int64_t lda, int64_t a2_off, const uint16_t* B, int64_t ldb, int64_t b2_off, int32_t b_layout, float* C,
                             int64_t ldc, int32_t mode, bot_stream_t stream);
typedef struct bot_bn_bwd_stats {
    const float* x;
    int64_t ldx;
    const float* mean;
    const float* invstd;
    const float* weight;
    const float* bias;
    int32_t relu;
    float p;
    uint64_t seed;
    const uint64_t* seed_offset;
    float* part;
    float* pmax;
} bot_bn_bwd_stats_t;
int32_t bot_gemm_halves3_nt_bn_rows(int64_t k);
int bot_gemm_halves3_nt3_f32(int64_t m, int64_t n, int64_t k, const float* scale_a, const float* scale_a2, int64_t k_split, const float* scale_b,
                             const uint16_t* A, int64_t lda, int64_t a2_off, const uint16_t* B, int64_t ldb, int64_t b2_off, int32_t b_layout, float* C,
                             int64_t ldc, const bot_bn_bwd_stats_t* bn, int32_t mode, bot_stream_t stream);
int bot_bn_act_bwd_reduce_partials_f32(const float* part, int32_t nblk, int32_t F, float* sum_g, float* sum_gx, bot_stream_t stream);
int bot_bn_bwd_bound_partials_f32(int32_t F, const float* pmax, int32_t nblk, const float* sum_g, const float* sum_gx, double total_count,
                                  const float* weight, const float* invstd, uint32_t* absmax_slots, bot_stream_t stream);
int bot_bn_bwd_partials_finish_f32(const float* part, const float* pmax, int32_t nblk, int32_t F, float* sum_g, float* sum_gx, int32_t batch_stats,
                                   double total_count, const float* weight, const float* invstd, uint32_t* absmax_slots, bot_stream_t stream);
int bot_halves_split_frag_f16(const float* x, int64_t ldx, int64_t n, int32_t F, const float* scale, uint16_t* out, int32_t piece, bot_stream_t stream);
int bot_gemm_halves3_tn2_f32(int64_t n_rows, int64_t k, int64_t p, int64_t kp, int64_t pp, const float* scale_x, const float* scale_d, const float* scale_d2,
                             int64_t p_split, const uint16_t* X, int64_t ldx, int64_t x2_off, const uint16_t* D, int64_t ldd, int64_t d2_off, float* out,
                             int64_t ldo, float* workspace, int32_t mode, bot_stream_t stream);

int bot_gemm_halves3_nt_grouped_f32(int64_t m, int64_t b_rows, const float* scale_a, const float* scale_b, const uint16_t* A, int64_t lda,
                                    int64_t a2_off, const uint16_t* B, int64_t ldb, int64_t b2_off, float* C, int64_t ldc, int32_t n_groups,
                                    const int64_t* groups, int32_t k_seg, const float* col_scale, const float* col_shift, int32_t relu,
                                    uint32_t* absmax_slots, int32_t mode, bot_stream_t stream);
int bot_gemm_halves3_nt_grouped2_f32(int64_t m, int64_t b_rows, const float* scale_a, const float* scale_b, const uint16_t* A, int64_t lda,
                                     int64_t a2_off, const uint16_t* B, int64_t ldb, int64_t b2_off, float* C, int64_t ldc, int32_t n_groups,
                                     const int64_t* groups, int32_t k_seg, const float* col_scale, const float* col_shift, int32_t relu,
                                     uint32_t* absmax_slots, float* stats_part, float* stats_minmax, float* stats_pivot, int32_t stats_F,
                                     int32_t mode, bot_stream_t stream);
int bot_bn_stats_halves_partials_f32(const float* part, const float* minmax, int32_t nblk, const float* pivot, int64_t n, int32_t F, float eps, float momentum,
                                     float* mean, float* invstd, float* running_mean, float* running_var, int64_t* num_batches_tracked,
                                     const float* weight, const float* bias, float p, float* hscale, float* bound_workspace, bot_stream_t stream);
int64_t bot_gemm_halves3_tn_grouped_workspace_floats(int64_t n_rows, int32_t n_tiles);
int bot_gemm_halves3_tn_grouped_f32(int64_t n_rows, const float* scale_x, const float* scale_d, const uint16_t* X, int64_t ldx, int64_t x2_off,
                                    const uint16_t* D, int64_t ldd, int64_t d2_off, float* out, int32_t n_tiles, const int64_t* tiles,
                                    float* workspace, int32_t mode, bot_stream_t stream);

int bot_label_split_f32(const int64_t* train_idx, int64_t n_train, const int64_t* labels, int64_t ldl, const uint8_t* mask, float mask_rate,
                        uint64_t seed, const uint64_t* seed_offset, int32_t use_labels, int32_t* code, float* wn, float* count, int32_t* workspace,
                        bot_stream_t stream);
int bot_build_input_f32(const float* feat, int64_t ldf, int64_t n, int32_t F, int32_t C, const int32_t* code, float p, uint64_t seed,
                        const uint64_t* seed_offset, float* out, int64_t ldo, bot_stream_t stream);
int bot_build_input_reuse_f32(const float* feat, int64_t ldf, int64_t n, int32_t F, int32_t C, const int32_t* code, const uint8_t* reuse,
                              const float* pred, int64_t ldp, float p, uint64_t seed, const uint64_t* seed_offset, float* out, int64_t ldo,
                              bot_stream_t stream);
int bot_node_loss_f32(const float* x, int64_t ldx, int64_t n, int32_t C, const int64_t* labels, int64_t ldl, const float* wn, const float* count,
                      int32_t kind, float eps, float* y, int64_t n_pad, float* dx, int64_t lddx, bot_stream_t stream);
int bot_rmsprop_step_f32(int32_t n_tensors, float* const* params, const float* const* grads, float* const* square_avg, const int64_t* numel,
                         float lr, const float* lr_dev, float alpha, float eps, float weight_decay, bot_stream_t stream);

int bot_gemm_halves_last_algo(int32_t* index, float* ms);
int bot_gemm_halves_library_version(int32_t* compiled, int32_t* runtime);

int bot_skinny_gemm_f32(const float* A, int64_t lda, const float* B, int64_t ldb, int32_t b_is_kn, float* C, int64_t ldc, int64_t m,
                        int32_t n, int32_t k, int32_t accumulate, int32_t batch, int64_t stride_a, int64_t stride_b, int64_t stride_c,
                        bot_stream_t stream);

int64_t bot_tn_narrow_workspace_floats(int64_t n, int32_t kx, int32_t ky);
int bot_tn_narrow_f32(const float* X, int64_t ldx, const float* Y, int64_t ldy, int64_t n, int32_t kx, int32_t ky, float* out, int64_t ldo,
                      int32_t transpose_out, float* workspace, bot_stream_t stream);
int64_t bot_tn_gemm_workspace_floats(int64_t n, int32_t kx, int32_t ky, int32_t batch);
int bot_tn_gemm_f32(const float* X, int64_t ldx, const float* Y, int64_t ldy, int64_t n, int32_t kx, int32_t ky, float* out, int64_t ldo,
                    int32_t transpose_out, int32_t batch, int64_t stride_x, int64_t stride_y, int64_t stride_out, float* workspace,
                    bot_stream_t stream);

#ifdef __cplusplus
}
#endif
#endif
```

Baseline: 235.6 million.

## Pack all layers' merged weights and fp16 halves splits in batched stack kernels

Adds a per-stack weight pack that, once per parameter version, merges fc/residual/attention weights and produces the fp16 hi/lo split operands for the forward and backward GEMMs for up to eight layers in two batched launches. The merge kernel also tracks absmax so the split kernel can derive its scale without a separate reduction pass. Forward and backward then reuse these packed buffers instead of rebuilding and splitting the weights per layer per call. This adds cache-keying logic on parameter versions and capture ids, plus a runtime check that raises if the pack is refilled between a forward and its backward.

```diff
diff --git a/bot_amd/_C.py b/bot_amd/_C.py
--- a/bot_amd/_C.py
+++ b/bot_amd/_C.py
@@ -60,6 +60,13 @@
     "bot_scatter_add_rows_f32": (ctypes.c_int, [_P, c_int64, _P, c_int64, c_int32, _P, c_int64, _P]),
     "bot_merge_weight_fwd_f32": (ctypes.c_int, [_P, _P, _P, _P, c_int32, c_int32, c_int32, c_int32, c_int32, c_int32, _P, _P]),
     "bot_merge_weight_bwd_f32": (ctypes.c_int, [_P, _P, _P, c_int32, c_int32, c_int32, c_int32, c_int32, c_int32, _P, _P, _P, _P, _P, _P]),
+    "bot_weight_pack_blocks": (c_int32, [c_int32, c_int32, c_int32, c_int32, c_int32]),
+    "bot_weight_pack_merge_f32": (ctypes.c_int, [_P, _P, _P, _P, c_int32, c_int32, c_int32, c_int32, c_int32, c_int32, _P, _P, _P]),
+    "bot_weight_pack_split_f16": (ctypes.c_int, [_P, c_int32, c_int32, _P, c_int32, _P, _P, _P, _P]),
+    "bot_weight_pack_split_aggfirst_f16": (ctypes.c_int, [_P, _P, c_int32, c_int32, c_int32, _P, c_int32, _P, _P, _P, _P, _P]),
+    "bot_weight_pack_stack_width": (c_int32, []),
+    "bot_weight_pack_stack_f16": (ctypes.c_int, [c_int32, _P, _P]),
+    "bot_stream_capture_id": (c_int64, [_P]),
     "bot_edge_mlp_workspace_floats": (c_int64, []),
     "bot_edge_mlp_fwd_f32": (ctypes.c_int, [_P, c_int32, _P, _P, c_int32, _P, c_int32, c_int64, _P, _P]),
     "bot_edge_mlp_bwd_f32": (ctypes.c_int, [_P, c_int32, _P, _P, c_int32, _P, c_int32, _P, c_int64, _P, _P, _P, _P, _P]),
@@ -1065,6 +1072,7 @@
         if lr_dev is not None and (lr_dev.dtype != torch.float32 or lr_dev.device != ps[0].device):
             raise BotKernelError("rmsprop_step: a tensor learning rate must be float32 on the parameters' device")
         _check(_lib.bot_rmsprop_step_f32(k, P, G, S, Nn, float(lr), _ptr(lr_dev), float(alpha), float(eps), float(weight_decay), _stream()), "rmsprop_step")
+        _written(*ps, *sq)
 
 
 def skinny_gemm(a, b, *, b_is_kn, out, accumulate=False, batch=1, strides=(0, 0, 0), m=None, n=None, k=None, ldc=None):
@@ -1433,3 +1441,69 @@
     _check(_lib.bot_merge_weight_bwd_f32(W.data_ptr(), al.data_ptr(), _ptr(ar), H, D, K, P, int(with_fc), block, dm.data_ptr(), dW.data_ptr(),
                                          _ptr(dWres), dal.data_ptr(), _ptr(dar), _stream()), "merge_weight_bwd")
     return dW, dWres, dal, dar
+
+
+PACK_LAUNCHES = 0
+
+
+def capture_id() -> int:
+    return int(_lib.bot_stream_capture_id(_stream()))
+
+
+def weight_pack_buffers(H, D, K, P, with_fc, has_res, block, device):
+    n_part = int(_lib.bot_weight_pack_blocks(K, P, int(with_fc), int(has_res), block))
+    if n_part < 1:
+        raise BotKernelError(f"weight_pack: no grid for K={K} P={P} block={block}")
+    f32, f16 = dict(dtype=torch.float32, device=device), dict(dtype=torch.float16, device=device)
+    b = {"merged": torch.empty((K, P), **f32), "part": torch.empty(2 * n_part, **f32), "n_part": n_part}
+    if with_fc:
+        piece = (K + 63) // 64 * 64
+        b.update(scale=torch.empty(2, **f32), fwd=torch.empty((2 * (P // 16) * (piece // 32), 512), **f16),
+                 bwd=torch.empty((2 * ((K + 15) // 16) * (P // 32), 512), **f16))
+    else:
+        FP, DP = (K + 63) // 64 * 64, (D + 63) // 64 * 64
+        b.update(scale_b=torch.empty(2, **f32), scale_t=torch.empty(2, **f32), B=torch.empty((H * D, 6 * FP), **f16),
+                 Wt=torch.empty((H * K, 3 * DP), **f16))
+    return b
+
+
+def _weight_pack_args(b, W, Wres, attn_l, attn_r, H, D, P, with_fc):
+    _dev(W, Wres, attn_l, attn_r, b["merged"])
+    for t in (W, Wres, attn_l, attn_r):
+        if t is not None and (t.dtype != torch.float32 or not t.is_contiguous()):
+            raise BotKernelError("weight_pack: contiguous float32 parameters only")
+    K = W.shape[1]
+    if W.shape[0] != H * D or b["merged"].shape != (K, P) or (Wres is not None and Wres.shape != W.shape):
+        raise BotKernelError(f"weight_pack: W {tuple(W.shape)} for H={H} D={D}, buffers for {tuple(b['merged'].shape)}")
+    if not with_fc and Wres is None:
+        raise BotKernelError("weight_pack: the aggregate-first form needs the residual weight")
+    return K
+
+
+def weight_pack_fill(b, W, Wres, attn_l, attn_r, H, D, P, with_fc, block):
+    global PACK_LAUNCHES
+    K = _weight_pack_args(b, W, Wres, attn_l, attn_r, H, D, P, with_fc)
+    _check(_lib.bot_weight_pack_merge_f32(W.data_ptr(), _ptr(Wres), attn_l.data_ptr(), _ptr(attn_r), H, D, K, P, int(with_fc), int(block),
+                                          b["merged"].data_ptr(), b["part"].data_ptr(), _stream()), "weight_pack_merge")
+    if with_fc:
+        _check(_lib.bot_weight_pack_split_f16(b["merged"].data_ptr(), K, P, b["part"].data_ptr(), b["n_part"], b["scale"].data_ptr(), b["fwd"].data_ptr(),
+                                              b["bwd"].data_ptr(), _stream()), "weight_pack_split")
+    else:
+        _check(_lib.bot_weight_pack_split_aggfirst_f16(W.data_ptr(), Wres.data_ptr(), H, D, K, b["part"].data_ptr(), b["n_part"], b["scale_b"].data_ptr(),
+                                                       b["scale_t"].data_ptr(), b["B"].data_ptr(), b["Wt"].data_ptr(), _stream()), "weight_pack_split_aggfirst")
+    PACK_LAUNCHES += 2
+    return b
+
+
+def weight_pack_fill_stack(layers):
+    global PACK_LAUNCHES
+    width = int(_lib.bot_weight_pack_stack_width())
+    for i in range(0, len(layers), 8):
+        rows = []
+        for (b, W, Wres, attn_l, attn_r, H, D, P, with_fc, block) in layers[i:i + 8]:
+            K = _weight_pack_args(b, W, Wres, attn_l, attn_r, H, D, P, with_fc)
+            outs = (b["scale"], b["fwd"], b["bwd"], None) if with_fc else (b["scale_b"], b["B"], b["Wt"], b["scale_t"])
+            rows.append([W.data_ptr(), _ptr(Wres) or 0, attn_l.data_ptr(), _ptr(attn_r) or 0, H, D, K, P, int(with_fc), int(block), b["merged"].data_ptr(),
+                         b["part"].data_ptr(), b["n_part"]] + [(_ptr(t) or 0) for t in outs])
+        _check(_lib.bot_weight_pack_stack_f16(len(rows), _table(rows, width), _stream()), "weight_pack_stack")
+        PACK_LAUNCHES += 2
diff --git a/bot_amd/csrc/common.h b/bot_amd/csrc/common.h
--- a/bot_amd/csrc/common.h
+++ b/bot_amd/csrc/common.h
@@ -156,6 +156,16 @@
         if (bits > __hip_atomic_load(p, __ATOMIC_RELAXED, __HIP_MEMORY_SCOPE_AGENT)) atomicMax(p, bits);
     }
 }
+__device__ __forceinline__ float halves_scale_of(float m) {
+    float s = 1.f;
+    if (m > 0.f && m < INFINITY) {
+        int e;
+        const float f = frexpf(m, &e);
+        if (f == 0.5f) e -= 1;
+        s = ldexpf(1.f, min(60, 14 - e));
+    }
+    return s;
+}
 #endif
 void launch_absmax_slots(const float* x, int64_t ldx, int64_t n, int32_t F, uint32_t* slots, hipStream_t st);
 
diff --git a/bot_amd/csrc/halves.hip b/bot_amd/csrc/halves.hip
--- a/bot_amd/csrc/halves.hip
+++ b/bot_amd/csrc/halves.hip
@@ -51,13 +51,7 @@
 #pragma unroll
     for (int o = 32; o > 0; o >>= 1) m = fmaxf(m, __shfl_xor(m, o));
     if (threadIdx.x == 0) {
-        float s = 1.f;
-        if (m > 0.f && m < INFINITY) {
-            int e;
-            const float f = frexpf(m, &e);
-            if (f == 0.5f) e -= 1;
-            s = ldexpf(1.f, min(60, 14 - e));
-        }
+        const float s = halves_scale_of(m);
         scale[0] = s;
         scale[1] = 1.f / s;
     }
diff --git a/bot_amd/csrc/merge.hip b/bot_amd/csrc/merge.hip
--- a/bot_amd/csrc/merge.hip
+++ b/bot_amd/csrc/merge.hip
@@ -1,3 +1,5 @@
+#include <hip/hip_fp16.h>
+
 #include "common.h"
 
 namespace bot {
@@ -17,12 +19,12 @@
     float* dar;
 };
 
-__global__ __launch_bounds__(kBlock) void merge_fwd_kernel(MergeArgs a, int n_tiles, int tiles_k) {
-    __shared__ float tile[32][33];
+template <bool TRACK>
+__device__ __forceinline__ void merge_fwd_body(const MergeArgs& a, int n_tiles, int tiles_k, int block, float (*tile)[33], float& vmax, float& wmax) {
     const int HD = a.H * a.D;
     const int c0 = a.with_fc ? a.blk : 0, c1 = c0 + (a.Wres ? a.blk : 0), c2 = c1 + a.H, c3 = c2 + (a.ar ? a.H : 0);
-    if ((int)blockIdx.x < n_tiles) {
-        const int tk = blockIdx.x % tiles_k, tp = blockIdx.x / tiles_k;
+    if (block < n_tiles) {
+        const int tk = block % tiles_k, tp = block / tiles_k;
         const int tx = threadIdx.x & 31, ty = threadIdx.x >> 5;
 #pragma unroll
         for (int j = 0; j < 32; j += 8) {
@@ -34,6 +36,7 @@
                 if (q < HD) v = (a.with_fc && first) ? a.W[(int64_t)q * a.K + k] : a.Wres[(int64_t)q * a.K + k];
             }
             tile[ty + j][tx] = v;
+            if (TRACK) vmax = fmaxf(vmax, fabsf(v));
         }
         __syncthreads();
 #pragma unroll
@@ -43,7 +46,7 @@
         }
         return;
     }
-    const int64_t gid = (int64_t)(blockIdx.x - n_tiles) * kBlock + threadIdx.x;
+    const int64_t gid = (int64_t)(block - n_tiles) * kBlock + threadIdx.x;
     const int nq = a.P - c1;
     if (gid >= (int64_t)nq * a.K) return;
     const int q = (int)(gid / a.K), k = (int)(gid - (int64_t)q * a.K), p = c1 + q;
@@ -60,13 +63,196 @@
             float w[8];
 #pragma unroll
             for (int t = 0; t < 8; ++t) w[t] = wc[(int64_t)(d + t) * a.K];
+            if (TRACK) {
+#pragma unroll
+                for (int t = 0; t < 8; ++t) wmax = fmaxf(wmax, fabsf(w[t]));
+            }
             s0 = fmaf(w[0], ah[d], s0), s1 = fmaf(w[1], ah[d + 1], s1), s2 = fmaf(w[2], ah[d + 2], s2), s3 = fmaf(w[3], ah[d + 3], s3);
             s0 = fmaf(w[4], ah[d + 4], s0), s1 = fmaf(w[5], ah[d + 5], s1), s2 = fmaf(w[6], ah[d + 6], s2), s3 = fmaf(w[7], ah[d + 7], s3);
         }
-        for (; d < a.D; ++d) s0 = fmaf(wc[(int64_t)d * a.K], ah[d], s0);
+        for (; d < a.D; ++d) {
+            const float w = wc[(int64_t)d * a.K];
+            if (TRACK) wmax = fmaxf(wmax, fabsf(w));
+            s0 = fmaf(w, ah[d], s0);
+        }
         v = (s0 + s1) + (s2 + s3);
     }
+    if (TRACK) vmax = fmaxf(vmax, fabsf(v));
     a.out[(int64_t)k * a.P + p] = v;
+}
+
+__global__ __launch_bounds__(kBlock) void merge_fwd_kernel(MergeArgs a, int n_tiles, int tiles_k) {
+    __shared__ float tile[32][33];
+    float vmax = 0.f, wmax = 0.f;
+    merge_fwd_body<false>(a, n_tiles, tiles_k, (int)blockIdx.x, tile, vmax, wmax);
+}
+
+__device__ __forceinline__ void pack_merge_block(const MergeArgs& a, int n_tiles, int tiles_k, int block, int n_blocks, float* part, float (*tile)[33],
+                                                 float (*red)[kBlock / kWave]) {
+    float vmax = 0.f, wmax = 0.f;
+    merge_fwd_body<true>(a, n_tiles, tiles_k, block, tile, vmax, wmax);
+    if (!a.with_fc && block >= n_tiles) vmax = 0.f;
+    vmax = wave_absmax(vmax), wmax = wave_absmax(wmax);
+    if ((threadIdx.x & 63) == 0) red[0][threadIdx.x >> 6] = vmax, red[1][threadIdx.x >> 6] = wmax;
+    __syncthreads();
+    if (threadIdx.x == 0) {
+        for (int w = 1; w < kBlock / kWave; ++w) vmax = fmaxf(vmax, red[0][w]), wmax = fmaxf(wmax, red[1][w]);
+        part[block] = vmax;
+        part[n_blocks + block] = wmax;
+    }
+}
+
+__global__ __launch_bounds__(kBlock) void pack_merge_kernel(MergeArgs a, int n_tiles, int tiles_k, float* part) {
+    __shared__ float tile[32][33];
+    __shared__ float red[2][kBlock / kWave];
+    pack_merge_block(a, n_tiles, tiles_k, (int)blockIdx.x, (int)gridDim.x, part, tile, red);
+}
+
+__device__ __forceinline__ float pack_max(const float* part, int n, float* red) {
+    float m = 0.f;
+    for (int i = threadIdx.x; i < n; i += kBlock) m = fmaxf(m, part[i]);
+    m = wave_absmax(m);
+    __syncthreads();
+    if ((threadIdx.x & 63) == 0) red[threadIdx.x >> 6] = m;
+    __syncthreads();
+    return fmaxf(fmaxf(red[0], red[1]), fmaxf(red[2], red[3]));
+}
+
+__device__ __forceinline__ void pack_halves(float v0, float v1, __half2& h1, __half2& h2) {
+    const __half a0 = __float2half_rn(v0), a1 = __float2half_rn(v1);
+    const float r0 = v0 - __half2float(a0), r1 = v1 - __half2float(a1);
+    h1 = __halves2half2(a0, a1);
+    h2 = __halves2half2(__float2half_rn(r0), __float2half_rn(r1));
+}
+
+struct PackSplit {
+    const float* Wm;
+    const float* W;
+    const float* Wres;
+    const float* part;
+    float* scale;
+    float* scale_t;
+    __half* fwd;
+    __half* bwd;
+    int64_t region_f, region_b;
+    int H, D, K, P, n_part, tiles_k, FP, DP, with_fc;
+};
+
+__device__ __forceinline__ void pack_split_block(const PackSplit& a, int block, float (*tile)[33], float* red) {
+    const float* Wm = a.Wm;
+    const int K = a.K, P = a.P, tiles_k = a.tiles_k;
+    __half* fwd = a.fwd;
+    __half* bwd = a.bwd;
+    const int64_t region_f = a.region_f, region_b = a.region_b;
+    const float s = halves_scale_of(pack_max(a.part, a.n_part, red));
+    if (block == 0 && threadIdx.x == 0) a.scale[0] = s, a.scale[1] = 1.f / s;
+    const int tk = block % tiles_k, tp = block / tiles_k;
+    const int tx = threadIdx.x & 31, ty = threadIdx.x >> 5;
+#pragma unroll
+    for (int j = 0; j < 32; j += 8) {
+        const int k = tk * 32 + ty + j, p = tp * 32 + tx;
+        tile[ty + j][tx] = k < K ? Wm[(int64_t)k * P + p] * s : 0.f;
+    }
+    __syncthreads();
+    const int tiles_p = P >> 5, rows_b = (K + 15) >> 4;
+#pragma unroll
+    for (int it = 0; it < 2; ++it) {
+        const int rem = threadIdx.x, l = rem >> 2, j = (rem & 3) * 2;
+        const int rr = 16 * it + (l & 15), cc = 8 * (l >> 4) + j;
+        __half2 h1, h2;
+        pack_halves(tile[cc][rr], tile[cc + 1][rr], h1, h2);
+        int64_t o = ((int64_t)(tp * 2 + it) * tiles_k + tk) * 512 + l * 8 + j;
+        *reinterpret_cast<__half2*>(fwd + o) = h1;
+        *reinterpret_cast<__half2*>(fwd + region_f + o) = h2;
+        if (tk * 2 + it < rows_b) {
+            pack_halves(tile[rr][cc], tile[rr][cc + 1], h1, h2);
+            o = ((int64_t)(tk * 2 + it) * tiles_p + tp) * 512 + l * 8 + j;
+            *reinterpret_cast<__half2*>(bwd + o) = h1;
+            *reinterpret_cast<__half2*>(bwd + region_b + o) = h2;
+        }
+    }
+}
+
+__global__ __launch_bounds__(kBlock) void pack_split_kernel(PackSplit a) {
+    __shared__ float tile[32][33];
+    __shared__ float red[kBlock / kWave];
+    pack_split_block(a, (int)blockIdx.x, tile, red);
+}
+
+__device__ __forceinline__ void pack_split_aggfirst_block(const PackSplit& a, int block, float* red) {
+    const float* W = a.W;
+    const float* Wres = a.Wres;
+    const int H = a.H, D = a.D, Fin = a.K, FP = a.FP, DP = a.DP;
+    __half* B = a.fwd;
+    __half* Wt = a.bwd;
+    const float mw = pack_max(a.part + a.n_part, a.n_part, red);
+    const float sb = halves_scale_of(fmaxf(pack_max(a.part, a.n_part, red), mw)), st = halves_scale_of(mw);
+    if (block == 0 && threadIdx.x == 0) a.scale[0] = sb, a.scale[1] = 1.f / sb, a.scale_t[0] = st, a.scale_t[1] = 1.f / st;
+    const int64_t gid = (int64_t)block * kBlock + threadIdx.x;
+    const int64_t nb = (int64_t)H * D * FP;
+    float v0 = 0.f, v1 = 0.f;
+    __half* o;
+    int piece;
+    if (gid < nb) {
+        const int j = (int)(gid / FP), c = (int)(gid - (int64_t)j * FP) * 2;
+        const float* src = (c < FP ? Wres : W) + (int64_t)j * Fin;
+        const int f = c < FP ? c : c - FP;
+        if (f < Fin) v0 = src[f] * sb;
+        if (f + 1 < Fin) v1 = src[f + 1] * sb;
+        piece = 2 * FP;
+        o = B + (int64_t)j * 6 * FP + c;
+    } else {
+        const int64_t g = gid - nb;
+        const int half = DP >> 1;
+        if (g >= (int64_t)H * Fin * half) return;
+        const int r = (int)(g / half), d = (int)(g - (int64_t)r * half) * 2;
+        const int h = r / Fin, f = r - h * Fin;
+        const float* src = W + ((int64_t)h * D + d) * Fin + f;
+        if (d < D) v0 = src[0] * st;
+        if (d + 1 < D) v1 = src[Fin] * st;
+        piece = DP;
+        o = Wt + (int64_t)r * 3 * DP + d;
+    }
+    __half2 h1, h2;
+    pack_halves(v0, v1, h1, h2);
+    *reinterpret_cast<__half2*>(o) = h1;
+    *reinterpret_cast<__half2*>(o + piece) = h2;
+    *reinterpret_cast<__half2*>(o + 2 * (int64_t)piece) =
+        __halves2half2(__float2half_rn(__low2float(h1) * (1.f / kHalvesShift)), __float2half_rn(__high2float(h1) * (1.f / kHalvesShift)));
+}
+
+__global__ __launch_bounds__(kBlock) void pack_split_aggfirst_kernel(PackSplit a) {
+    __shared__ float red[kBlock / kWave];
+    pack_split_aggfirst_block(a, (int)blockIdx.x, red);
+}
+
+constexpr int kPackLayers = 8;
+struct PackStackMerge {
+    MergeArgs m[kPackLayers];
+    float* part[kPackLayers];
+    int n_tiles[kPackLayers], tiles_k[kPackLayers], first[kPackLayers + 1], n;
+};
+struct PackStackSplit {
+    PackSplit s[kPackLayers];
+    int first[kPackLayers + 1], n;
+};
+
+__global__ __launch_bounds__(kBlock) void pack_stack_merge_kernel(PackStackMerge a) {
+    __shared__ float tile[32][33];
+    __shared__ float red[2][kBlock / kWave];
+    int l = 0;
+    while (l + 1 < a.n && (int)blockIdx.x >= a.first[l + 1]) ++l;
+    pack_merge_block(a.m[l], a.n_tiles[l], a.tiles_k[l], (int)blockIdx.x - a.first[l], a.first[l + 1] - a.first[l], a.part[l], tile, red);
+}
+
+__global__ __launch_bounds__(kBlock) void pack_stack_split_kernel(PackStackSplit a) {
+    __shared__ float tile[32][33];
+    __shared__ float red[kBlock / kWave];
+    int l = 0;
+    while (l + 1 < a.n && (int)blockIdx.x >= a.first[l + 1]) ++l;
+    const PackSplit& s = a.s[l];
+    if (s.with_fc) pack_split_block(s, (int)blockIdx.x - a.first[l], tile, red);
+    else pack_split_aggfirst_block(s, (int)blockIdx.x - a.first[l], red);
 }
 
 __global__ __launch_bounds__(kBlock) void merge_bwd_w_kernel(MergeArgs a) {
@@ -147,4 +333,136 @@
     return hip_status("merge_weight_bwd launch");
 }
 
-}
+static void pack_grid(int32_t K, int32_t P, int32_t c1, int& tiles_k, int& n_tiles, int64_t& blocks) {
+    tiles_k = (K + 31) / 32, n_tiles = tiles_k * ((c1 + 31) / 32);
+    blocks = n_tiles + ((int64_t)(P - c1) * K + bot::kBlock - 1) / bot::kBlock;
+}
+
+int32_t bot_weight_pack_blocks(int32_t K, int32_t P, int32_t with_fc, int32_t has_res, int32_t block) {
+    if (K < 1 || P < 1 || block < 1) return 0;
+    const int32_t c1 = (with_fc ? block : 0) + (has_res ? block : 0);
+    if (c1 > P) return 0;
+    int tiles_k, n_tiles;
+    int64_t blocks;
+    pack_grid(K, P, c1, tiles_k, n_tiles, blocks);
+    return (int32_t)blocks;
+}
+
+int bot_weight_pack_merge_f32(const float* W, const float* Wres, const float* attn_l, const float* attn_r, int32_t H, int32_t D, int32_t K,
+                              int32_t P, int32_t with_fc, int32_t block, float* merged, float* part, bot_stream_t stream) {
+    using namespace bot;
+    if (int rc = merge_check("weight_pack_merge", W, attn_l, H, D, K, P, Wres, attn_r, with_fc, block)) return rc;
+    BOT_REQUIRE(merged && part, BOT_E_NULL, "weight_pack_merge: merged / part is NULL");
+    MergeArgs a{W, Wres, attn_l, attn_r, H, D, K, P, with_fc, block, merged, nullptr, nullptr, nullptr, nullptr, nullptr};
+    int tiles_k, n_tiles;
+    int64_t blocks;
+    pack_grid(K, P, (with_fc ? block : 0) + (Wres ? block : 0), tiles_k, n_tiles, blocks);
+    hipLaunchKernelGGL(pack_merge_kernel, dim3((unsigned)blocks), dim3(kBlock), 0, (hipStream_t)stream, a, n_tiles, tiles_k, part);
+    return hip_status("weight_pack_merge launch");
+}
+
+static int pack_split_desc(const float* merged, int32_t K, int32_t P, const float* part, int32_t n_part, float* scale, uint16_t* fwd, uint16_t* bwd,
+                           bot::PackSplit& d, int64_t& blocks) {
+    using namespace bot;
+    BOT_REQUIRE(K >= 1 && P >= 64 && P % 64 == 0 && n_part >= 1, BOT_E_RANGE, "weight_pack_split: K=%d P=%d (a multiple of 64) n_part=%d", K, P, n_part);
+    BOT_REQUIRE(merged && part && scale && fwd && bwd, BOT_E_NULL, "weight_pack_split: NULL pointer");
+    BOT_REQUIRE(aligned(fwd, 16) && aligned(bwd, 16), BOT_E_ALIGN, "weight_pack_split: the operands must be 16-byte aligned");
+    const int tiles_k = (K + 63) / 64 * 2, tiles_p = P / 32;
+    d = PackSplit{};
+    d.Wm = merged, d.part = part, d.scale = scale, d.fwd = (__half*)fwd, d.bwd = (__half*)bwd;
+    d.region_f = (int64_t)(P / 16) * tiles_k * 512, d.region_b = (int64_t)((K + 15) / 16) * tiles_p * 512;
+    d.K = K, d.P = P, d.n_part = n_part, d.tiles_k = tiles_k, d.with_fc = 1;
+    blocks = (int64_t)tiles_k * tiles_p;
+    return 0;
+}
+
+static int pack_split_aggfirst_desc(const float* W, const float* Wres, int32_t H, int32_t D, int32_t Fin, const float* part, int32_t n_part, float* scale_b,
+                                    float* scale_t, uint16_t* B, uint16_t* Wt, bot::PackSplit& d, int64_t& blocks) {
+    using namespace bot;
+    BOT_REQUIRE(H >= 1 && D >= 1 && Fin >= 1 && n_part >= 1, BOT_E_RANGE, "weight_pack_split_aggfirst: H=%d D=%d Fin=%d n_part=%d", H, D, Fin, n_part);
+    BOT_REQUIRE(W && Wres && part && scale_b && scale_t && B && Wt, BOT_E_NULL, "weight_pack_split_aggfirst: NULL pointer");
+    BOT_REQUIRE(aligned(B, 4) && aligned(Wt, 4), BOT_E_ALIGN, "weight_pack_split_aggfirst: the operands must be 4-byte aligned");
+    d = PackSplit{};
+    d.W = W, d.Wres = Wres, d.part = part, d.scale = scale_b, d.scale_t = scale_t, d.fwd = (__half*)B, d.bwd = (__half*)Wt;
+    d.H = H, d.D = D, d.K = Fin, d.n_part = n_part, d.FP = (Fin + 63) / 64 * 64, d.DP = (D + 63) / 64 * 64, d.with_fc = 0;
+    blocks = ((int64_t)H * D * d.FP + (int64_t)H * Fin * (d.DP / 2) + kBlock - 1) / kBlock;
+    return 0;
+}
+
+int bot_weight_pack_split_f16(const float* merged, int32_t K, int32_t P, const float* part, int32_t n_part, float* scale, uint16_t* fwd, uint16_t* bwd,
+                              bot_stream_t stream) {
+    using namespace bot;
+    PackSplit d;
+    int64_t blocks;
+    if (int rc = pack_split_desc(merged, K, P, part, n_part, scale, fwd, bwd, d, blocks)) return rc;
+    hipLaunchKernelGGL(pack_split_kernel, dim3((unsigned)blocks), dim3(kBlock), 0, (hipStream_t)stream, d);
+    return hip_status("weight_pack_split launch");
+}
+
+int bot_weight_pack_split_aggfirst_f16(const float* W, const float* Wres, int32_t H, int32_t D, int32_t Fin, const float* part, int32_t n_part,
+                                       float* scale_b, float* scale_t, uint16_t* B, uint16_t* Wt, bot_stream_t stream) {
+    using namespace bot;
+    PackSplit d;
+    int64_t blocks;
+    if (int rc = pack_split_aggfirst_desc(W, Wres, H, D, Fin, part, n_part, scale_b, scale_t, B, Wt, d, blocks)) return rc;
+    hipLaunchKernelGGL(pack_split_aggfirst_kernel, dim3((unsigned)blocks), dim3(kBlock), 0, (hipStream_t)stream, d);
+    return hip_status("weight_pack_split_aggfirst launch");
+}
+
+int32_t bot_weight_pack_stack_width(void) { return 17; }
+
+int bot_weight_pack_stack_f16(int32_t n_layers, const int64_t* layers, bot_stream_t stream) {
+    using namespace bot;
+    BOT_REQUIRE(n_layers >= 1 && n_layers <= kPackLayers, BOT_E_RANGE, "weight_pack_stack: %d layers (1 .. %d)", n_layers, kPackLayers);
+    BOT_REQUIRE(layers != nullptr, BOT_E_NULL, "weight_pack_stack: layers is NULL");
+    PackStackMerge pm{};
+    PackStackSplit ps{};
+    pm.n = ps.n = n_layers;
+    int64_t b1 = 0, b2 = 0;
+    for (int l = 0; l < n_layers; ++l) {
+        const int64_t* r = layers + 17 * l;
+        const float* W = (const float*)r[0];
+        const float* Wres = (const float*)r[1];
+        const float* al = (const float*)r[2];
+        const float* ar = (const float*)r[3];
+        const int32_t H = (int32_t)r[4], D = (int32_t)r[5], K = (int32_t)r[6], P = (int32_t)r[7], with_fc = (int32_t)r[8], block = (int32_t)r[9];
+        float* merged = (float*)r[10];
+        float* part = (float*)r[11];
+        const int32_t n_part = (int32_t)r[12];
+        if (int rc = merge_check("weight_pack_stack", W, al, H, D, K, P, Wres, ar, with_fc, block)) return rc;
+        BOT_REQUIRE(merged && part, BOT_E_NULL, "weight_pack_stack: layer %d: merged / part is NULL", l);
+        int tiles_k, n_tiles;
+        int64_t blocks;
+        pack_grid(K, P, (with_fc ? block : 0) + (Wres ? block : 0), tiles_k, n_tiles, blocks);
+        BOT_REQUIRE(blocks == n_part, BOT_E_RANGE, "weight_pack_stack: layer %d: n_part=%d, the grid has %lld workgroups", l, n_part, (long long)blocks);
+        pm.m[l] = MergeArgs{W, Wres, al, ar, H, D, K, P, with_fc, block, merged, nullptr, nullptr, nullptr, nullptr, nullptr};
+        pm.part[l] = part, pm.n_tiles[l] = n_tiles, pm.tiles_k[l] = tiles_k, pm.first[l] = (int)b1;
+        b1 += blocks;
+        int64_t sb;
+        if (with_fc) {
+            if (int rc = pack_split_desc(merged, K, P, part, n_part, (float*)r[13], (uint16_t*)r[14], (uint16_t*)r[15], ps.s[l], sb)) return rc;
+        } else {
+            if (int rc = pack_split_aggfirst_desc(W, Wres, H, D, K, part, n_part, (float*)r[13], (float*)r[16], (uint16_t*)r[14], (uint16_t*)r[15], ps.s[l], sb))
+                return rc;
+        }
+        ps.first[l] = (int)b2;
+        b2 += sb;
+        BOT_REQUIRE(b1 < (1 << 30) && b2 < (1 << 30), BOT_E_RANGE, "weight_pack_stack: grid too large");
+    }
+    pm.first[n_layers] = (int)b1, ps.first[n_layers] = (int)b2;
+    hipLaunchKernelGGL(pack_stack_merge_kernel, dim3((unsigned)b1), dim3(kBlock), 0, (hipStream_t)stream, pm);
+    hipLaunchKernelGGL(pack_stack_split_kernel, dim3((unsigned)b2), dim3(kBlock), 0, (hipStream_t)stream, ps);
+    return hip_status("weight_pack_stack launch");
+}
+
+int64_t bot_stream_capture_id(bot_stream_t stream) {
+    hipStreamCaptureStatus status = hipStreamCaptureStatusNone;
+    unsigned long long id = 0;
+    if (hipStreamGetCaptureInfo((hipStream_t)stream, &status, &id) != hipSuccess) {
+        (void)hipGetLastError();
+        return -1;
+    }
+    return status == hipStreamCaptureStatusActive ? (int64_t)id + 1 : 0;
+}
+
+}
diff --git a/bot_amd/nn/__init__.py b/bot_amd/nn/__init__.py
--- a/bot_amd/nn/__init__.py
+++ b/bot_amd/nn/__init__.py
@@ -343,6 +343,11 @@
             h = self.input_drop(h)
         h_last = None
         infer = self.fuse_layers and not self.training and not torch.is_grad_enabled() and (h.is_cuda or fused.FORCE)
+        packs = [None] * self.n_layers
+        if self.fuse_layers and not infer and h.is_cuda and fused.WEIGHT_PACK:
+            norms = [None if i == self.n_layers - 1 else (self.norms[i] if len(self.norms) else False) for i in range(self.n_layers)]
+            packs = fused.pack_of(self).refresh(list(self.convs), norms, self.activation, [graph] * self.n_layers if blocks is None else blocks,
+                                                self.training, self.residual, h)
         for i in range(self.n_layers):
             last = i == self.n_layers - 1
             g = graph if blocks is None else blocks[i]
@@ -363,7 +368,7 @@
                     nxt_g, rows = (graph, h.shape[0]) if blocks is None else (blocks[i + 1], g.number_of_dst_nodes())
                     y_needed = nxt_norm is False or not fused.halves_only_consumer(
                         self.convs[i + 1], nxt_norm, self.activation, nxt_g, self.training, self.residual, rows, h.is_cuda)
-                h = fused.gat_hidden_layer(self.convs[i], norm, g, h, self.dropout.p, self.training, y_needed=y_needed)
+                h = fused.gat_hidden_layer(self.convs[i], norm, g, h, self.dropout.p, self.training, y_needed=y_needed, wp=packs[i])
                 if last:
                     h = h.view(h.shape[0], self.convs[i]._num_heads, -1)
                 else:
diff --git a/bot_amd/nn/fused.py b/bot_amd/nn/fused.py
--- a/bot_amd/nn/fused.py
+++ b/bot_amd/nn/fused.py
@@ -1,6 +1,7 @@
 from __future__ import annotations
 
 import os
+import weakref
 from types import SimpleNamespace
 
 import torch
@@ -66,13 +67,13 @@
 class _MergeWeight(torch.autograd.Function):
 
     @staticmethod
-    def forward(ctx, W, Wres, attn_l, attn_r, H, D, with_fc):
-        blk = block_width(H * D) if with_fc else H * D
-        used = (blk if with_fc else 0) + (blk if Wres is not None else 0) + H + (H if attn_r is not None else 0)
-        P = used + (-used) % 128
+    def forward(ctx, W, Wres, attn_l, attn_r, H, D, with_fc, wp=None):
+        blk, P = merged_shape(H, D, with_fc, Wres is not None, attn_r is not None)
         ctx.save_for_backward(W, attn_l, attn_r)
         ctx.wres_ref = Wres
         ctx.cfg = (H, D, P, with_fc, Wres is not None, blk)
+        if wp is not None:
+            return wp.merged.detach()
         return _C.merge_weight_fwd(W, Wres, attn_l.reshape(-1), None if attn_r is None else attn_r.reshape(-1), H, D, P, with_fc, block=blk)
 
     @staticmethod
@@ -91,15 +92,21 @@
                 dW, dWres, dal, dar = body()
         else:
             dW, dWres, dal, dar = body()
-        return dW, dWres, dal.view_as(attn_l), (None if dar is None else dar.view_as(attn_r)), None, None, None
-
-
-def merged_weight(conv, with_fc=True):
+        return dW, dWres, dal.view_as(attn_l), (None if dar is None else dar.view_as(attn_r)), None, None, None, None
+
+
+def merged_shape(H, D, with_fc, has_res, has_er):
+    blk = block_width(H * D) if with_fc else H * D
+    used = (blk if with_fc else 0) + (blk if has_res else 0) + H + (H if has_er else 0)
+    return blk, used + (-used) % 128
+
+
+def merged_weight(conv, with_fc=True, wp=None):
     W = conv.fc.weight
     if W.is_cuda and WEIGHT_KP:
         return _MergeWeight.apply(W, conv.res_fc.weight if conv.res_fc is not None else None, conv.attn_l,
                                   conv.attn_r if isinstance(conv.attn_r, torch.Tensor) else None, conv._num_heads, conv._out_feats,
-                                  with_fc)
+                                  with_fc, wp)
     return _kp(cat_weight(conv) if with_fc else cat_weight_aggfirst(conv))
 
 
@@ -215,7 +222,9 @@
 
 class _GATHidden(torch.autograd.Function):
     @staticmethod
-    def forward(ctx, h, Wcat, bn_w, bn_b, graph, bn, H, D, has_res, has_er, slope, attn_p, drop_p, bn_training, kp, sym, y_needed=True):
+    def forward(ctx, h, Wcat, bn_w, bn_b, graph, bn, H, D, has_res, has_er, slope, attn_p, drop_p, bn_training, kp, sym, y_needed=True, wp=None):
+        ctx.wp = wp if (wp is not None and gemm.enabled(h)) else None
+        ctx.wp_fill = wp.fill_id if ctx.wp is not None else None
         N, HD = graph.number_of_dst_nodes(), H * D
         csc = graph.csc
         ctx.cfg, ctx.graph = (H, D, has_res, has_er, slope), graph
@@ -224,7 +233,7 @@
         xh = None
         if gemm.enabled(h):
             xh = gemm.take(h, 0)
-            ws = gemm.split_right(Wcat.t().contiguous() if kp else Wcat)
+            ws = ctx.wp.fwd if ctx.wp is not None else gemm.split_right(Wcat.t().contiguous() if kp else Wcat)
             ctx.wscale = ws.scale
             ctx.xscale = xh.scale
             out = gemm.mm_nt(xh, ws)
@@ -352,7 +361,7 @@
             else:
                 dh_ = gemm.split(dout, 0)
             if ctx.needs_input_grad[0]:
-                dh = gemm.mm_nt(dh_, gemm.split_right(Wcat if kp else Wcat.t().contiguous(), scale=ctx.wscale), link=ctx.bn_link)
+                dh = gemm.mm_nt(dh_, _right_bwd(ctx, Wcat, kp), link=ctx.bn_link)
             if ctx.needs_input_grad[1]:
                 def wgrad():
                     dW = gemm.tn(xh, dh_)
@@ -364,7 +373,13 @@
             if ctx.needs_input_grad[0]:
                 dh = torch.mm(dout, Wcat.t()) if kp else torch.mm(dout, Wcat)
         return (dh, dW, d_bn_w if ctx.needs_input_grad[2] else None, d_bn_b if ctx.needs_input_grad[3] else None,
-                None, None, None, None, None, None, None, None, None, None, None, None, None)
+                None, None, None, None, None, None, None, None, None, None, None, None, None, None)
+
+
+def _right_bwd(ctx, Wcat, kp):
+    if ctx.wp is not None:
+        return ctx.wp.checked(ctx.wp_fill).bwd
+    return gemm.split_right(Wcat if kp else Wcat.t().contiguous(), scale=ctx.wscale)
 
 
 def _backward_direct(ctx, dy, s, P, B):
@@ -403,7 +418,7 @@
     dW = dh = None
     xh = gemm.Halves(h, ctx.xscale, *ctx.halves)
     if ctx.needs_input_grad[0]:
-        Ws = gemm.split_right(Wcat if kp else Wcat.t().contiguous(), scale=ctx.wscale)
+        Ws = _right_bwd(ctx, Wcat, kp)
         link = ctx.bn_link
         st = link.stats_for(N, Ws.n, piece) if link is not None else None
         dh = _C.gemm_halves3_nt(buf, Ws.buf, s1, Ws.scale, piece, Ws.piece, piece, a2_off=piece, scale_a2=s2, k_split=c, b_frag=Ws.order == 3, n=Ws.n, bn=st)
@@ -415,7 +430,7 @@
             return dWk if kp else dWk.t().contiguous()
         dW = side.run(wgrad, xh, buf, s1, s2) if (side.usable(buf) and xh.piece * piece >= side.MIN_OUT) else wgrad()
     return (dh, dW, d_bn_w if ctx.needs_input_grad[2] else None, d_bn_b if ctx.needs_input_grad[3] else None,
-            None, None, None, None, None, None, None, None, None, None, None, None, None)
+            None, None, None, None, None, None, None, None, None, None, None, None, None, None)
 
 
 def cat_weight_aggfirst(conv):
@@ -500,7 +515,8 @@
 class _GATHiddenAggFirst(torch.autograd.Function):
 
     @staticmethod
-    def forward(ctx, h, W, Wr, bn_w, bn_b, graph, bn, H, D, has_res, has_er, slope, attn_p, drop_p, bn_training, kp, sym, y_needed=True):
+    def forward(ctx, h, W, Wr, bn_w, bn_b, graph, bn, H, D, has_res, has_er, slope, attn_p, drop_p, bn_training, kp, sym, y_needed=True, wp=None):
+        ctx.wp, ctx.wp_fill = wp, (wp.fill_id if wp is not None else None)
         N, Fin, HD = h.shape[0], h.shape[1], H * D
         Nd = graph.number_of_dst_nodes()
         csc = graph.csc
@@ -555,14 +571,17 @@
             A = torch.empty((Nd, 2 * KA), dtype=torch.float16, device=h.device)
             _C.halves_split_cols(h if Nd == N else h[:Nd], xscale, 2, A, KA, 0, FP)
             _C.spmm_bcast_halves(csc, xsrc, a_d, None, xscale, A, FP, FP, KA, FP)
-            Wres = (Wr.t()[:HD] if kp else Wr[:HD]).contiguous()
-            slots = _C.absmax_slots(h.device)
-            _C.absmax_into(Wres, slots)
-            _C.absmax_into(W, slots)
-            wscale = _C.halves_scale_from_slots(slots)
-            B = torch.empty((HD, 6 * FP), dtype=torch.float16, device=h.device)
-            _C.halves_split_cols(Wres, wscale, 1, B, 2 * FP, 0, FP)
-            _C.halves_split_cols(W, wscale, 1, B, 2 * FP, FP, FP)
+            if wp is not None:
+                B, wscale = wp.B, wp.scale_b
+            else:
+                Wres = (Wr.t()[:HD] if kp else Wr[:HD]).contiguous()
+                slots = _C.absmax_slots(h.device)
+                _C.absmax_into(Wres, slots)
+                _C.absmax_into(W, slots)
+                wscale = _C.halves_scale_from_slots(slots)
+                B = torch.empty((HD, 6 * FP), dtype=torch.float16, device=h.device)
+                _C.halves_split_cols(Wres, wscale, 1, B, 2 * FP, 0, FP)
+                _C.halves_split_cols(W, wscale, 1, B, 2 * FP, FP, FP)
             x = out2[:Nd, :HD]
             partials = None
             if bn is not None and h.is_cuda | FORCE:
@@ -629,7 +648,7 @@
             if Dh is None:
                 dscale = _C.halves_scale_from_slots(slots) if slots is not None else _C.halves_scale(dx)
                 Dh = _C.halves_split_heads(dx, dscale, H, D, DP)
-            Wt = gemm.split(Wh.transpose(1, 2).reshape(H * Fin, D), 1)
+            Wt = ctx.wp.checked(ctx.wp_fill).Wt if ctx.wp is not None else gemm.split(Wh.transpose(1, 2).reshape(H * Fin, D), 1)
             _C.gemm_halves3_nt_grouped(Dh, Wt.buf, dscale, Wt.scale, H * DP, Wt.piece, dz[0], g_dz, 0)
             flat = torch.empty(HD * Fin + P2 * Fin, dtype=h.dtype, device=h.device)
 
@@ -697,7 +716,7 @@
         if need_dh:
             dh = torch.addmm(dh_g, dout2, Wr.t() if kp else Wr)
         return (dh, dW, dWr, d_bn_w if ctx.needs_input_grad[3] else None, d_bn_b if ctx.needs_input_grad[4] else None,
-                None, None, None, None, None, None, None, None, None, None, None, None, None)
+                None, None, None, None, None, None, None, None, None, None, None, None, None, None)
 
 
 def halves_only_consumer(conv, norm, activation, graph, training, stack_residual, n_rows, on_device) -> bool:
@@ -728,7 +747,7 @@
     return v
 
 
-def gat_hidden_layer(conv, bn, graph, h, dropout_p, training, y_needed=True):
+def gat_hidden_layer(conv, bn, graph, h, dropout_p, training, y_needed=True, wp=None):
     from . import has_zero_in_degree
     if not conv._allow_zero_in_degree:
         assert not has_zero_in_degree(graph), "0-in-degree nodes (models.py:477-479)"
@@ -742,18 +761,130 @@
     if use_agg_first(conv):
         global AGG_CALLS
         AGG_CALLS += 1
-        return _GATHiddenAggFirst.apply(h, conv.fc.weight, merged_weight(conv, with_fc=False), bn_w, bn_b, graph, bn, H, D,
+        if wp is not None and wp.kind != "aggfirst":
+            wp = None
+        return _GATHiddenAggFirst.apply(h, conv.fc.weight, merged_weight(conv, with_fc=False, wp=wp), bn_w, bn_b, graph, bn, H, D,
                                         conv.res_fc is not None, conv.attn_r is not None, conv.leaky_relu.negative_slope,
                                         attn_p, dropout_p if training and bn is not None else 0.0, bn_training, WEIGHT_KP,
-                                        conv._use_symmetric_norm, y_needed)
+                                        conv._use_symmetric_norm, y_needed, wp)
+    if wp is not None and wp.kind != "merged":
+        wp = None
     if bn is None:
-        return _GATHidden.apply(h, merged_weight(conv), None, None, graph, None, H, D, conv.res_fc is not None,
+        return _GATHidden.apply(h, merged_weight(conv, wp=wp), None, None, graph, None, H, D, conv.res_fc is not None,
                                 conv.attn_r is not None, conv.leaky_relu.negative_slope, attn_p, 0.0, False, WEIGHT_KP,
-                                conv._use_symmetric_norm)
-    return _GATHidden.apply(h, merged_weight(conv), bn.weight if bn.affine else None, bn.bias if bn.affine else None, graph, bn,
+                                conv._use_symmetric_norm, True, wp)
+    return _GATHidden.apply(h, merged_weight(conv, wp=wp), bn.weight if bn.affine else None, bn.bias if bn.affine else None, graph, bn,
                             H, D, conv.res_fc is not None, conv.attn_r is not None, conv.leaky_relu.negative_slope,
                             conv.attn_drop.p if training else 0.0, dropout_p if training else 0.0, bn_training, WEIGHT_KP,
-                            conv._use_symmetric_norm, y_needed)
+                            conv._use_symmetric_norm, y_needed, wp)
+
+
+WEIGHT_PACK = os.environ.get("BOT_WEIGHT_PACK", "1") != "0"
+PACKS = 0
+
+
+def _capture_id() -> int:
+    return _C.capture_id() if torch.cuda.is_available() else 0
+
+
+class LayerPack:
+
+    def __init__(self, owner, kind, conv, device):
+        self.owner, self.kind = owner, kind
+        H, D, K = conv._num_heads, conv._out_feats, conv.fc.weight.shape[1]
+        self.with_fc = kind == "merged"
+        self.blk, self.P = merged_shape(H, D, self.with_fc, conv.res_fc is not None, conv.attn_r is not None)
+        self.H, self.D, self.K = H, D, K
+        b = self.bufs = _C.weight_pack_buffers(H, D, K, self.P, self.with_fc, conv.res_fc is not None, self.blk, device)
+        self.merged = b["merged"]
+        if self.with_fc:
+            piece = (K + gemm.PIECE_ALIGN - 1) // gemm.PIECE_ALIGN * gemm.PIECE_ALIGN
+            self.fwd = gemm.Halves(b["fwd"], b["scale"], self.P, K, piece, 3)
+            self.bwd = gemm.Halves(b["bwd"], b["scale"], K, self.P, self.P, 3)
+        else:
+            DP = (D + gemm.PIECE_ALIGN - 1) // gemm.PIECE_ALIGN * gemm.PIECE_ALIGN
+            self.B, self.scale_b = b["B"], b["scale_b"]
+            self.Wt = gemm.Halves(b["Wt"], b["scale_t"], H * K, D, DP, 1)
+
+    @property
+    def fill_id(self):
+        return self.owner.fill_id
+
+    def fill_args(self, conv):
+        return (self.bufs, conv.fc.weight.detach(), conv.res_fc.weight.detach() if conv.res_fc is not None else None,
+                conv.attn_l.detach().reshape(-1), conv.attn_r.detach().reshape(-1) if conv.attn_r is not None else None,
+                self.H, self.D, self.P, self.with_fc, self.blk)
+
+    def checked(self, fill_id):
+        if fill_id != self.owner.fill_id:
+            raise RuntimeError("bot_amd.nn.fused: the stack's weight pack was refilled between this forward and its backward (the parameters "
+                               "changed and the model ran again); run the backward first, or set BOT_WEIGHT_PACK=0")
+        return self
+
+
+def _pack_kind(conv, norm, activation, graph, training, stack_residual, h, rows, first):
+    W = conv.fc.weight if hasattr(conv, "fc") else None
+    if (W is None or not W.is_cuda or W.dtype != torch.float32 or not WEIGHT_KP or not h.is_cuda or h.dtype != torch.float32
+            or not can_fuse(conv, norm, activation, graph, training, stack_residual)
+            or not all(p is None or p.is_contiguous() for p in (W, conv.res_fc.weight if conv.res_fc is not None else None, conv.attn_l, conv.attn_r))):
+        return None
+    H, D, K = conv._num_heads, conv._out_feats, W.shape[1]
+    if use_agg_first(conv):
+        attn_p = conv.attn_drop.p if training else 0.0
+        ok = (first and not h.requires_grad and conv.res_fc is not None
+              and _l0_halves_ok(h, H, D, K, True, conv._use_symmetric_norm, attn_p, graph))
+        return "aggfirst" if ok else None
+    if not (gemm.MODE == "halves" and rows >= gemm.MIN_ROWS and gemm.RIGHT_FRAG and gemm.NT_KERNEL == "halves3"):
+        return None
+    _, P = merged_shape(H, D, True, conv.res_fc is not None, conv.attn_r is not None)
+    piece = (K + gemm.PIECE_ALIGN - 1) // gemm.PIECE_ALIGN * gemm.PIECE_ALIGN
+    frag = (P >= gemm.NT_MIN_COLS or gemm.left_order(piece) == 2) and (K >= gemm.NT_MIN_COLS or gemm.left_order(P) == 2)
+    return "merged" if frag else None
+
+
+_STACK_PACKS = weakref.WeakKeyDictionary()
+
+
+def pack_of(stack):
+    pack = _STACK_PACKS.get(stack)
+    if pack is None:
+        pack = _STACK_PACKS[stack] = WeightPack()
+    return pack
+
+
+class WeightPack:
+
+    def __init__(self):
+        self.key = self.shape_key = None
+        self.layers = []
+        self.cid = self.bufs_cid = 0
+        self.fill_id = 0
+
+    def refresh(self, convs, norms, activation, graphs, training, stack_residual, h):
+        global PACKS
+        kinds, rows = [], h.shape[0]
+        for i, (conv, norm, g) in enumerate(zip(convs, norms, graphs)):
+            kinds.append(None if norm is False else _pack_kind(conv, norm, activation, g, training, stack_residual, h, rows, i == 0))
+            rows = g.number_of_dst_nodes()
+        if not any(kinds):
+            return [None] * len(kinds)
+        packed = [c for c, k in zip(convs, kinds) if k]
+        params = [p for c in packed for p in (c.fc.weight, c.res_fc.weight if c.res_fc is not None else None, c.attn_l, c.attn_r) if p is not None]
+        cid = _capture_id()
+        shape_key = (tuple(kinds), str(h.device)) + tuple((c._num_heads, c._out_feats, c.fc.weight.shape[1], c.res_fc is not None, c.attn_r is not None)
+                                                          for c in packed)
+        key = (_versions(*params), tuple(id(p) for p in params), shape_key, gemm.MODE, gemm.NT_KERNEL, gemm.RIGHT_FRAG, WEIGHT_KP, gemm.LEFT_NODUP,
+               gemm.NODUP_MIN_PIECE, _C._stream())
+        if key == self.key and cid == self.cid:
+            return self.layers
+        if shape_key != self.shape_key or self.bufs_cid not in (0, cid):
+            self.layers = [LayerPack(self, k, c, h.device) if k else None for c, k in zip(convs, kinds)]
+            self.shape_key, self.bufs_cid = shape_key, cid
+        _C.weight_pack_fill_stack([lp.fill_args(c) for lp, c in zip(self.layers, convs) if lp is not None])
+        self.key, self.cid = key, cid
+        self.fill_id += 1
+        PACKS += 1
+        return self.layers
 
 
 
diff --git a/include/bot_gnn.h b/include/bot_gnn.h
--- a/include/bot_gnn.h
+++ b/include/bot_gnn.h
@@ -175,6 +175,17 @@
 int bot_merge_weight_bwd_f32(const float* W, const float* attn_l, const float* attn_r, int32_t H, int32_t D, int32_t K,
                              int32_t P, int32_t with_fc, int32_t block, const float* d_merged, float* dW, float* dWres,
                              float* d_attn_l, float* d_attn_r, bot_stream_t stream);
+
+int32_t bot_weight_pack_blocks(int32_t K, int32_t P, int32_t with_fc, int32_t has_res, int32_t block);
+int bot_weight_pack_merge_f32(const float* W, const float* Wres, const float* attn_l, const float* attn_r, int32_t H, int32_t D, int32_t K,
+                              int32_t P, int32_t with_fc, int32_t block, float* merged, float* part, bot_stream_t stream);
+int bot_weight_pack_split_f16(const float* merged, int32_t K, int32_t P, const float* part, int32_t n_part, float* scale, uint16_t* fwd,
+                              uint16_t* bwd, bot_stream_t stream);
+int bot_weight_pack_split_aggfirst_f16(const float* W, const float* Wres, int32_t H, int32_t D, int32_t Fin, const float* part, int32_t n_part,
+                                       float* scale_b, float* scale_t, uint16_t* B, uint16_t* Wt, bot_stream_t stream);
+int32_t bot_weight_pack_stack_width(void);
+int bot_weight_pack_stack_f16(int32_t n_layers, const int64_t* layers, bot_stream_t stream);
+int64_t bot_stream_capture_id(bot_stream_t stream);
 
 int64_t bot_edge_mlp_workspace_floats(void);
 int bot_edge_mlp_fwd_f32(const float* ef, int32_t I, const float* W1, const float* b1, int32_t J, const float* W2,
```

New measurement: 237.3 million (median of 5 runs). About the same (+0.7%).
